# ebanalyse/ebnerd-benchmark

Hardware: AMD Instinct MI355X
Metric: training impressions/sec (higher is better)
Workload: dtype f32

## Files before the change

ebnerd-benchmark_amd/csrc/ebn_attention.hip:

```cpp
#include "ebn_common.h"

int ebn_attn_mfma_fwd(const float* qkv, int64_t ld_qkv, float* out, int64_t ld_out, int64_t n_seq, int32_t L,
                      int32_t h, int32_t d, const EbnDrop& dr, hipStream_t s, bool* handled);
int ebn_attn_mfma_bwd(const float* qkv, int64_t ld_qkv, const float* dout, int64_t ld_dout, float* dqkv,
                      int64_t ld_dqkv, int64_t n_seq, int32_t L, int32_t h, int32_t d, const EbnDrop& dr,
                      hipStream_t s, bool* handled, const float* pool_w, const float* pool_d, int64_t ld_pool);

namespace {

constexpr int DMAX = 32;

struct AttnArgs {
  const float* qkv;
  int64_t ld_qkv;
  const float* dout;
  int64_t ld_dout;
  float* out;
  int64_t ld_out;
  int64_t n_prob;
  int32_t L, h, d;
  const uint32_t* key_ptr;
  uint32_t thresh;
  float scale;
};

template <int GW>
__device__ __forceinline__ void load_tile(float* __restrict__ tile, const float* __restrict__ src,
                                          int64_t ld, int64_t row0, int col0, int L, int d, int gl) {
  const int n = L * d;
  for (int e = gl; e < n; e += GW) {
    const int l = e / d;
    const int c = e - l * d;
    tile[e] = src[(row0 + l) * ld + col0 + c];
  }
}

template <int GW>
__device__ __forceinline__ void softmax_scores(const float* __restrict__ sQ, const float* __restrict__ sK,
                                               float* __restrict__ sP, int L, int LP, int d, int gl) {
  if (gl < L) {
    float q[DMAX];
#pragma unroll
    for (int c = 0; c < DMAX; ++c) q[c] = (c < d) ? sQ[gl * d + c] : 0.f;
    const float inv = 1.0f / sqrtf(static_cast<float>(d));
    float mx = -INFINITY;
    for (int j = 0; j < L; ++j) {
      float s = 0.f;
#pragma unroll
      for (int c = 0; c < DMAX; ++c)
        if (c < d) s = fmaf(q[c], sK[j * d + c], s);
      s *= inv;
      sP[gl * LP + j] = s;
      mx = fmaxf(mx, s);
    }
    float sum = 0.f;
    for (int j = 0; j < L; ++j) {
      const float p = expf(sP[gl * LP + j] - mx);
      sP[gl * LP + j] = p;
      sum += p;
    }
    for (int j = 0; j < L; ++j) sP[gl * LP + j] = sP[gl * LP + j] / sum;
  }
}

template <int GW>
__global__ __launch_bounds__(64) void attn_fwd_kernel(AttnArgs a) {
  extern __shared__ __attribute__((aligned(16))) float smem[];
  constexpr int G = 64 / GW;
  const int lane = threadIdx.x;
  const int g = lane / GW;
  const int gl = lane % GW;
  const int L = a.L, d = a.d;
  const int LP = (L & 1) ? L + 2 : L + 1;
  const int tile = L * d;
  const int per_group = 3 * tile + L * LP;
  float* base = smem + g * per_group;
  float* sQ = base;
  float* sK = base + tile;
  float* sV = base + 2 * tile;
  float* sP = base + 3 * tile;

  const int64_t prob = static_cast<int64_t>(blockIdx.x) * G + g;
  const bool active = prob < a.n_prob;
  const int64_t seq = active ? prob / a.h : 0;
  const int head = active ? static_cast<int>(prob - seq * a.h) : 0;
  const int E = a.h * d;
  const int64_t row0 = seq * L;
  if (active) {
    load_tile<GW>(sQ, a.qkv, a.ld_qkv, row0, head * d, L, d, gl);
// ... 339 lines not shown
  const bool short_ok = L <= 64 && static_cast<size_t>((L <= 32 ? 2 : 1) * (3 * L * d + L * LPs)) * sizeof(float) <= 65536;
  if (!short_ok) {
    const size_t lds = static_cast<size_t>(3 * L * d + 2 * L) * sizeof(float);
    EBN_REQUIRE(lds <= 160 * 1024 && a.n_prob <= 0x7FFFFFFF, EBN_ERR_UNSUPPORTED);
    allow_big_lds(attn_long_fwd_kernel, lds);
    EBN_LAUNCH(attn_long_fwd_kernel, dim3(static_cast<unsigned>(a.n_prob)), dim3(LONG_THREADS), lds, ebn_stream(stream), a);
    EBN_CHECK_LAUNCH();
    return EBN_OK;
  }
  const int LP = (L & 1) ? L + 2 : L + 1;
  const int per_group = 3 * L * d + L * LP;
  EBN_REQUIRE(static_cast<size_t>((L <= 32 ? 2 : 1) * per_group) * sizeof(float) <= 65536, EBN_ERR_UNSUPPORTED);
  if (L <= 32) {
    const int64_t grid = ebn_ceil_div(a.n_prob, 2);
    EBN_LAUNCH(attn_fwd_kernel<32>, dim3(static_cast<unsigned>(grid)), dim3(64),
                       2 * per_group * sizeof(float), ebn_stream(stream), a);
  } else {
    EBN_LAUNCH(attn_fwd_kernel<64>, dim3(static_cast<unsigned>(a.n_prob)), dim3(64),
                       per_group * sizeof(float), ebn_stream(stream), a);
  }
  EBN_CHECK_LAUNCH();
  return EBN_OK;
}

extern "C" int ebn_attn_bwd_f32(const float* qkv, int64_t ld_qkv, const float* dout, int64_t ld_dout,
                                float* dqkv, int64_t ld_dqkv, int64_t n_seq, int32_t L, int32_t h, int32_t d,
                                const ebn_step_state* st, int32_t site, float drop_p, ebn_stream_t stream) {
  int rc = check_attn_args(qkv, dqkv, n_seq, L, h, d);
  if (rc != EBN_OK) return rc;
  EBN_REQUIRE(dout, EBN_ERR_BAD_ARG);
  if (n_seq == 0) return EBN_OK;
  EBN_REQUIRE(ld_qkv >= 3 * h * d && ld_dqkv >= 3 * h * d && ld_dout >= h * d, EBN_ERR_BAD_ARG);
  const EbnDrop dr = ebn_make_drop(st, site, drop_p);
  bool handled = false;
  rc = ebn_attn_mfma_bwd(qkv, ld_qkv, dout, ld_dout, dqkv, ld_dqkv, n_seq, L, h, d, dr, ebn_stream(stream), &handled, nullptr,
                         nullptr, 0);
  if (rc != EBN_OK || handled) return rc;
  AttnArgs a{qkv, ld_qkv, dout, ld_dout, dqkv, ld_dqkv, n_seq * h, L, h, d, dr.key_ptr, dr.thresh, dr.scale};
  const int LPs = (L & 1) ? L + 2 : L + 1;
  const bool short_ok = L <= 64 && static_cast<size_t>((L <= 32 ? 2 : 1) * (4 * L * d + 2 * L * LPs)) * sizeof(float) <= 65536;
  if (!short_ok) {
    const size_t lds = static_cast<size_t>(4 * L * d + 3 * L) * sizeof(float);
    EBN_REQUIRE(lds <= 160 * 1024 && a.n_prob <= 0x7FFFFFFF, EBN_ERR_UNSUPPORTED);
    allow_big_lds(attn_long_bwd_kernel, lds);
    EBN_LAUNCH(attn_long_bwd_kernel, dim3(static_cast<unsigned>(a.n_prob)), dim3(LONG_THREADS), lds, ebn_stream(stream), a);
    EBN_CHECK_LAUNCH();
    return EBN_OK;
  }
  const int LP = (L & 1) ? L + 2 : L + 1;
  const int per_group = 4 * L * d + 2 * L * LP;
  EBN_REQUIRE(static_cast<size_t>((L <= 32 ? 2 : 1) * per_group) * sizeof(float) <= 65536, EBN_ERR_UNSUPPORTED);
  if (L <= 32) {
    const int64_t grid = ebn_ceil_div(a.n_prob, 2);
    EBN_LAUNCH(attn_bwd_kernel<32>, dim3(static_cast<unsigned>(grid)), dim3(64),
                       2 * per_group * sizeof(float), ebn_stream(stream), a);
  } else {
    EBN_LAUNCH(attn_bwd_kernel<64>, dim3(static_cast<unsigned>(a.n_prob)), dim3(64),
                       per_group * sizeof(float), ebn_stream(stream), a);
  }
  EBN_CHECK_LAUNCH();
  return EBN_OK;
}

extern "C" int ebn_attn_bwd_pooled_f32(const float* qkv, int64_t ld_qkv, const float* dout, int64_t ld_dout,
                                       const float* pool_w, const float* pool_dout, int64_t ld_pool, float* dqkv,
                                       int64_t ld_dqkv, int64_t n_seq, int32_t L, int32_t h, int32_t d,
                                       const ebn_step_state* st, int32_t site, float drop_p, ebn_stream_t stream) {
  int rc = check_attn_args(qkv, dqkv, n_seq, L, h, d);
  if (rc != EBN_OK) return rc;
  EBN_REQUIRE(dout && pool_w && pool_dout, EBN_ERR_BAD_ARG);
  if (n_seq == 0) return EBN_OK;
  EBN_REQUIRE(ld_qkv >= 3 * h * d && ld_dqkv >= 3 * h * d && ld_dout >= h * d && ld_pool >= h * d, EBN_ERR_BAD_ARG);
  const EbnDrop dr = ebn_make_drop(st, site, drop_p);
  bool handled = false;
  rc = ebn_attn_mfma_bwd(qkv, ld_qkv, dout, ld_dout, dqkv, ld_dqkv, n_seq, L, h, d, dr, ebn_stream(stream), &handled, pool_w,
                         pool_dout, ld_pool);
  if (rc != EBN_OK) return rc;
  return handled ? EBN_OK : EBN_ERR_UNSUPPORTED;
}

extern "C" int ebn_attn_bwd_pooled_supported(int32_t L, int32_t d) {
  return (L > 0 && L <= 64 && (d == 16 || d == 20 || d == 32)) ? 1 : 0;
}
```

ebnerd-benchmark_amd/csrc/ebn_attention_mfma.hip:

```cpp
#include <stdlib.h>

#include "ebn_common.h"

namespace {

typedef float f32x16 __attribute__((ext_vector_type(16)));

constexpr int ATT_WAVES = 4;

struct MfmaAttnArgs {
  const float* qkv;
  int64_t ld_qkv;
  const float* dout;
  int64_t ld_dout;
  float* out;
  int64_t ld_out;
  int64_t n_prob;
  int32_t L, h;
  const uint32_t* key_ptr;
  uint32_t thresh;
  float scale;
  const float* pool_w;
  const float* pool_d;
  int64_t ld_pool;
  uint32_t stagger_units, stagger_shift, stagger_mod;
};

__device__ __forceinline__ int crow(int r, int hi) { return (r & 3) + 8 * (r >> 2) + 4 * hi; }

template <int D>
struct Tile {
  static constexpr int STRIDE = (D % 16 == 0) ? D + 4 : D;
  static constexpr int FLOATS = 32 * STRIDE;
  static constexpr int VPR = D / 4;
  static constexpr int VECS = 32 * VPR;
  static constexpr int ROUNDS = (VECS + 63) / 64;
};

__device__ __forceinline__ void wave_lds_sync() {
  __builtin_amdgcn_fence(__ATOMIC_RELEASE, "wavefront");
  __builtin_amdgcn_wave_barrier();
  __builtin_amdgcn_fence(__ATOMIC_ACQUIRE, "wavefront");
}

template <int D>
struct Staged {
  float4 v[Tile<D>::ROUNDS];
};

template <int D>
__device__ __forceinline__ void stage_load(Staged<D>& st, const float* __restrict__ base, uint32_t ld, int L, int lane) {
  using T = Tile<D>;
#pragma unroll
  for (int t = 0; t < T::ROUNDS; ++t) {
    int v = lane + 64 * t;
    if (T::VECS % 64 != 0 && v >= T::VECS) v = 0;
    const int r = v / T::VPR, c4 = v - r * T::VPR;
    const uint32_t rc = r < L ? r : 0;
    st.v[t] = *reinterpret_cast<const float4*>(base + (rc * ld + static_cast<uint32_t>(c4 * 4)));
  }
}

template <int D>
struct PoolTerm {
  float w[Tile<D>::ROUNDS];
  float4 p[Tile<D>::ROUNDS];
};

template <int D>
__device__ __forceinline__ void pool_load(PoolTerm<D>& pt, const float* __restrict__ w_rows, const float* __restrict__ d_cols,
                                          int L, int lane) {
  using T = Tile<D>;
#pragma unroll
  for (int t = 0; t < T::ROUNDS; ++t) {
    int v = lane + 64 * t;
    if (T::VECS % 64 != 0 && v >= T::VECS) v = 0;
    const int r = v / T::VPR, c4 = v - r * T::VPR;
    pt.w[t] = w_rows[r < L ? r : 0];
    pt.p[t] = *reinterpret_cast<const float4*>(d_cols + c4 * 4);
  }
}

template <int D>
__device__ __forceinline__ void pool_add(Staged<D>& st, const PoolTerm<D>& pt) {
#pragma unroll
  for (int t = 0; t < Tile<D>::ROUNDS; ++t) {
    st.v[t].x = fmaf(pt.w[t], pt.p[t].x, st.v[t].x);
    st.v[t].y = fmaf(pt.w[t], pt.p[t].y, st.v[t].y);
    st.v[t].z = fmaf(pt.w[t], pt.p[t].z, st.v[t].z);
    st.v[t].w = fmaf(pt.w[t], pt.p[t].w, st.v[t].w);
  }
}

template <int D, bool DROP>
__device__ __forceinline__ void stage_store(float* __restrict__ lds, const Staged<D>& st, int L, int lane, uint32_t key,
                                            uint64_t e0, int E, uint32_t thresh, float scale) {
  using T = Tile<D>;
#pragma unroll
  for (int t = 0; t < T::ROUNDS; ++t) {
    const int v = lane + 64 * t;
    if (T::VECS % 64 != 0 && v >= T::VECS) break;
    const int r = v / T::VPR, c4 = v - r * T::VPR;
    if (r >= L) continue;
    float4 y = st.v[t];
    if (DROP) {
      const uint64_t pr = (e0 >> 1) + ((static_cast<uint32_t>(r) * static_cast<uint32_t>(E) + static_cast<uint32_t>(c4 * 4)) >> 1);
      const uint32_t h0 = ebn_dropout_pair_hash(key, pr), h1 = ebn_dropout_pair_hash(key, pr + 1);
      y.x *= ((h0 & 0xFFFFu) >= thresh) ? scale : 0.f;
// ... 74 lines not shown
                                                 float mul) {
  if (row >= L) return;
#pragma unroll
  for (int g = 0; g < 4; ++g) {
    const int c0 = 8 * g + 4 * hi;
    if (c0 < D) {
      float4 v = make_float4(acc[4 * g] * mul, acc[4 * g + 1] * mul, acc[4 * g + 2] * mul, acc[4 * g + 3] * mul);
      *reinterpret_cast<float4*>(lds + row * Tile<D>::STRIDE + c0) = v;
    }
  }
}

template <int D, bool DROP>
__device__ __forceinline__ void tile_rows_to_global(float* __restrict__ base, uint32_t ld, const f32x16& acc, int L, int row,
                                                    int hi, float mul, uint32_t key, uint64_t e0, int E, uint32_t thresh,
                                                    float scale) {
  if (row >= L) return;
#pragma unroll
  for (int g = 0; g < 4; ++g) {
    const int c0 = 8 * g + 4 * hi;
    if (c0 < D) {
      float4 y = make_float4(acc[4 * g] * mul, acc[4 * g + 1] * mul, acc[4 * g + 2] * mul, acc[4 * g + 3] * mul);
      if (DROP) {
        const uint64_t pr = (e0 >> 1) + ((static_cast<uint32_t>(row) * static_cast<uint32_t>(E) + static_cast<uint32_t>(c0)) >> 1);
        const uint32_t h0 = ebn_dropout_pair_hash(key, pr), h1 = ebn_dropout_pair_hash(key, pr + 1);
        y.x *= ((h0 & 0xFFFFu) >= thresh) ? scale : 0.f;
        y.y *= ((h0 >> 16) >= thresh) ? scale : 0.f;
        y.z *= ((h1 & 0xFFFFu) >= thresh) ? scale : 0.f;
        y.w *= ((h1 >> 16) >= thresh) ? scale : 0.f;
      }
      *reinterpret_cast<float4*>(base + (static_cast<uint32_t>(row) * ld + static_cast<uint32_t>(c0))) = y;
    }
  }
}

template <int D>
__device__ __forceinline__ void global_row_form(float (&x)[D / 2], const float* __restrict__ base, uint32_t ld, int L, int row, int hi) {
  constexpr int KH = D / 2;
  const float2* p = reinterpret_cast<const float2*>(base + (static_cast<uint32_t>(row < L ? row : 0) * ld + static_cast<uint32_t>(hi * KH)));
#pragma unroll
  for (int s = 0; s < KH / 2; ++s) {
    const float2 v = p[s];
    x[2 * s] = v.x;
    x[2 * s + 1] = v.y;
  }
}

__device__ __forceinline__ void softmax_in_lane(f32x16& t, int L, int hi, float inv2) {
  float m = -INFINITY;
#pragma unroll
  for (int r = 0; r < 16; ++r) {
    t[r] *= inv2;
    if (crow(r, hi) < L) m = fmaxf(m, t[r]);
  }
  m = fmaxf(m, __shfl_xor(m, 32, 64));
  float z = 0.f;
#pragma unroll
  for (int r = 0; r < 16; ++r) {
    t[r] = (crow(r, hi) < L) ? __builtin_amdgcn_exp2f(t[r] - m) : 0.f;
    z += t[r];
  }
  z += __shfl_xor(z, 32, 64);
  const float rz = 1.0f / z;
#pragma unroll
  for (int r = 0; r < 16; ++r) t[r] *= rz;
}

constexpr int TP_STRIDE = 36;
constexpr int TP_FLOATS = 32 * TP_STRIDE;

__device__ __forceinline__ void tile_transpose(f32x16& t, float* __restrict__ buf, int L, int lane_row, int hi) {
  float* w = buf + 4 * hi * TP_STRIDE + lane_row;
#pragma unroll
  for (int r = 0; r < 16; ++r) w[((r & 3) + 8 * (r >> 2)) * TP_STRIDE] = t[r];
  wave_lds_sync();
  const float* rd = buf + lane_row * TP_STRIDE + 4 * hi;
#pragma unroll
  for (int g = 0; g < 4; ++g) {
    const float4 v = *reinterpret_cast<const float4*>(rd + 8 * g);
    t[4 * g] = (8 * g + 4 * hi + 0 < L) ? v.x : 0.f;
    t[4 * g + 1] = (8 * g + 4 * hi + 1 < L) ? v.y : 0.f;
    t[4 * g + 2] = (8 * g + 4 * hi + 2 < L) ? v.z : 0.f;
    t[4 * g + 3] = (8 * g + 4 * hi + 3 < L) ? v.w : 0.f;
  }
}


struct AttnProb {
  int64_t row0;
  uint32_t seq;
  uint32_t head;
};

__device__ __forceinline__ uint32_t xcd_chunked_block() {
  const uint32_t nwg = gridDim.x, orig = blockIdx.x;
  const uint32_t q = nwg >> 3, r = nwg & 7u, xcd = orig & 7u, idx = orig >> 3;
  return ((xcd < r) ? xcd * (q + 1) : r * (q + 1) + (xcd - r) * q) + idx;
}

__device__ __forceinline__ void stagger_first_round(const MfmaAttnArgs& a) {
  if (a.stagger_units != 0u && blockIdx.x < (a.stagger_mod << a.stagger_shift)) {
    const uint32_t n = ((blockIdx.x >> a.stagger_shift) % a.stagger_mod) * a.stagger_units;
    for (uint32_t i = 0; i < n; ++i) __builtin_amdgcn_s_sleep(8);
  }
}

__device__ __forceinline__ AttnProb attn_prob(int64_t prob, int h, int L) {
  AttnProb p;
  p.seq = static_cast<uint32_t>(prob) / static_cast<uint32_t>(h);
  p.head = static_cast<uint32_t>(prob) - p.seq * static_cast<uint32_t>(h);
  p.row0 = static_cast<int64_t>(p.seq) * L;
  return p;
}

template <int D>
__host__ __device__ constexpr int fwd_wave_floats(int L) {
  return L * Tile<D>::STRIDE > TP_FLOATS ? L * Tile<D>::STRIDE : TP_FLOATS;
}

template <int D, int LC>
__global__ __launch_bounds__(64 * ATT_WAVES) void attn_mfma_fwd_kernel(MfmaAttnArgs a) {
  extern __shared__ __attribute__((aligned(16))) float smem[];
  const int lane = threadIdx.x & 63;
  const int wv = __builtin_amdgcn_readfirstlane(threadIdx.x >> 6);
  const int64_t prob = static_cast<int64_t>(xcd_chunked_block()) * ATT_WAVES + wv;
  if (prob >= a.n_prob) return;
  const int L = LC ? LC : a.L, E = a.h * D;
  float* sv = smem + wv * fwd_wave_floats<D>(L);
  const int row = lane & 31, hi = lane >> 5;
  const float inv2 = 1.44269504088896341f / sqrtf(static_cast<float>(D));
  const bool drop = a.key_ptr != nullptr;
  const uint32_t key = drop ? *a.key_ptr : 0u;

  const AttnProb p = attn_prob(prob, a.h, L);
  const float* qb = a.qkv + p.row0 * a.ld_qkv + p.head * D;
  float qr[D / 2], kr[D / 2];
  {
    Staged<D> tv;
    stage_load<D>(tv, qb + 2 * E, a.ld_qkv, L, lane);
    global_row_form<D>(qr, qb, a.ld_qkv, L, row, hi);
    global_row_form<D>(kr, qb + E, a.ld_qkv, L, row, hi);
    stage_store<D, false>(sv, tv, L, lane, 0u, 0u, 0, 0u, 0.f);
  }
  wave_lds_sync();
  float vc[16];
  lds_col_form<D>(vc, sv, L, row, hi);

  f32x16 P = mm_rows<D / 2>(kr, qr);
  softmax_in_lane(P, L, hi, inv2);
  wave_lds_sync();
  tile_transpose(P, sv, L, row, hi);
  const f32x16 O = mm_col_tile(vc, P);
  float* ob = a.out + p.row0 * a.ld_out + p.head * D;
  const uint64_t e0 = static_cast<uint64_t>(p.row0) * E + p.head * D;
  if (drop) tile_rows_to_global<D, true>(ob, a.ld_out, O, L, row, hi, 1.0f, key, e0, E, a.thresh, a.scale);
  else tile_rows_to_global<D, false>(ob, a.ld_out, O, L, row, hi, 1.0f, 0u, 0u, 0, 0u, 0.f);
}

template <int D>
__host__ __device__ constexpr int fwd_group_v_offset(int L) {
  return 2 * L * Tile<D>::STRIDE > TP_FLOATS ? 2 * L * Tile<D>::STRIDE : TP_FLOATS;
}
__host__ __device__ constexpr int group_tile_pad(int L);
template <int D>
__host__ __device__ constexpr int fwd_group_wave_floats(int L) {
  return fwd_group_v_offset<D>(L) + L * Tile<D>::STRIDE + group_tile_pad(L);
// ... 14 lines not shown
  const int wave_floats = fwd_group_wave_floats<D>(L), v_off = fwd_group_v_offset<D>(L);
  const int row = lane & 31, hi = lane >> 5;
  const float inv2 = 1.44269504088896341f / sqrtf(static_cast<float>(D));
  const bool drop = a.key_ptr != nullptr;
  const uint32_t key = drop ? *a.key_ptr : 0u;

  const AttnProb p0 = attn_prob(static_cast<int64_t>(xcd_chunked_block()) * G, a.h, L);
  const uint32_t gcol = p0.head * D;
  const float* gq = a.qkv + p0.row0 * a.ld_qkv + gcol;
  const int nvec = L * GV;
  {
    float4 vq[ROUNDS], vk[ROUNDS], vv[ROUNDS];
    uint32_t dst[ROUNDS];
#pragma unroll
    for (int t = 0; t < ROUNDS; ++t) {
      const int idx = tid + NT * t;
      const int idc = idx < nvec ? idx : 0;
      const uint32_t r = static_cast<uint32_t>(idc) / static_cast<uint32_t>(GV), c4g = static_cast<uint32_t>(idc) - r * GV;
      const uint32_t head = c4g / T::VPR, c4 = c4g - head * T::VPR;
      dst[t] = head * wave_floats + r * T::STRIDE + c4 * 4;
      const uint32_t off = r * static_cast<uint32_t>(a.ld_qkv) + c4g * 4;
      vq[t] = *reinterpret_cast<const float4*>(gq + off);
      vk[t] = *reinterpret_cast<const float4*>(gq + E + off);
      vv[t] = *reinterpret_cast<const float4*>(gq + 2 * E + off);
    }
#pragma unroll
    for (int t = 0; t < ROUNDS; ++t) {
      if (tid + NT * t < nvec) {
        *reinterpret_cast<float4*>(smem + dst[t]) = vq[t];
        *reinterpret_cast<float4*>(smem + dst[t] + region) = vk[t];
        *reinterpret_cast<float4*>(smem + dst[t] + v_off) = vv[t];
      }
    }
  }
  __syncthreads();

  float* sq = smem + wv * wave_floats;
  float* sk = sq + region;
  float* sv = sq + v_off;
  f32x16 P;
  {
    float qr[D / 2], kr[D / 2];
    lds_row_form<D>(qr, sq, L, row, hi);
    lds_row_form<D>(kr, sk, L, row, hi);
    P = mm_rows<D / 2>(kr, qr);
  }
  float vc[16];
  lds_col_form<D>(vc, sv, L, row, hi);
  softmax_in_lane(P, L, hi, inv2);
  wave_lds_sync();
  tile_transpose(P, sq, L, row, hi);
  {
    const f32x16 O = mm_col_tile(vc, P);
    tile_rows_to_lds<D>(sv, O, L, row, hi, 1.0f);
  }
  __syncthreads();

  float* go = a.out + p0.row0 * a.ld_out + gcol;
#pragma unroll
  for (int t = 0; t < ROUNDS; ++t) {
    const int idx = tid + NT * t;
    if (idx < nvec) {
      const uint32_t r = static_cast<uint32_t>(idx) / static_cast<uint32_t>(GV), c4g = static_cast<uint32_t>(idx) - r * GV;
      const uint32_t head = c4g / T::VPR, c4 = c4g - head * T::VPR;
      float4 y = *reinterpret_cast<const float4*>(smem + head * wave_floats + v_off + r * T::STRIDE + c4 * 4);
      if (drop) {
        const uint64_t pr = ((static_cast<uint64_t>(p0.row0) * E + gcol) >> 1) + ((r * static_cast<uint32_t>(E) + c4g * 4) >> 1);
        const uint32_t h0 = ebn_dropout_pair_hash(key, pr), h1 = ebn_dropout_pair_hash(key, pr + 1);
        y.x *= ((h0 & 0xFFFFu) >= a.thresh) ? a.scale : 0.f;
        y.y *= ((h0 >> 16) >= a.thresh) ? a.scale : 0.f;
        y.z *= ((h1 & 0xFFFFu) >= a.thresh) ? a.scale : 0.f;
        y.w *= ((h1 >> 16) >= a.thresh) ? a.scale : 0.f;
      }
      *reinterpret_cast<float4*>(go + (r * static_cast<uint32_t>(a.ld_out) + c4g * 4)) = y;
    }
  }
}

template <int D>
__host__ __device__ constexpr int bwd_wave_floats(int L) {
  return 3 * L * Tile<D>::STRIDE > L * Tile<D>::STRIDE + TP_FLOATS ? 3 * L * Tile<D>::STRIDE : L * Tile<D>::STRIDE + TP_FLOATS;
}

template <int D, int LC>
__global__ __launch_bounds__(64 * ATT_WAVES) void attn_mfma_bwd_kernel(MfmaAttnArgs a) {
  using T = Tile<D>;
  constexpr int KH = D / 2;
  extern __shared__ __attribute__((aligned(16))) float smem[];
  const int lane = threadIdx.x & 63;
  const int wv = __builtin_amdgcn_readfirstlane(threadIdx.x >> 6);
  const int64_t prob = static_cast<int64_t>(xcd_chunked_block()) * ATT_WAVES + wv;
  if (prob >= a.n_prob) return;
  const int L = LC ? LC : a.L, E = a.h * D;
  const int region = L * T::STRIDE;
  float* sq = smem + wv * bwd_wave_floats<D>(L);
  float* sk = sq + region;
  float* sg = sk + region;
  const int row = lane & 31, hi = lane >> 5;
  const float inv = 1.0f / sqrtf(static_cast<float>(D));
  const float inv2 = inv * 1.44269504088896341f;
  const bool drop = a.key_ptr != nullptr, pooled = a.pool_w != nullptr;
  const uint32_t key = drop ? *a.key_ptr : 0u;

  const AttnProb p = attn_prob(prob, a.h, L);
  const float* qb = a.qkv + p.row0 * a.ld_qkv + p.head * D;
  float vr[KH];
  {
    Staged<D> tq, tk, tg;
    stage_load<D>(tq, qb, a.ld_qkv, L, lane);
    stage_load<D>(tk, qb + E, a.ld_qkv, L, lane);
    stage_load<D>(tg, a.dout + p.row0 * a.ld_dout + p.head * D, a.ld_dout, L, lane);
    global_row_form<D>(vr, qb + 2 * E, a.ld_qkv, L, row, hi);
    if (pooled) {
      PoolTerm<D> pt;
      pool_load<D>(pt, a.pool_w + p.row0, a.pool_d + p.seq * a.ld_pool + p.head * D, L, lane);
      pool_add<D>(tg, pt);
    }
    stage_store<D, false>(sq, tq, L, lane, 0u, 0u, 0, 0u, 0.f);
    stage_store<D, false>(sk, tk, L, lane, 0u, 0u, 0, 0u, 0.f);
    if (drop) stage_store<D, true>(sg, tg, L, lane, key, static_cast<uint64_t>(p.row0) * E + p.head * D, E, a.thresh, a.scale);
    else stage_store<D, false>(sg, tg, L, lane, 0u, 0u, 0, 0u, 0.f);
  }
  wave_lds_sync();

  float* ob = a.out + p.row0 * a.ld_out + p.head * D;
  f32x16 P, dP;
  {
    float qr[KH], kr[KH];
    lds_row_form<D>(qr, sq, L, row, hi);
    lds_row_form<D>(kr, sk, L, row, hi);
    P = mm_rows<KH>(kr, qr);
  }
  softmax_in_lane(P, L, hi, inv2);
  {
    float gr[KH];
    lds_row_form<D>(gr, sg, L, row, hi);
    dP = mm_rows<KH>(gr, vr);
  }
  float rowdot = 0.f;
#pragma unroll
  for (int r = 0; r < 16; ++r) rowdot = fmaf(P[r], dP[r], rowdot);
  rowdot += __shfl_xor(rowdot, 32, 64);

  float col[16];
  lds_col_form<D>(col, sg, L, row, hi);
  {
    const f32x16 dV = mm_col_tile(col, P);
    tile_rows_to_global<D, false>(ob + 2 * E, a.ld_out, dV, L, row, hi, 1.0f, 0u, 0u, 0, 0u, 0.f);
  }
#pragma unroll
  for (int r = 0; r < 16; ++r) P[r] = P[r] * (dP[r] - rowdot);
  lds_col_form<D>(col, sk, L, row, hi);
  {
    const f32x16 dQ = mm_col_tile(col, P);
    tile_rows_to_global<D, false>(ob, a.ld_out, dQ, L, row, hi, inv, 0u, 0u, 0, 0u, 0.f);
  }
  wave_lds_sync();
  tile_transpose(P, sk, L, row, hi);
  lds_col_form<D>(col, sq, L, row, hi);
  {
    const f32x16 dK = mm_col_tile(col, P);
    tile_rows_to_global<D, false>(ob + E, a.ld_out, dK, L, row, hi, inv, 0u, 0u, 0, 0u, 0.f);
  }
}


template <int D>
__host__ __device__ constexpr int bwd_group_g_offset(int L) {
  return 2 * L * Tile<D>::STRIDE > TP_FLOATS ? 2 * L * Tile<D>::STRIDE : TP_FLOATS;
}
__host__ __device__ constexpr int group_tile_pad(int L) { return L == 30 ? 12 : 0; }
template <int D>
__host__ __device__ constexpr int bwd_group_wave_floats(int L) {
  return bwd_group_g_offset<D>(L) + L * Tile<D>::STRIDE + group_tile_pad(L);
}

template <int D, int LC, int G>
__global__ __launch_bounds__(64 * G) void attn_mfma_bwd_group_kernel(MfmaAttnArgs a) {
  using T = Tile<D>;
  constexpr int KH = D / 2;
  constexpr int NT = 64 * G;
  constexpr int GV = G * T::VPR;
  constexpr int ROUNDS = (32 * GV + NT - 1) / NT;
  extern __shared__ __attribute__((aligned(16))) float smem[];
  const int tid = threadIdx.x;
  const int lane = tid & 63;
  const int wv = __builtin_amdgcn_readfirstlane(tid >> 6);
  const int L = LC ? LC : a.L, E = a.h * D;
  const int region = L * T::STRIDE;
  const int wave_floats = bwd_group_wave_floats<D>(L), g_off = bwd_group_g_offset<D>(L);
  const int row = lane & 31, hi = lane >> 5;
  const float inv = 1.0f / sqrtf(static_cast<float>(D));
  const float inv2 = inv * 1.44269504088896341f;
  const bool drop = a.key_ptr != nullptr, pooled = a.pool_w != nullptr;
  const uint32_t key = drop ? *a.key_ptr : 0u;

  stagger_first_round(a);
  const AttnProb p0 = attn_prob(static_cast<int64_t>(xcd_chunked_block()) * G, a.h, L);
  const uint32_t gcol = p0.head * D;
  const float* gq = a.qkv + p0.row0 * a.ld_qkv + gcol;
  const float* gd = a.dout + p0.row0 * a.ld_dout + gcol;
  const int nvec = L * GV;
  float vr[KH];
// ... 150 lines not shown
  for (int r = 0; r < 16; ++r) {
    const int il = crow(r, hi);
    const float ci = __shfl(c_ib, il, 64);
    s[r] = (32 * ib + il < L) ? __builtin_amdgcn_exp2f(s[r] * inv2 - ci) : 0.f;
  }
}

template <int D, int LC>
__global__ __launch_bounds__(64 * ATT2_WAVES) void attn_mfma2_fwd_kernel(MfmaAttnArgs a) {
  using T = Tile<D>;
  constexpr int KH = D / 2;
  extern __shared__ __attribute__((aligned(16))) float smem[];
  const int lane = threadIdx.x & 63;
  const int wv = __builtin_amdgcn_readfirstlane(threadIdx.x >> 6);
  const int64_t prob = static_cast<int64_t>(xcd_chunked_block()) * ATT2_WAVES + wv;
  if (prob >= a.n_prob) return;
  const int L = LC ? LC : a.L, E = a.h * D;
  const int region = L * T::STRIDE;
  float* sq = smem + wv * 3 * region;
  float* sk = sq + region;
  float* sv = sk + region;
  const int row = lane & 31, hi = lane >> 5;
  const int64_t seq = prob / a.h;
  const int head = static_cast<int>(prob - seq * a.h);
  const int64_t row0 = seq * L;
  const float* qb = a.qkv + row0 * a.ld_qkv + head * D;
  const float inv2 = 1.44269504088896341f / sqrtf(static_cast<float>(D));
  {
    Staged<D> tq[NB2], tk[NB2], tv[NB2];
#pragma unroll
    for (int b = 0; b < NB2; ++b) {
      stage_load<D>(tq[b], qb + 32 * b * a.ld_qkv, a.ld_qkv, L - 32 * b, lane);
      stage_load<D>(tk[b], qb + E + 32 * b * a.ld_qkv, a.ld_qkv, L - 32 * b, lane);
      stage_load<D>(tv[b], qb + 2 * E + 32 * b * a.ld_qkv, a.ld_qkv, L - 32 * b, lane);
    }
#pragma unroll
    for (int b = 0; b < NB2; ++b) {
      stage_store<D, false>(sq + 32 * b * T::STRIDE, tq[b], L - 32 * b, lane, 0u, 0u, 0, 0u, 0.f);
      stage_store<D, false>(sk + 32 * b * T::STRIDE, tk[b], L - 32 * b, lane, 0u, 0u, 0, 0u, 0.f);
      stage_store<D, false>(sv + 32 * b * T::STRIDE, tv[b], L - 32 * b, lane, 0u, 0u, 0, 0u, 0.f);
    }
  }
  wave_lds_sync();
  float qr[NB2][KH], kr[NB2][KH], vc[NB2][16];
#pragma unroll
  for (int b = 0; b < NB2; ++b) {
    lds_row_form<D>(qr[b], sq + 32 * b * T::STRIDE, L - 32 * b, row, hi);
    lds_row_form<D>(kr[b], sk + 32 * b * T::STRIDE, L - 32 * b, row, hi);
    lds_col_form<D>(vc[b], sv + 32 * b * T::STRIDE, L - 32 * b, row, hi);
  }
  float c[NB2];
#pragma unroll
  for (int ib = 0; ib < NB2; ++ib) {
    f32x16 t[NB2];
#pragma unroll
    for (int jb = 0; jb < NB2; ++jb) t[jb] = mm_rows<KH>(kr[jb], qr[ib]);
    c[ib] = softmax2_in_lane<false>(t, L, hi, inv2);
  }
  wave_lds_sync();
#pragma unroll
  for (int jb = 0; jb < NB2; ++jb) {
    f32x16 O = zero_tile();
#pragma unroll
    for (int ib = 0; ib < NB2; ++ib) {
      f32x16 S = mm_rows<KH>(qr[ib], kr[jb]);
      softmax2_from_stats(S, L, ib, hi, inv2, c[ib]);
      mm_col_tile_acc(O, vc[ib], S);
    }
    tile_rows_to_lds<D>(sq + 32 * jb * T::STRIDE, O, L - 32 * jb, row, hi, 1.0f);
  }
  wave_lds_sync();
  float* ob = a.out + row0 * a.ld_out + head * D;
  const uint64_t e0 = static_cast<uint64_t>(row0) * E + head * D;
#pragma unroll
  for (int b = 0; b < NB2; ++b) {
    if (a.key_ptr != nullptr)
      stage_out<D, true>(sq + 32 * b * T::STRIDE, ob + 32 * b * a.ld_out, a.ld_out, L - 32 * b, lane, *a.key_ptr,
                         e0 + static_cast<uint64_t>(32 * b) * E, E, a.thresh, a.scale);
    else
      stage_out<D, false>(sq + 32 * b * T::STRIDE, ob + 32 * b * a.ld_out, a.ld_out, L - 32 * b, lane, 0u, 0u, 0, 0u, 0.f);
  }
}

template <int D, int LC>
__global__ __launch_bounds__(64 * ATT2_WAVES) void attn_mfma2_bwd_kernel(MfmaAttnArgs a) {
  using T = Tile<D>;
  constexpr int KH = D / 2;
  extern __shared__ __attribute__((aligned(16))) float smem[];
  const int lane = threadIdx.x & 63;
  const int wv = __builtin_amdgcn_readfirstlane(threadIdx.x >> 6);
  const int64_t prob = static_cast<int64_t>(xcd_chunked_block()) * ATT2_WAVES + wv;
  if (prob >= a.n_prob) return;
  const int L = LC ? LC : a.L, E = a.h * D;
  const int region = L * T::STRIDE;
  float* sq = smem + wv * 4 * region;
  float* sk = sq + region;
  float* sv = sk + region;
  float* sg = sv + region;
  const int row = lane & 31, hi = lane >> 5;
  const int64_t seq = prob / a.h;
  const int head = static_cast<int>(prob - seq * a.h);
  const int64_t row0 = seq * L;
  const float* qb = a.qkv + row0 * a.ld_qkv + head * D;
  const float* gb = a.dout + row0 * a.ld_dout + head * D;
  const float inv = 1.0f / sqrtf(static_cast<float>(D));
  const float inv2 = inv * 1.44269504088896341f;
#pragma unroll
  for (int b = 0; b < NB2; ++b) {
    Staged<D> tq, tk, tv, tg;
    const int Lb = L - 32 * b;
    stage_load<D>(tq, qb + 32 * b * a.ld_qkv, a.ld_qkv, Lb, lane);
    stage_load<D>(tk, qb + E + 32 * b * a.ld_qkv, a.ld_qkv, Lb, lane);
    stage_load<D>(tv, qb + 2 * E + 32 * b * a.ld_qkv, a.ld_qkv, Lb, lane);
    stage_load<D>(tg, gb + 32 * b * a.ld_dout, a.ld_dout, Lb, lane);
    if (a.pool_w != nullptr) {
      PoolTerm<D> pt;
      pool_load<D>(pt, a.pool_w + row0 + 32 * b, a.pool_d + seq * a.ld_pool + head * D, Lb, lane);
      pool_add<D>(tg, pt);
    }
    stage_store<D, false>(sq + 32 * b * T::STRIDE, tq, Lb, lane, 0u, 0u, 0, 0u, 0.f);
    stage_store<D, false>(sk + 32 * b * T::STRIDE, tk, Lb, lane, 0u, 0u, 0, 0u, 0.f);
    stage_store<D, false>(sv + 32 * b * T::STRIDE, tv, Lb, lane, 0u, 0u, 0, 0u, 0.f);
    if (a.key_ptr != nullptr)
      stage_store<D, true>(sg + 32 * b * T::STRIDE, tg, Lb, lane, *a.key_ptr,
                           static_cast<uint64_t>(row0 + 32 * b) * E + head * D, E, a.thresh, a.scale);
    else
      stage_store<D, false>(sg + 32 * b * T::STRIDE, tg, Lb, lane, 0u, 0u, 0, 0u, 0.f);
  }
  wave_lds_sync();

  float* ob = a.out + row0 * a.ld_out + head * D;
  float c[NB2], rowdot[NB2];
  float vr[NB2][KH];
#pragma unroll
  for (int b = 0; b < NB2; ++b) lds_row_form<D>(vr[b], sv + 32 * b * T::STRIDE, L - 32 * b, row, hi);
  wave_lds_sync();
#pragma unroll
  for (int ib = 0; ib < NB2; ++ib) {
    f32x16 P[NB2], dP[NB2];
    {
      float qr[KH];
      lds_row_form<D>(qr, sq + 32 * ib * T::STRIDE, L - 32 * ib, row, hi);
#pragma unroll
      for (int jb = 0; jb < NB2; ++jb) {
        float kr[KH];
        lds_row_form<D>(kr, sk + 32 * jb * T::STRIDE, L - 32 * jb, row, hi);
        P[jb] = mm_rows<KH>(kr, qr);
      }
    }
    c[ib] = softmax2_in_lane<true>(P, L, hi, inv2);
    float rd = 0.f;
#pragma unroll
    for (int jb = 0; jb < NB2; ++jb) {
      float gr[KH];
      lds_row_form<D>(gr, sg + 32 * jb * T::STRIDE, L - 32 * jb, row, hi);
      dP[jb] = mm_rows<KH>(gr, vr[ib]);
#pragma unroll
      for (int r = 0; r < 16; ++r) rd = fmaf(P[jb][r], dP[jb][r], rd);
    }
    rd += __shfl_xor(rd, 32, 64);
    rowdot[ib] = rd;
    float col[16];
    {
      f32x16 dV = zero_tile();
#pragma unroll
      for (int jb = 0; jb < NB2; ++jb) {
        lds_col_form<D>(col, sg + 32 * jb * T::STRIDE, L - 32 * jb, row, hi);
        mm_col_tile_acc(dV, col, P[jb]);
      }
      wave_lds_sync();
      tile_rows_to_lds<D>(sv + 32 * ib * T::STRIDE, dV, L - 32 * ib, row, hi, 1.0f);
      wave_lds_sync();
      stage_out<D, false>(sv + 32 * ib * T::STRIDE, ob + 2 * E + 32 * ib * a.ld_out, a.ld_out, L - 32 * ib, lane, 0u, 0u, 0, 0u, 0.f);
    }
#pragma unroll
    for (int jb = 0; jb < NB2; ++jb)
#pragma unroll
      for (int r = 0; r < 16; ++r) P[jb][r] = P[jb][r] * (dP[jb][r] - rd);
    {
      f32x16 dQ = zero_tile();
#pragma unroll
      for (int jb = 0; jb < NB2; ++jb) {
        lds_col_form<D>(col, sk + 32 * jb * T::STRIDE, L - 32 * jb, row, hi);
        mm_col_tile_acc(dQ, col, P[jb]);
      }
      wave_lds_sync();
      tile_rows_to_lds<D>(sv + 32 * ib * T::STRIDE, dQ, L - 32 * ib, row, hi, inv);
      wave_lds_sync();
      stage_out<D, false>(sv + 32 * ib * T::STRIDE, ob + 32 * ib * a.ld_out, a.ld_out, L - 32 * ib, lane, 0u, 0u, 0, 0u, 0.f);
    }
  }
#pragma unroll
  for (int jb = 0; jb < NB2; ++jb) {
    float kr[KH], gr[KH];
    lds_row_form<D>(kr, sk + 32 * jb * T::STRIDE, L - 32 * jb, row, hi);
    lds_row_form<D>(gr, sg + 32 * jb * T::STRIDE, L - 32 * jb, row, hi);
    f32x16 dK = zero_tile();
#pragma unroll
    for (int ib = 0; ib < NB2; ++ib) {
      f32x16 P, dP;
      {
        float qr[KH];
        lds_row_form<D>(qr, sq + 32 * ib * T::STRIDE, L - 32 * ib, row, hi);
        P = mm_rows<KH>(qr, kr);
      }
      softmax2_from_stats(P, L, ib, hi, inv2, c[ib]);
      dP = mm_rows<KH>(vr[ib], gr);
#pragma unroll
      for (int r = 0; r < 16; ++r) {
        const float rdi = __shfl(rowdot[ib], crow(r, hi), 64);
        P[r] = P[r] * (dP[r] - rdi);
// ... 68 lines not shown
}

template <int D>
static void launch_mfma2(bool bwd, const MfmaAttnArgs& a, hipStream_t s) {
  if (D == 20 && a.L == 50 && !bwd) launch_mfma2_lc<D, 50>(bwd, a, s);
  else launch_mfma2_lc<D, 0>(bwd, a, s);
}

int ebn_attn_mfma_fwd(const float* qkv, int64_t ld_qkv, float* out, int64_t ld_out, int64_t n_seq, int32_t L,
                      int32_t h, int32_t d, const EbnDrop& dr, hipStream_t s, bool* handled) {
  *handled = mfma_path_ok(L, d, ld_qkv, ld_out, ld_out, qkv, out, out) && n_seq * h < (int64_t{1} << 31);
  if (!*handled) return EBN_OK;
  MfmaAttnArgs a{qkv, ld_qkv, nullptr, 0, out, ld_out, n_seq * h, L, h, dr.key_ptr, dr.thresh, dr.scale, nullptr, nullptr, 0, 0u, 0u, 1u};
  if (L > 32) {
    if (d == 16) launch_mfma2<16>(false, a, s);
    else if (d == 20) launch_mfma2<20>(false, a, s);
    else launch_mfma2<32>(false, a, s);
    EBN_CHECK_LAUNCH();
    return EBN_OK;
  }
  const bool big = a.n_prob * L * 3 * d * static_cast<int64_t>(sizeof(float)) >= FWD_GROUP_MIN_QKV_BYTES;
  if (d == 20 && (h % BWD_GROUP) == 0 && big && !bwd_group_off()) {
    const size_t lds = static_cast<size_t>(BWD_GROUP) * fwd_group_wave_floats<20>(L) * sizeof(float);
    const dim3 grid(static_cast<unsigned>(a.n_prob / BWD_GROUP)), block(64 * BWD_GROUP);
    if (L == 30) {
      allow_lds(attn_mfma_fwd_group_kernel<20, 30, BWD_GROUP>, lds);
      EBN_LAUNCH((attn_mfma_fwd_group_kernel<20, 30, BWD_GROUP>), grid, block, lds, s, a);
    } else {
      allow_lds(attn_mfma_fwd_group_kernel<20, 0, BWD_GROUP>, lds);
      EBN_LAUNCH((attn_mfma_fwd_group_kernel<20, 0, BWD_GROUP>), grid, block, lds, s, a);
    }
    EBN_CHECK_LAUNCH();
    return EBN_OK;
  }
  const size_t wb = static_cast<size_t>(ATT_WAVES) * sizeof(float);
  if (d == 16) launch_waves(attn_mfma_fwd_kernel<16, 0>, wb * fwd_wave_floats<16>(L), a, s);
  else if (d == 20 && L == 30) launch_waves(attn_mfma_fwd_kernel<20, 30>, wb * fwd_wave_floats<20>(L), a, s);
  else if (d == 20 && L == 20) launch_waves(attn_mfma_fwd_kernel<20, 20>, wb * fwd_wave_floats<20>(L), a, s);
  else if (d == 20) launch_waves(attn_mfma_fwd_kernel<20, 0>, wb * fwd_wave_floats<20>(L), a, s);
  else launch_waves(attn_mfma_fwd_kernel<32, 0>, wb * fwd_wave_floats<32>(L), a, s);
  EBN_CHECK_LAUNCH();
  return EBN_OK;
}

int ebn_attn_mfma_bwd(const float* qkv, int64_t ld_qkv, const float* dout, int64_t ld_dout, float* dqkv,
                      int64_t ld_dqkv, int64_t n_seq, int32_t L, int32_t h, int32_t d, const EbnDrop& dr,
                      hipStream_t s, bool* handled, const float* pool_w, const float* pool_d, int64_t ld_pool) {
  *handled = mfma_path_ok(L, d, ld_qkv, ld_dout, ld_dqkv, qkv, dout, dqkv) && n_seq * h < (int64_t{1} << 31) &&
             (pool_w == nullptr || ((ld_pool % 4) == 0 && ebn_aligned16(pool_d)));
  if (!*handled) return EBN_OK;
  MfmaAttnArgs a{qkv, ld_qkv, dout, ld_dout, dqkv, ld_dqkv, n_seq * h, L, h, dr.key_ptr, dr.thresh, dr.scale, pool_w, pool_d, ld_pool, 0u, 0u, 1u};
  if (L > 32) {
    if (d == 16) launch_mfma2<16>(true, a, s);
    else if (d == 20) launch_mfma2<20>(true, a, s);
    else launch_mfma2<32>(true, a, s);
    EBN_CHECK_LAUNCH();
    return EBN_OK;
  }
  if (d == 20 && (h % BWD_GROUP) == 0 && a.n_prob >= BWD_GROUP_MIN_PROBLEMS && !bwd_group_off()) {
    const size_t lds = static_cast<size_t>(BWD_GROUP) * bwd_group_wave_floats<20>(L) * sizeof(float);
    const dim3 grid(static_cast<unsigned>(a.n_prob / BWD_GROUP)), block(64 * BWD_GROUP);
    a.stagger_shift = stagger_shift_of_device();
    a.stagger_units = a.stagger_shift != 0u ? 7u : 0u;
    a.stagger_mod = 5u;
    if (L == 30) {
      allow_lds(attn_mfma_bwd_group_kernel<20, 30, BWD_GROUP>, lds);
      EBN_LAUNCH((attn_mfma_bwd_group_kernel<20, 30, BWD_GROUP>), grid, block, lds, s, a);
    } else {
      allow_lds(attn_mfma_bwd_group_kernel<20, 0, BWD_GROUP>, lds);
      EBN_LAUNCH((attn_mfma_bwd_group_kernel<20, 0, BWD_GROUP>), grid, block, lds, s, a);
    }
    EBN_CHECK_LAUNCH();
    return EBN_OK;
  }
  const size_t wb = static_cast<size_t>(ATT_WAVES) * sizeof(float);
  if (d == 16) launch_waves(attn_mfma_bwd_kernel<16, 0>, wb * bwd_wave_floats<16>(L), a, s);
  else if (d == 20 && L == 30) launch_waves(attn_mfma_bwd_kernel<20, 30>, wb * bwd_wave_floats<20>(L), a, s);
  else if (d == 20 && L == 20) launch_waves(attn_mfma_bwd_kernel<20, 20>, wb * bwd_wave_floats<20>(L), a, s);
  else if (d == 20) launch_waves(attn_mfma_bwd_kernel<20, 0>, wb * bwd_wave_floats<20>(L), a, s);
  else launch_waves(attn_mfma_bwd_kernel<32, 0>, wb * bwd_wave_floats<32>(L), a, s);
  EBN_CHECK_LAUNCH();
  return EBN_OK;
}
```

ebnerd-benchmark_amd/csrc/ebn_encoder.hip:

```cpp
#include "ebn_common.h"

#define EBN_TRY(call)            \
  do {                           \
    int rc__ = (call);           \
    if (rc__ != EBN_OK) return rc__; \
  } while (0)

static int check_dims(const ebn_encoder_dims* d) {
  EBN_REQUIRE(d, EBN_ERR_BAD_ARG);
  EBN_REQUIRE(d->n_seq >= 0 && d->L > 0 && d->Din > 0 && d->h > 0 && d->d > 0 && d->A > 0, EBN_ERR_BAD_ARG);
  return EBN_OK;
}

extern "C" int ebn_encoder_fwd_f32(const ebn_encoder_dims* dims, const ebn_encoder_params* p,
                                   const ebn_encoder_acts* a, const ebn_encoder_scratch* s,
                                   const ebn_step_state* st, ebn_stream_t stream) {
  EBN_TRY(check_dims(dims));
  EBN_REQUIRE(p && a && p->Wqkv && p->W && p->b && p->q, EBN_ERR_BAD_ARG);
  EBN_REQUIRE(a->X && a->QKV && a->Y && a->U && a->w && a->out, EBN_ERR_BAD_ARG);
  const int64_t R = dims->n_seq * dims->L;
  const int E = dims->h * dims->d;
  if (R == 0) return EBN_OK;
  float* ws = s ? s->gemm_ws : nullptr;
  const int64_t ws_n = s ? s->gemm_ws_floats : 0;
  EBN_TRY(ebn_gemm_f32_site(0, 0, R, 3 * E, dims->Din, 1.0f, a->X, dims->Din, p->Wqkv, 3 * E, 0.0f, a->QKV, 3 * E, ws, ws_n,
                            1, stream));
  EBN_TRY(ebn_attn_fwd_f32(a->QKV, 3 * E, a->Y, E, dims->n_seq, dims->L, dims->h, dims->d, st, dims->drop_site,
                           dims->drop_p, stream));
  EBN_TRY(ebn_gemm_f32_ws(0, 0, R, dims->A, E, 1.0f, a->Y, E, p->W, dims->A, 0.0f, a->U, dims->A, ws, ws_n, stream));
  EBN_TRY(ebn_attpool_fwd_f32(a->U, p->b, p->q, a->Y, a->out, a->w, dims->n_seq, dims->L, E, dims->A, stream));
  return EBN_OK;
}

extern "C" int ebn_encoder_fwd_gather_f32(const ebn_encoder_dims* dims, const ebn_encoder_params* p, const ebn_encoder_acts* a,
                                          const ebn_encoder_scratch* s, const int32_t* ids, const float* table, int64_t table_rows,
                                          int32_t* oob_flag, ebn_stream_t stream) {
  EBN_TRY(check_dims(dims));
  EBN_REQUIRE(p && a && ids && table && p->Wqkv && p->W && p->b && p->q, EBN_ERR_BAD_ARG);
  EBN_REQUIRE(a->QKV && a->Y && a->U && a->w && a->out, EBN_ERR_BAD_ARG);
  EBN_REQUIRE(dims->drop_p <= 0.0f, EBN_ERR_UNSUPPORTED);
  const int64_t R = dims->n_seq * dims->L;
  const int E = dims->h * dims->d;
  if (R == 0) return EBN_OK;
  float* ws = s ? s->gemm_ws : nullptr;
  const int64_t ws_n = s ? s->gemm_ws_floats : 0;
  EBN_TRY(ebn_gemm_f32_rowmap(ids, table_rows, R, 3 * E, dims->Din, table, dims->Din, p->Wqkv, 3 * E, a->QKV, 3 * E, oob_flag, stream));
  EBN_TRY(ebn_attn_fwd_f32(a->QKV, 3 * E, a->Y, E, dims->n_seq, dims->L, dims->h, dims->d, nullptr, -1, 0.0f, stream));
  EBN_TRY(ebn_gemm_f32_ws(0, 0, R, dims->A, E, 1.0f, a->Y, E, p->W, dims->A, 0.0f, a->U, dims->A, ws, ws_n, stream));
  EBN_TRY(ebn_attpool_fwd_f32(a->U, p->b, p->q, a->Y, a->out, a->w, dims->n_seq, dims->L, E, dims->A, stream));
  return EBN_OK;
}

extern "C" int ebn_encoder_bwd_f32(const ebn_encoder_dims* dims, const ebn_encoder_params* p,
                                   const ebn_encoder_acts* a, const float* dout, const ebn_encoder_grads* g,
                                   const ebn_encoder_scratch* s, float* dX, int32_t accumulate,
                                   const ebn_step_state* st, ebn_stream_t stream) {
  EBN_TRY(check_dims(dims));
  EBN_REQUIRE(p && a && g && s && dout, EBN_ERR_BAD_ARG);
  EBN_REQUIRE(p->Wqkv && p->W && p->q, EBN_ERR_BAD_ARG);
  EBN_REQUIRE(a->X && a->QKV && a->Y && a->U && a->w, EBN_ERR_BAD_ARG);
  EBN_REQUIRE(g->dWqkv && g->dW && g->db && g->dq, EBN_ERR_BAD_ARG);
  EBN_REQUIRE(s->dY && s->dQKV && s->de && s->partials, EBN_ERR_BAD_ARG);
  const int64_t R = dims->n_seq * dims->L;
  const int E = dims->h * dims->d;
  const int A = dims->A;
  if (R == 0) return EBN_OK;
  const float beta = accumulate ? 1.0f : 0.0f;
  EBN_TRY(ebn_attpool_bwd_pool_f32(a->Y, a->w, dout, nullptr, s->de, dims->n_seq, dims->L, E, stream));
  EBN_TRY(ebn_attpool_bwd_dpre_f32(a->U, p->q, s->de, g->dq, g->db, s->partials, R, A, accumulate, stream));
  const bool fold = ebn_attn_bwd_pooled_supported(dims->L, dims->d) != 0 && (E % 4) == 0 && ebn_aligned16(dout) &&
                    ebn_aligned16(s->dY) && ebn_aligned16(a->QKV) && ebn_aligned16(s->dQKV);
  if (fold) {
    EBN_TRY(ebn_dense_bwd_pair_f32(R, E, A, a->Y, E, a->U, A, p->W, A, beta, g->dW, A, s->dY, E, s->gemm_ws, s->gemm_ws_floats,
                                   stream));
    EBN_TRY(ebn_attn_bwd_pooled_f32(a->QKV, 3 * E, s->dY, E, a->w, dout, E, s->dQKV, 3 * E, dims->n_seq, dims->L, dims->h,
                                    dims->d, st, dims->drop_site, dims->drop_p, stream));
  } else {
    EBN_TRY(ebn_gemm_f32_ws(1, 0, E, A, R, 1.0f, a->Y, E, a->U, A, beta, g->dW, A, s->gemm_ws, s->gemm_ws_floats, stream));
    EBN_TRY(ebn_gemm_f32_rank1(R, E, A, 1.0f, a->U, A, p->W, A, s->dY, E, a->w, dout, E, dims->L, s->gemm_ws,
                               s->gemm_ws_floats, stream));
    EBN_TRY(ebn_attn_bwd_f32(a->QKV, 3 * E, s->dY, E, s->dQKV, 3 * E, dims->n_seq, dims->L, dims->h, dims->d, st, dims->drop_site,
                             dims->drop_p, stream));
  }
  if (dX != nullptr)
    return ebn_dense_bwd_pair_f32(R, dims->Din, 3 * E, a->X, dims->Din, s->dQKV, 3 * E, p->Wqkv, 3 * E, beta, g->dWqkv, 3 * E, dX,
                                  dims->Din, s->gemm_ws, s->gemm_ws_floats, stream);
  EBN_TRY(ebn_gemm_f32_ws(1, 0, dims->Din, 3 * E, R, 1.0f, a->X, dims->Din, s->dQKV, 3 * E, beta, g->dWqkv, 3 * E,
                          s->gemm_ws, s->gemm_ws_floats, stream));
  return EBN_OK;
}

extern "C" int ebn_user_stage_train_f32(const ebn_encoder_dims* dims, const ebn_encoder_params* p, const ebn_encoder_acts* a,
                                        const float* cand, const float* labels, float* scores, float* probs, float* loss_rows,
                                        float* loss_out, float* dcand, float* duser, const ebn_encoder_grads* g,
                                        const ebn_encoder_scratch* s, float* head_partials, float* dX, int32_t C,
                                        int32_t loss_kind, float inv_batch, const ebn_step_state* st, ebn_stream_t stream) {
  EBN_TRY(check_dims(dims));
  EBN_REQUIRE(p && a && g && s && cand && labels && scores && probs && loss_rows && loss_out && dcand && duser && dX, EBN_ERR_BAD_ARG);
  EBN_REQUIRE(p->Wqkv && p->W && p->b && p->q && a->X && a->QKV && a->Y && a->U && a->w && a->out, EBN_ERR_BAD_ARG);
  EBN_REQUIRE(g->dWqkv && g->dW && g->db && g->dq && s->dY && s->dQKV && s->de && s->partials, EBN_ERR_BAD_ARG);
  EBN_REQUIRE(C > 0 && dims->drop_p <= 0.0f, EBN_ERR_BAD_ARG);
  const int64_t B = dims->n_seq, R = dims->n_seq * dims->L;
  const int E = dims->h * dims->d, A = dims->A, L = dims->L;
  if (R == 0) return EBN_OK;
  const bool fused = head_partials != nullptr && ebn_user_head_supported(L, C, E, A) != 0 &&
                     ebn_attn_bwd_pooled_supported(L, dims->d) != 0 && ebn_aligned16(a->U) && ebn_aligned16(a->Y) &&
                     ebn_aligned16(cand) && ebn_aligned16(dcand) && ebn_aligned16(duser) && ebn_aligned16(a->out) &&
                     ebn_aligned16(p->b) && ebn_aligned16(p->q) && ebn_aligned16(s->dY) && ebn_aligned16(a->QKV) &&
                     ebn_aligned16(s->dQKV);
  if (!fused) {
    EBN_TRY(ebn_encoder_fwd_f32(dims, p, a, s, st, stream));
    EBN_TRY(ebn_score_loss_train_f32(cand, a->out, labels, scores, probs, loss_rows, loss_out, dcand, duser, B, C, E, loss_kind,
                                     inv_batch, stream));
    return ebn_encoder_bwd_f32(dims, p, a, duser, g, s, dX, 0, st, stream);
  }
  float* ws = s->gemm_ws;
  const int64_t ws_n = s->gemm_ws_floats;
  EBN_TRY(ebn_gemm_f32_site(0, 0, R, 3 * E, dims->Din, 1.0f, a->X, dims->Din, p->Wqkv, 3 * E, 0.0f, a->QKV, 3 * E, ws, ws_n, 1, stream));
  EBN_TRY(ebn_attn_fwd_f32(a->QKV, 3 * E, a->Y, E, B, L, dims->h, dims->d, nullptr, -1, 0.0f, stream));
  EBN_TRY(ebn_gemm_f32_ws(0, 0, R, A, E, 1.0f, a->Y, E, p->W, A, 0.0f, a->U, A, ws, ws_n, stream));
  EBN_TRY(ebn_user_head_train_f32(a->U, p->b, p->q, a->Y, cand, labels, a->w, a->out, scores, probs, loss_rows, loss_out, dcand,
                                  duser, s->de, g->dq, g->db, head_partials, B, L, C, E, A, loss_kind, inv_batch, stream));
  EBN_TRY(ebn_dense_bwd_pair_f32(R, E, A, a->Y, E, a->U, A, p->W, A, 0.0f, g->dW, A, s->dY, E, ws, ws_n, stream));
  EBN_TRY(ebn_attn_bwd_pooled_f32(a->QKV, 3 * E, s->dY, E, a->w, duser, E, s->dQKV, 3 * E, B, L, dims->h, dims->d, nullptr, -1, 0.0f,
                                  stream));
  return ebn_dense_bwd_pair_f32(R, dims->Din, 3 * E, a->X, dims->Din, s->dQKV, 3 * E, p->Wqkv, 3 * E, 0.0f, g->dWqkv, 3 * E, dX,
                                dims->Din, ws, ws_n, stream);
}
```

ebnerd-benchmark_amd/csrc/ebn_gemm.hip:

```cpp
#include <stdlib.h>

#include "ebn_common.h"
#include "ebn_finish.h"
#include "ebn_tn_finale.h"

typedef float ebn_f32x4 __attribute__((ext_vector_type(4)));
typedef int ebn_i32x4 __attribute__((ext_vector_type(4)));
__device__ ebn_f32x4 ebn_raw_buffer_load_x4(ebn_i32x4 rsrc, int voffset, int soffset, int aux) __asm("llvm.amdgcn.raw.buffer.load.v4f32");
__device__ void ebn_raw_buffer_load_lds(ebn_i32x4 rsrc, __attribute__((address_space(3))) void* lds, int size, int voffset,
                                        int soffset, int offset, int aux) __asm("llvm.amdgcn.raw.buffer.load.lds");

int ebn_gemm_direct_tn_slices(int64_t M, int64_t N, int64_t K);
int ebn_gemm_direct_tn_launch(int64_t M, int64_t N, int64_t K, float alpha, const float* A, int64_t lda, const float* B, int64_t ldb,
                              float* part, hipStream_t s);
bool ebn_gemm_direct_wanted(int32_t transA, int32_t transB, int64_t M, int64_t N, int64_t K);
int ebn_gemm_direct_launch(int32_t transB, int64_t M, int64_t N, int64_t K, float alpha, const float* A, int64_t lda, const float* B,
                           int64_t ldb, float* C, int64_t ldc, hipStream_t s);

namespace {

typedef float f32x16 __attribute__((ext_vector_type(16)));


typedef float f32x4n __attribute__((ext_vector_type(4)));
// ... 798 lines not shown
  if (nk > 1) EBN_SM_LOAD(1, 1);
  EBN_SM_STORE(0, 0);
  __syncthreads();
  for (int kt = 0; kt < nk; kt += 2) {
    if (kt + 2 < nk) EBN_SM_LOAD(0, kt + 2);
    EBN_SM_MMA(0, kt);
    if (kt + 1 < nk) EBN_SM_STORE(1, 1);
    __syncthreads();
    if (kt + 1 >= nk) break;
    if (kt + 3 < nk) EBN_SM_LOAD(1, kt + 3);
    EBN_SM_MMA(1, kt + 1);
    if (kt + 2 < nk) EBN_SM_STORE(0, 0);
    __syncthreads();
  }
#undef EBN_SM_LOAD
#undef EBN_SM_STORE
#undef EBN_SM_MMA
#undef EBN_SM_READ
#undef EBN_SM_MUL
  const f32x4 acc = (acc0 + acc1) + (acc2 + acc3);
  if (do_colsum) {
    constexpr int CG = T / 4, KR = THREADS / CG;
    float* sc = smem_small;
    *reinterpret_cast<float4*>(&sc[(tid / CG) * (T + 4) + (tid % CG) * 4]) = csum;
    __syncthreads();
    if (tid < T && n0 + tid < N) {
      float t = 0.f;
      for (int r = 0; r < KR; ++r) t += sc[r * (T + 4) + tid];
      epi.colsum[n0 + tid] = t;
      if (FIN) ebn_adam_flat_apply(fin->adam, fin->adam.st->adam_alpha, (epi.colsum + n0 + tid) - fin->adam.grad, t);
    }
  }
  const int64_t col = n0 + wn * 16 + r16;
  if (col < N) {
    const float al = FIN ? fin->adam.st->adam_alpha : 0.f;
#pragma unroll
    for (int r = 0; r < 4; ++r) {
      const int64_t row = m0 + wm * 16 + 4 * kq + r;
      if (row >= M) continue;
      float v = alpha * acc[r];
      if (beta != 0.f) v += beta * C[row * ldc + col];
      if (epi.rs != nullptr)
        v = fmaf(epi.rs[row], epi.cv[static_cast<int64_t>(static_cast<uint32_t>(row) / static_cast<uint32_t>(epi.L)) * epi.ldcv + col], v);
      if (epi.bias != nullptr) v = fmaxf(v + epi.bias[col], 0.f);
      if (epi.l2w != nullptr) v = fmaf(epi.two_lambda, epi.l2w[row * ldc + col], v);
      C[row * ldc + col] = v;
      if (FIN) ebn_adam_flat_apply(fin->adam, al, (C + row * ldc + col) - fin->adam.grad, v);
    }
  }
}

template <bool TA, bool TB, int T>
__global__ __launch_bounds__(T * T / 4) void gemm_small_vec_kernel(int64_t M, int64_t N, int64_t K, float alpha,
                                                                      const float* __restrict__ A, int64_t lda,
                                                                      const float* __restrict__ B, int64_t ldb, float beta,
                                                                      float* __restrict__ C, int64_t ldc, GemmEpi epi) {
  small_vec_body<TA, TB, T>(M, N, K, alpha, A, lda, B, ldb, beta, C, ldc, epi, blockIdx.x, blockIdx.y);
}

struct SmallProblem {
  int64_t M, N, K;
  float alpha;
  const float* A;
  int64_t lda;
  const float* B;
  int64_t ldb;
  float beta;
  float* C;
  int64_t ldc;
  int32_t tiles_x, tiles;
};

__global__ __launch_bounds__(GEMM_THREADS) void gemm_small_pair_kernel(SmallProblem p0, SmallProblem p1) {
  const GemmEpi none{nullptr, nullptr, 0, 1, nullptr};
  const int b = blockIdx.x;
  if (b < p0.tiles)
    small_vec_body<true, false, 32>(p0.M, p0.N, p0.K, p0.alpha, p0.A, p0.lda, p0.B, p0.ldb, p0.beta, p0.C, p0.ldc, none,
                                    b % p0.tiles_x, b / p0.tiles_x);
  else
    small_vec_body<false, true, 32>(p1.M, p1.N, p1.K, p1.alpha, p1.A, p1.lda, p1.B, p1.ldb, p1.beta, p1.C, p1.ldc, none,
                                    (b - p0.tiles) % p1.tiles_x, (b - p0.tiles) / p1.tiles_x);
}

struct SmallGroup {
  SmallProblem p[EBN_TN_GROUP_MAX];
  float* colsum[EBN_TN_GROUP_MAX];
  const float* l2w[EBN_TN_GROUP_MAX];
  float two_lambda[EBN_TN_GROUP_MAX];
  int32_t first[EBN_TN_GROUP_MAX + 1];
  int32_t n;
};

__device__ __forceinline__ int xcd_chunked_tile(int v, int nwg) {
  const int q = nwg >> 3, r = nwg & 7, xcd = v & 7, idx = v >> 3;
  return ((xcd < r) ? xcd * (q + 1) : r * (q + 1) + (xcd - r) * q) + idx;
}

template <int T>
__global__ __launch_bounds__(T * T / 4) void gemm_small_tn_group_kernel(SmallGroup g) {
  const int b = xcd_chunked_tile(blockIdx.x, gridDim.x);
  int i = 0;
  while (i + 1 < g.n && b >= g.first[i + 1]) ++i;
  const SmallProblem& p = g.p[i];
  GemmEpi epi{nullptr, nullptr, 0, 1, nullptr};
  epi.colsum = g.colsum[i];
  epi.l2w = g.l2w[i];
  epi.two_lambda = g.two_lambda[i];
  const int t = b - g.first[i];
  small_vec_body<true, false, T>(p.M, p.N, p.K, p.alpha, p.A, p.lda, p.B, p.ldb, p.beta, p.C, p.ldc, epi, t % p.tiles_x, t / p.tiles_x);
}

static_assert(EBN_TN_FINALE_MAX_REST == EBN_DVN_FINALE_MAX_REST, "ebn_tn_finale.h / ebnerd_hip.h");
struct SmallGroupFin {
  SmallGroup g;
  EbnTnFinale f;
};

template <int T>
__global__ __launch_bounds__(T * T / 4) void gemm_small_tn_finale_kernel(SmallGroupFin gf) {
  extern __shared__ __attribute__((aligned(16))) float smem_small[];
  const SmallGroup& g = gf.g;
  const EbnTnFinale& f = gf.f;
  const int nwg = gridDim.x, tid = threadIdx.x, b = xcd_chunked_tile(blockIdx.x, nwg);
  constexpr int NT = T * T / 4;
  if (b < g.first[g.n]) {
    int i = 0;
    while (i + 1 < g.n && b >= g.first[i + 1]) ++i;
    const SmallProblem& p = g.p[i];
    GemmEpi epi{nullptr, nullptr, 0, 1, nullptr};
    epi.colsum = g.colsum[i];
    epi.l2w = g.l2w[i];
    epi.two_lambda = g.two_lambda[i];
    const int t = b - g.first[i];
    small_vec_body<true, false, T, true>(p.M, p.N, p.K, p.alpha, p.A, p.lda, p.B, p.ldb, p.beta, p.C, p.ldc, epi, t % p.tiles_x, t / p.tiles_x, &f);
  }
  const float al = f.adam.st->adam_alpha;
  {
    const int64_t per = (f.rest_total + nwg - 1) / nwg, e0 = static_cast<int64_t>(b) * per;
    const int64_t e1 = e0 + per < f.rest_total ? e0 + per : f.rest_total;
    for (int64_t e = e0 + tid; e < e1; e += NT) {
      int64_t off = e;
      int r = 0;
      while (r + 1 < f.n_rest && off >= f.rest_len[r]) off -= f.rest_len[r++];
      off += f.rest_off[r];
      ebn_adam_flat_apply(f.adam, al, off, f.adam.grad[off]);
    }
  }
  const int nh = (2 * f.A + 255) / 256 + 1;
  if (f.head_partials != nullptr && b < nh) {
    __syncthreads();
    ebn_user_head_finish_body(smem_small, b, nh, f.head_partials, f.B, f.A, f.dq, f.db, f.loss_rows, f.loss_out);
    if (b < nh - 1) {
      const int idx = b * 256 + tid;
      if (tid < 256 && idx < 2 * f.A) {
        const int sidx = idx / f.A, k = idx - sidx * f.A;
        float* gp = (sidx == 0 ? f.dq : f.db) + k;
        ebn_adam_flat_apply(f.adam, al, gp - f.adam.grad, *gp);
      }
    } else if (tid == 0 && f.n_l2 > 0) {
      float tot = 0.f;
      for (int l = 0; l < f.n_l2; ++l) {
        float tl = 0.f;
        for (int j = 0; j < f.l2_tiles[l]; ++j) tl += f.l2_part[l * f.l2_slots + j];
        tot += tl;
      }
      f.loss_out[0] += f.l2 * tot;
// ... 242 lines not shown
  EBN_REQUIRE(M < (static_cast<int64_t>(1) << 31), EBN_ERR_UNSUPPORTED);
  if (M == 0 || N == 0) return EBN_OK;
  EBN_REQUIRE(A && B && C && row_scale && seq_rows, EBN_ERR_BAD_ARG);
  EBN_REQUIRE(lda >= K && ldb >= K && ldc >= N && ld_seq >= N, EBN_ERR_BAD_ARG);
  const GemmEpi epi{row_scale, seq_rows, ld_seq, L, nullptr};
  hipStream_t s = ebn_stream(stream);
  const bool vec = (lda % 4) == 0 && ebn_aligned16(A) && (ldb % 4) == 0 && ebn_aligned16(B) && (K % 4) == 0;
  if (vec)
    return gemm_dispatch(0, 1, M, N, K, alpha, A, lda, B, ldb, 0.0f, C, ldc, workspace, workspace_floats, 0, epi, s);
  int64_t grid = ebn_ceil_div(M * N, 256);
  if (grid > 4096) grid = 4096;
  EBN_LAUNCH(rank1_fill_kernel, dim3(static_cast<unsigned>(grid)), dim3(256), 0, s, C, ldc, M, N, epi);
  EBN_CHECK_LAUNCH();
  return gemm_dispatch(0, 1, M, N, K, alpha, A, lda, B, ldb, 1.0f, C, ldc, workspace, workspace_floats, 0,
                       GemmEpi{nullptr, nullptr, 0, 1, nullptr}, s);
}

extern "C" int ebn_dense_relu_fwd_f32(int64_t M, int64_t N, int64_t K, const float* A, int64_t lda, const float* B,
                                      int64_t ldb, const float* bias, float* C, int64_t ldc, float* workspace,
                                      int64_t workspace_floats, ebn_stream_t stream) {
  EBN_REQUIRE(M >= 0 && N >= 0 && K >= 0, EBN_ERR_BAD_ARG);
  if (M == 0 || N == 0) return EBN_OK;
  EBN_REQUIRE(A && B && C && bias, EBN_ERR_BAD_ARG);
  EBN_REQUIRE(lda >= K && ldb >= N && ldc >= N, EBN_ERR_BAD_ARG);
  hipStream_t s = ebn_stream(stream);
  const bool vec = (lda % 4) == 0 && ebn_aligned16(A) && (K % 4) == 0 && (ldb % 4) == 0 && ebn_aligned16(B) && (N % 4) == 0;
  if (vec)
    return gemm_dispatch(0, 0, M, N, K, 1.0f, A, lda, B, ldb, 0.0f, C, ldc, workspace, workspace_floats, 0,
                         GemmEpi{nullptr, nullptr, 0, 1, bias}, s);
  const int rc = gemm_dispatch(0, 0, M, N, K, 1.0f, A, lda, B, ldb, 0.0f, C, ldc, workspace, workspace_floats, 0,
                               GemmEpi{nullptr, nullptr, 0, 1, nullptr}, s);
  if (rc != EBN_OK) return rc;
  for (int64_t r = 0; ldc != N && r < M; ++r) {
    const int rr = ebn_bias_relu_f32(C + r * ldc, bias, C + r * ldc, 1, static_cast<int32_t>(N), stream);
    if (rr != EBN_OK) return rr;
  }
  return (ldc == N) ? ebn_bias_relu_f32(C, bias, C, M, static_cast<int32_t>(N), stream) : EBN_OK;
}

extern "C" int ebn_gemm_f32_ws(int32_t transA, int32_t transB, int64_t M, int64_t N, int64_t K, float alpha,
                               const float* A, int64_t lda, const float* B, int64_t ldb, float beta,
                               float* C, int64_t ldc, float* workspace, int64_t workspace_floats,
                               ebn_stream_t stream) {
  return ebn_gemm_f32_site(transA, transB, M, N, K, alpha, A, lda, B, ldb, beta, C, ldc, workspace, workspace_floats, 0,
                           stream);
}

extern "C" int ebn_dense_bwd_pair_f32(int64_t R, int64_t K_in, int64_t N_out, const float* X, int64_t ldx, const float* dY,
                                      int64_t lddy, const float* W, int64_t ldw, float beta_w, float* dW, int64_t lddw,
                                      float* dX, int64_t lddx, float* workspace, int64_t workspace_floats,
                                      ebn_stream_t stream) {
  EBN_REQUIRE(R >= 0 && K_in >= 0 && N_out >= 0, EBN_ERR_BAD_ARG);
  if (K_in == 0 || N_out == 0) return EBN_OK;
  EBN_REQUIRE(X && dY && W && dW && dX, EBN_ERR_BAD_ARG);
  EBN_REQUIRE(ldx >= K_in && lddy >= N_out && ldw >= N_out && lddw >= N_out && lddx >= K_in, EBN_ERR_BAD_ARG);
  hipStream_t s = ebn_stream(stream);
  const bool aligned = (ldx % 4) == 0 && (lddy % 4) == 0 && (ldw % 4) == 0 && ebn_aligned16(X) && ebn_aligned16(dY) &&
                       ebn_aligned16(W) && (K_in % 4) == 0 && (N_out % 4) == 0;
  const int64_t span = (R + SBK) * (ldx > lddy ? ldx : lddy) * 4 + 64 * ((ldx > lddy ? ldx : lddy) > ldw ? (ldx > lddy ? ldx : lddy) : ldw) * 4;
  const bool small = R > 0 && gemm_plan(K_in, N_out, R, workspace ? workspace_floats : 0).bm == 32 &&
                     gemm_plan(R, K_in, N_out, workspace ? workspace_floats : 0).bm == 32;
  if (aligned && small && span < (int64_t{1} << 31)) {
    SmallProblem p0{K_in, N_out, R, 1.0f, X, ldx, dY, lddy, beta_w, dW, lddw, static_cast<int32_t>(ebn_ceil_div(N_out, SBN)), 0};
    p0.tiles = p0.tiles_x * static_cast<int32_t>(ebn_ceil_div(K_in, SBM));
    SmallProblem p1{R, K_in, N_out, 1.0f, dY, lddy, W, ldw, 0.0f, dX, lddx, static_cast<int32_t>(ebn_ceil_div(K_in, SBN)), 0};
    p1.tiles = p1.tiles_x * static_cast<int32_t>(ebn_ceil_div(R, SBM));
    constexpr size_t lds = static_cast<size_t>(2) * 2 * SBM * SLV * sizeof(float);
    static const hipError_t attr = hipFuncSetAttribute(reinterpret_cast<const void*>(&gemm_small_pair_kernel),
                                                       hipFuncAttributeMaxDynamicSharedMemorySize, static_cast<int>(lds));
    if (attr != hipSuccess) return static_cast<int>(attr);
    EBN_LAUNCH(gemm_small_pair_kernel, dim3(static_cast<unsigned>(p0.tiles + p1.tiles)), dim3(GEMM_THREADS), lds, s, p0, p1);
    EBN_CHECK_LAUNCH();
    return EBN_OK;
  }
  const GemmEpi none{nullptr, nullptr, 0, 1, nullptr};
  if (R == 0) {
    return gemm_dispatch(1, 0, K_in, N_out, 0, 1.0f, X, ldx, dY, lddy, beta_w, dW, lddw, workspace, workspace_floats, 0, none, s);
  }
  const int rc = gemm_dispatch(1, 0, K_in, N_out, R, 1.0f, X, ldx, dY, lddy, beta_w, dW, lddw, workspace, workspace_floats, 0, none, s);
  if (rc != EBN_OK) return rc;
  return gemm_dispatch(0, 1, R, K_in, N_out, 1.0f, dY, lddy, W, ldw, 0.0f, dX, lddx, workspace, workspace_floats, 0, none, s);
}

extern "C" int ebn_gemm_f32_rowmap(const int32_t* ids, int64_t table_rows, int64_t M, int64_t N, int64_t K, const float* table,
                                   int64_t ldt, const float* B, int64_t ldb, float* C, int64_t ldc, int32_t* oob_flag, ebn_stream_t stream) {
  EBN_REQUIRE(ebn_dim_ok(M, N, K) && table_rows > 0, EBN_ERR_BAD_ARG);
  if (M == 0 || N == 0) return EBN_OK;
  EBN_REQUIRE(ids && table && B && C && ldt >= K && ldb >= N && ldc >= N && K > 0, EBN_ERR_BAD_ARG);
  const bool ok = M >= 256 && (ldt % 4) == 0 && (ldb % 4) == 0 && (K % 4) == 0 && (N % 4) == 0 && ebn_aligned16(table) && ebn_aligned16(B) &&
                  (table_rows * ldt + K + 16) * 4 < (int64_t{1} << 32) && ((K + 16) * ldb + 256) * 4 < (int64_t{1} << 32);
  if (!ok) return EBN_ERR_UNSUPPORTED;
  GemmEpi epi{nullptr, nullptr, 0, 1, nullptr};
  epi.rowmap = ids;
  epi.rowmap_rows = table_rows;
  epi.oob = oob_flag;
  return launch_gemm<256, 64, 4>(0, 0, M, N, K, 1.0f, table, ldt, B, ldb, 0.0f, C, ldc, 1, 1, 1, ebn_ceil_div(K, BK) * BK, nullptr,
                                 ebn_stream(stream), 0, epi);
}

extern "C" int ebn_gemm_tn_group_f32(const ebn_tn_problem* problems, int32_t n, ebn_stream_t stream) {
  EBN_REQUIRE(problems != nullptr && n >= 1 && n <= EBN_TN_GROUP_MAX, EBN_ERR_BAD_ARG);
  int64_t tiles64 = 0;
  for (int i = 0; i < n; ++i) {
    const ebn_tn_problem& q = problems[i];
    EBN_REQUIRE(ebn_dim_ok(q.M, q.N, q.K) && q.K >= 1, EBN_ERR_BAD_ARG);
    if (q.M == 0 || q.N == 0) continue;
    EBN_REQUIRE(q.A && q.B && q.C, EBN_ERR_BAD_ARG);
    EBN_REQUIRE(q.lda >= q.M && q.ldb >= q.N && q.ldc >= q.N, EBN_ERR_BAD_ARG);
    EBN_REQUIRE((q.lda % 4) == 0 && (q.ldb % 4) == 0 && (q.M % 4) == 0 && (q.N % 4) == 0 && ebn_aligned16(q.A) && ebn_aligned16(q.B),
                EBN_ERR_UNSUPPORTED);
    EBN_REQUIRE((q.K + SBK) * (q.lda > q.ldb ? q.lda : q.ldb) * 4 + 64 * 4 < (int64_t{1} << 31), EBN_ERR_UNSUPPORTED);
    tiles64 += ebn_ceil_div(q.M, 64) * ebn_ceil_div(q.N, 64);
  }
  const int T = tiles64 >= 192 ? 64 : 32;
  SmallGroup g{};
  int64_t total = 0;
  g.n = 0;
  for (int i = 0; i < n; ++i) {
    const ebn_tn_problem& q = problems[i];
    if (q.M == 0 || q.N == 0) continue;
    const int j = g.n++;
    g.p[j] = SmallProblem{q.M, q.N, q.K, 1.0f, q.A, q.lda, q.B, q.ldb, 0.0f, q.C, q.ldc, static_cast<int32_t>(ebn_ceil_div(q.N, T)), 0};
    g.p[j].tiles = g.p[j].tiles_x * static_cast<int32_t>(ebn_ceil_div(q.M, T));
    g.colsum[j] = q.colsum;
    g.l2w[j] = q.l2_W;
    g.two_lambda[j] = q.two_lambda;
    g.first[j] = static_cast<int32_t>(total);
    total += g.p[j].tiles;
    EBN_REQUIRE(total < (int64_t{1} << 30), EBN_ERR_UNSUPPORTED);
  }
  if (g.n == 0) return EBN_OK;
  g.first[g.n] = static_cast<int32_t>(total);
#define EBN_TN_GROUP(TT)                                                                                                          \
  do {                                                                                                                            \
    constexpr size_t lds = static_cast<size_t>(2) * 2 * (TT) * SLV * sizeof(float);                                               \
    static const hipError_t attr = hipFuncSetAttribute(reinterpret_cast<const void*>(&gemm_small_tn_group_kernel<TT>),            \
                                                       hipFuncAttributeMaxDynamicSharedMemorySize, static_cast<int>(lds));        \
    if (attr != hipSuccess) return static_cast<int>(attr);                                                                        \
    EBN_LAUNCH(gemm_small_tn_group_kernel<TT>, dim3(static_cast<unsigned>(total)), dim3((TT) * (TT) / 4), lds, ebn_stream(stream), g); \
  } while (0)
  if (T == 64) EBN_TN_GROUP(64);
  else EBN_TN_GROUP(32);
#undef EBN_TN_GROUP
  EBN_CHECK_LAUNCH();
  return EBN_OK;
}

int ebn_tn_group_finale_launch(const ebn_tn_problem* problems, int32_t n, const EbnTnFinale& fin, hipStream_t s) {
  EBN_REQUIRE(problems != nullptr && n >= 1 && n <= EBN_TN_GROUP_MAX, EBN_ERR_BAD_ARG);
  int64_t tiles64 = 0;
  for (int i = 0; i < n; ++i) {
    const ebn_tn_problem& q = problems[i];
    EBN_REQUIRE(ebn_dim_ok(q.M, q.N, q.K) && q.K >= 1 && q.M > 0 && q.N > 0, EBN_ERR_BAD_ARG);
    EBN_REQUIRE(q.A && q.B && q.C, EBN_ERR_BAD_ARG);
    EBN_REQUIRE(q.lda >= q.M && q.ldb >= q.N && q.ldc >= q.N, EBN_ERR_BAD_ARG);
    EBN_REQUIRE((q.lda % 4) == 0 && (q.ldb % 4) == 0 && (q.M % 4) == 0 && (q.N % 4) == 0 && ebn_aligned16(q.A) && ebn_aligned16(q.B),
                EBN_ERR_UNSUPPORTED);
    EBN_REQUIRE((q.K + SBK) * (q.lda > q.ldb ? q.lda : q.ldb) * 4 + 64 * 4 < (int64_t{1} << 31), EBN_ERR_UNSUPPORTED);
    tiles64 += ebn_ceil_div(q.M, 64) * ebn_ceil_div(q.N, 64);
  }
  const int T = tiles64 >= 192 ? 64 : 32;
  SmallGroupFin gf{};
  gf.f = fin;
  SmallGroup& g = gf.g;
  int64_t total = 0;
  g.n = n;
// ... 34 lines not shown
```

ebnerd-benchmark_amd/ebrec/models/newsrec/_engine.py:

```python
from __future__ import annotations

import ctypes

import numpy as np
import torch

from ebrec import _hip

from ._engine_base import (ADAM_EPS, BCE_ON, BETA1, BETA2, LOSS_KIND, FlatParams, StepStateOwner, conv_glorot_np,
                           glorot_uniform_np, loss_kind_of, pair_score_tail, require_gpu, score_loss_tail)
from ._engine_segments import SegmentsMixin
from ._engine_staging import StagingMixin


def eval_loss_from_news(eng, news_all: torch.Tensor, his_idx, pred_idx, y):
    his_idx, pred_idx = np.asarray(his_idx), np.asarray(pred_idx)
    B, C = his_idx.shape[0], pred_idx.shape[1]
    H, E = his_idx.shape[1], eng.E
    idx = torch.from_numpy(np.ascontiguousarray(np.concatenate([his_idx.reshape(-1), pred_idx.reshape(-1)]), dtype=np.int32)).to(eng.device)
    NE = torch.empty(B * (H + C), E, device=eng.device)
    S = _hip.stream_handle
    _hip.call("ebn_gather_rows_f32", _hip.ptr(idx), _hip.ptr(news_all), _hip.ptr(NE), B * (H + C), E, news_all.shape[0], None, -1,
              ctypes.c_float(0.0), None, S())
    user = eng.encode_users_from_news(NE[: B * H].view(B, H, E))
# ... 11 lines not shown
        self.QKV, self.Y, self.U, self.w = f(R, 3 * E), f(R, E), f(R, A), f(R)
        self.out = f(n_seq, E)
        self.dY, self.dQKV, self.de = f(R, E), f(R, 3 * E), f(R)
        self.partials = f(int(_hip.lib().ebn_attpool_partials_len(R, A)))
        wsf = _hip.lib().ebn_gemm_workspace_floats
        ws = max(int(wsf(Din, 3 * E, R)), int(wsf(E, A, R)), int(wsf(R, 3 * E, Din)), int(wsf(R, A, E)), int(wsf(R, E, A)),
                 int(wsf(R, Din, 3 * E)), 1)
        self.ws = f(ws)
        self.fwd_scratch = _hip.EncoderScratch(None, None, None, None, self.ws.data_ptr(), self.ws.numel())
        self.dX = f(R, Din) if need_dx else None


class NRMSEngine(StagingMixin, SegmentsMixin, StepStateOwner):
    def __init__(self, table: np.ndarray, title_size: int, history_size: int, head_num: int, head_dim: int,
                 attention_hidden_dim: int, dropout: float, learning_rate: float, loss: str, seed=None,
                 train_embedding: bool = True, device=None, process_group=None, shard_table: bool = False,
                 shard_mode: str = "alltoall", deterministic: bool = True, units=None, l2: float = 0.0,
                 shard_partition: str | None = None, shard_capacity_factor: float = 1.25, table_grad_exchange: str = "auto",
                 bce_on: str = "logits", precision: str = "exact"):
        self.device = require_gpu() if device is None else torch.device(device)
        if precision not in ("exact", "split"):
            raise ValueError(f"precision must be 'exact' (fp32 MFMA, the default) or 'split' (bf16x6 split on the bf16 matrix pipe, "
                             f"fp32-accurate, fp32 accumulate), got {precision}")
        self.precision = precision
        if loss not in LOSS_KIND:
            raise ValueError(f"this loss not defined {loss}")
        loss_kind_of(loss, bce_on)
        self.bce_on = bce_on
        self.T, self.H = int(title_size), int(history_size)
        self.h, self.d, self.A = int(head_num), int(head_dim), int(attention_hidden_dim)
        self.E = self.h * self.d
        self.p = float(dropout)
        self.loss = loss
        self.seed = seed
        self.train_embedding = bool(train_embedding)
        if table_grad_exchange not in ("auto", "dense", "sparse"):
            raise ValueError(f"table_grad_exchange must be auto | dense | sparse, got {table_grad_exchange}")
        self.table_grad_exchange = table_grad_exchange
        self._sparse_pin = None
        self.pg = process_group
        table = np.ascontiguousarray(table, dtype=np.float32)
        self.V, self.D = table.shape
        self.exchange = None
        if shard_table:
            from ._dist import ShardedTableExchange

            self.exchange = ShardedTableExchange(self.V, self.D, group=process_group, mode=shard_mode, partition=shard_partition,
                                                 capacity_factor=shard_capacity_factor)
            table = self.exchange.shard_of(table)
        self.table = torch.from_numpy(np.ascontiguousarray(table)).to(self.device)
        D, E, A = self.D, self.E, self.A
        self.units = [int(u) for u in units] if units else []
        if self.units and self.precision == "split":
            raise ValueError("precision='split' covers the news encoder without the optional per-token Dense stack "
                             "(newsencoder_units_per_layer); use precision='exact' with it")
        if self.units and self.units[-1] != E:
            raise ValueError(f"newsencoder_units_per_layer must end with head_num*head_dim = {E} (the news vector is dotted with "
                             f"the {E}-wide user vector, nrms.py:201), got {self.units}")
        shapes = {"n_Wqkv": (D, 3 * E)}
        if self.units:
            from ._mlp import MLPStack

            shapes.update(MLPStack.shapes("n_", E, self.units))
        shapes.update({"n_W": (E, A), "n_b": (A,), "n_q": (A,), "u_Wqkv": (E, 3 * E), "u_W": (E, A), "u_b": (A,), "u_q": (A,)})
        self.params = FlatParams(shapes, self.device)
        self._graphs = {}
        self.mlp = MLPStack(self.params, "n_", E, self.units, self.device, l2, on_realloc=lambda: self._graphs.clear()) if self.units else None
        self._init_weights(seed)
        self.deterministic = bool(deterministic)
        if self.train_embedding:
            self.table_grad = torch.zeros_like(self.table)
            self.table_m = torch.zeros_like(self.table)
            self.table_v = torch.zeros_like(self.table)
            if self.deterministic:
                self.table_acc = torch.zeros(self.table.shape, dtype=torch.int64, device=self.device)
        self._init_step_state(seed, learning_rate)
        self._bufs = {}
        self.oob_flag = torch.zeros(1, dtype=torch.int32, device=self.device)
        self.keep_table_grad = False
        self.range_flag = torch.zeros(1, dtype=torch.int32, device=self.device)
        self.loss_dev = torch.zeros(1, device=self.device)
        self.use_graph = False
        self.fuse_user_head = True
        self.fuse_eval_gather = True
        self.defer_finish = True
        self.atomic_table_grad = False
        self.graph_collectives = False
        self.overlap_collectives = True
        self.skip_collectives = False
        self._pending = []
        self.defer_flag_checks = False
        self.trace = None
        self.world = 1
        if process_group is not None or (torch.distributed.is_available() and torch.distributed.is_initialized()):
            self.world = torch.distributed.get_world_size(process_group)
        self.guard = None
        if self.world > 1:
            from ._dist import LockStepGuard

            self.guard = LockStepGuard(process_group)
        self.force_collectives = False
        self.adam_in_finish = True
        self._adam_done_in_finish = False

    @property
    def multi(self) -> bool:
        return self.world > 1 or self.force_collectives

    def _init_weights(self, seed):
        D, E, A = self.D, self.E, self.A
        s = (lambda: seed) if seed is not None else (lambda: None)
        pv = self.params.view
        with torch.no_grad():
            for pre, din in (("n", D), ("u", E)):
                w = np.concatenate([glorot_uniform_np((din, E), s()) for _ in range(3)], axis=1)
                pv(f"{pre}_Wqkv").copy_(torch.from_numpy(w))
                pv(f"{pre}_W").copy_(torch.from_numpy(glorot_uniform_np((E, A), s())))
                pv(f"{pre}_b").zero_()
                pv(f"{pre}_q").copy_(torch.from_numpy(glorot_uniform_np((A, 1), s())[:, 0]))
        if self.mlp is not None:
            self.mlp.init_weights((lambda k: None) if seed is None else (lambda k: int(seed) * 1000 + k), glorot_uniform_np)

    def weight_names(self):
        base = ["news.emb", "news.attn.WQ", "news.attn.WK", "news.attn.WV"]
        if self.mlp is not None:
            base += self.mlp.weight_names("news")
        return base + ["news.att.W", "news.att.b", "news.att.q", "user.attn.WQ", "user.attn.WK", "user.attn.WV", "user.att.W",
                       "user.att.b", "user.att.q"]

    def get_weights(self):
        E = self.E
        out = [self._full_table().cpu().numpy()]
        for pre in ("n", "u"):
            w = self.params.view(f"{pre}_Wqkv").cpu().numpy()
            out += [w[:, :E].copy(), w[:, E:2 * E].copy(), w[:, 2 * E:].copy()]
            if pre == "n" and self.mlp is not None:
                out += self.mlp.get_weights()
            out += [self.params.view(f"{pre}_W").cpu().numpy(), self.params.view(f"{pre}_b").cpu().numpy(),
                    self.params.view(f"{pre}_q").cpu().numpy().reshape(-1, 1)]
        return out

    def set_weights(self, weights):
        n_mlp = 6 * len(self.units)
        if len(weights) != 13 + n_mlp:
            raise ValueError(f"expected {13 + n_mlp} weight arrays (emb, 2x[WQ,WK,WV,W,b,q]{' + 6 per Dense/BN layer' if n_mlp else ''}), "
                             f"got {len(weights)}")
        w = [np.asarray(a, dtype=np.float32) for a in weights]
        if n_mlp:
            self.mlp.set_weights([torch.from_numpy(np.ascontiguousarray(a)) for a in w[4:4 + n_mlp]])
            w = w[:4] + w[4 + n_mlp:]
        if w[0].shape != (self.V, self.D):
            raise ValueError(f"embedding shape {w[0].shape} != {(self.V, self.D)}")
        with torch.no_grad():
            t0 = w[0] if self.exchange is None else self.exchange.shard_of(w[0])
            self.table.copy_(torch.from_numpy(np.ascontiguousarray(t0)))
            i = 1
            for pre in ("n", "u"):
                self.params.view(f"{pre}_Wqkv").copy_(torch.from_numpy(np.concatenate(w[i:i + 3], axis=1)))
                self.params.view(f"{pre}_W").copy_(torch.from_numpy(w[i + 3]))
                self.params.view(f"{pre}_b").copy_(torch.from_numpy(w[i + 4].reshape(-1)))
                self.params.view(f"{pre}_q").copy_(torch.from_numpy(w[i + 5].reshape(-1)))
                i += 6

    def _full_table(self) -> torch.Tensor:
        if self.exchange is None or self.exchange.world == 1:
            return self.table
# ... 505 lines not shown
        S = _hip.stream_handle
        nb, ub = self._train_bufs(B, C)
        st = _hip.ptr(self.state)
        site1, p1 = (1, self.p) if self.p > 0 else (-1, 0.0)
        deferred = self._deferred(C)
        if part in ("all", "a"):
            self._adam_done_in_finish = False
        if part == "b":
            if deferred:
                return self._news_bwd_deferred(nb, ub, B, N, "p2")
            return self._news_bwd_p2(nb, N, nb.X, nb.dNE, site1, p1)
        if part in ("all", "a"):
            if deferred:
                self._news_forward(nb, N, True, B * H, looked_up=True)
                self._user_stage_deferred(B, C, nb, ub)
            else:
                self._fwd_user_stage_kernels(B, C, nb, ub)
        if part == "a":
            if deferred:
                return self._news_bwd_deferred(nb, ub, B, N, "p1")
            return self._news_bwd_p1(nb, N, nb.dNE)
        if part == "all" and deferred:
            self._news_bwd_deferred(nb, ub, B, N, "p1")
            self._adam_done_in_finish = self._adam_fused(C)
            if self._adam_done_in_finish:
                self._news_bwd_deferred(nb, ub, B, N, "p2a")
                if nb.dX is not None:
                    self._news_bwd_p3(nb, N, nb.dX)
                self._news_bwd_deferred(nb, ub, B, N, "p2b")
            else:
                self._news_bwd_deferred(nb, ub, B, N, "p2")
                if nb.dX is not None:
                    self._news_bwd_p3(nb, N, nb.dX)
        elif part == "all":
            self._encoder_bwd("n", nb, N, nb.X, nb.dNE, nb.dX, B * H)
        elif nb.dX is not None:
            self._news_bwd_p3(nb, N, nb.dX)
        self._table_grad_kernels(nb, N, sparse_table_grads)

    def _deferred(self, C) -> bool:
        L = _hip.lib()
        return bool(self.defer_finish and self.mlp is None and self.precision == "exact" and self.fuse_user_head
                    and self._fold_pooling(self.T) and self._fold_pooling(self.H)
                    and int(L.ebn_user_head_supported(self.H, C, self.E, self.A)) != 0)

    def _adam_fused(self, C) -> bool:
        return bool(self.adam_in_finish and not self.multi and self._deferred(C))

    def _adam_flat_args(self):
        a = getattr(self, "_adam_flat", None)
        if a is None:
            P = self.params
            a = _hip.AdamFlat()
            a.theta, a.grad, a.m, a.v, a.numel = P.data.data_ptr(), P.grad.data_ptr(), P.m.data_ptr(), P.v.data_ptr(), P.numel
            a.beta1, a.beta2, a.eps, a.grad_scale = BETA1, BETA2, ADAM_EPS, 1.0
            rest = sorted((P.offsets[k], int(np.prod(P.shapes[k]))) for k in ("u_Wqkv", "u_W"))
            a.n_rest = len(rest)
            for i, (off, n) in enumerate(rest):
                a.rest_off[i], a.rest_len[i] = off, n
            self._adam_flat = a
        return a

    def _defer_bufs(self, nb):
        if getattr(nb, "ws_dw", None) is None:
            L = _hip.lib()
            nb.ws_dw = torch.empty(max(int(L.ebn_gemm_partials_workspace_floats(self.E, self.A, nb.R)), 1), device=self.device)
            nb.ws_dwqkv = torch.empty(max(int(L.ebn_gemm_partials_workspace_floats(self.D, 3 * self.E, nb.R)), 1), device=self.device)
            nb.finish_jobs = {}
        return nb

    def _user_stage_deferred(self, B, C, nb, ub):
        S, H, E, A = _hip.stream_handle, self.H, self.E, self.A
        R = B * H
        pv, g = self.params.view, self.params.g
        ws, wsn = _hip.ptr(ub.ws), ub.ws.numel()
        one, zero = ctypes.c_float(1.0), ctypes.c_float(0.0)
        X, cand, dcand = nb.out, nb.out[B * H:], nb.dNE[B * H:]
        _hip.call("ebn_gemm_f32_site", 0, 0, R, 3 * E, E, one, _hip.ptr(X), E, _hip.ptr(pv("u_Wqkv")), 3 * E, zero, _hip.ptr(ub.QKV), 3 * E, ws, wsn, 1, S())
        _hip.call("ebn_attn_fwd_f32", _hip.ptr(ub.QKV), 3 * E, _hip.ptr(ub.Y), E, B, H, self.h, self.d, None, -1, zero, S())
        _hip.call("ebn_gemm_f32_ws", 0, 0, R, A, E, one, _hip.ptr(ub.Y), E, _hip.ptr(pv("u_W")), A, zero, _hip.ptr(ub.U), A, ws, wsn, S())
        _hip.call("ebn_user_head_train_f32", _hip.ptr(ub.U), _hip.ptr(pv("u_b")), _hip.ptr(pv("u_q")), _hip.ptr(ub.Y), _hip.ptr(cand), _hip.ptr(nb.labels),
                  _hip.ptr(ub.w), _hip.ptr(ub.out), _hip.ptr(nb.scores), _hip.ptr(nb.probs), _hip.ptr(ub.loss_rows), _hip.ptr(self.loss_dev), _hip.ptr(dcand),
                  _hip.ptr(ub.duser), _hip.ptr(ub.de), None, None, _hip.ptr(ub.head_partials), B, H, C, E, A, self.loss_kind, ctypes.c_float(1.0 / B), S())
        _hip.call("ebn_dense_bwd_pair_f32", R, E, A, _hip.ptr(ub.Y), E, _hip.ptr(ub.U), A, _hip.ptr(pv("u_W")), A, zero, _hip.ptr(g("u_W")), A,
                  _hip.ptr(ub.dY), E, ws, wsn, S())
        _hip.call("ebn_attn_bwd_pooled_f32", _hip.ptr(ub.QKV), 3 * E, _hip.ptr(ub.dY), E, _hip.ptr(ub.w), _hip.ptr(ub.duser), E, _hip.ptr(ub.dQKV), 3 * E,
                  B, H, self.h, self.d, None, -1, zero, S())
        _hip.call("ebn_dense_bwd_pair_f32", R, E, 3 * E, _hip.ptr(X), E, _hip.ptr(ub.dQKV), 3 * E, _hip.ptr(pv("u_Wqkv")), 3 * E, zero, _hip.ptr(g("u_Wqkv")),
                  3 * E, _hip.ptr(nb.dNE), E, ws, wsn, S())

    def _news_bwd_deferred(self, nb, ub, B, N, part):
        S, E, A, T, D = _hip.stream_handle, self.E, self.A, self.T, self.D
        R = N * T
        pv, g = self.params.view, self.params.g
        one, zero = ctypes.c_float(1.0), ctypes.c_float(0.0)
        L = _hip.lib()
        self._defer_bufs(nb)
        if part == "p1":
            _hip.call("ebn_attpool_bwd_pool_f32", _hip.ptr(nb.Y), _hip.ptr(nb.w), _hip.ptr(nb.dNE), None, _hip.ptr(nb.de), N, T, E, S())
            _hip.call("ebn_attpool_bwd_dpre_f32", _hip.ptr(nb.U), _hip.ptr(pv("n_q")), _hip.ptr(nb.de), None, None, _hip.ptr(nb.partials), R, A, 0, S())
            n = ctypes.c_int32(0)
            _hip.call("ebn_gemm_f32_partials", 1, 0, E, A, R, one, _hip.ptr(nb.Y), E, _hip.ptr(nb.U), A, _hip.ptr(nb.ws_dw), nb.ws_dw.numel(), ctypes.byref(n), S())
            nb.finish_jobs["dW"] = int(n.value)
            _hip.call("ebn_gemm_f32_ws", 0, 1, R, E, A, one, _hip.ptr(nb.U), A, _hip.ptr(pv("n_W")), A, zero, _hip.ptr(nb.dY), E, _hip.ptr(nb.ws), nb.ws.numel(), S())
            return
        site, p = (1, self.p) if self.p > 0 else (-1, 0.0)
        if part in ("p2", "p2a"):
            _hip.call("ebn_attn_bwd_pooled_f32", _hip.ptr(nb.QKV), 3 * E, _hip.ptr(nb.dY), E, _hip.ptr(nb.w), _hip.ptr(nb.dNE), E, _hip.ptr(nb.dQKV), 3 * E,
                      N, T, self.h, self.d, _hip.ptr(self.state), site, ctypes.c_float(p), S())
            n = ctypes.c_int32(0)
            _hip.call("ebn_gemm_f32_partials", 1, 0, D, 3 * E, R, one, _hip.ptr(nb.X), D, _hip.ptr(nb.dQKV), 3 * E, _hip.ptr(nb.ws_dwqkv), nb.ws_dwqkv.numel(),
                      ctypes.byref(n), S())
            nb.finish_jobs["dWqkv"] = int(n.value)
            if part == "p2a":
                return
        jobs = (_hip.FinishJob * 4)()
        jobs[0] = _hip.FinishJob(_hip.FINISH_COLRED, int(L.ebn_attpool_partials_len(R, A)) // (2 * A), 1, A, nb.partials.data_ptr(), g("n_q").data_ptr(),
                                 g("n_b").data_ptr(), A, 0.0, 1.0, None, None)
        jobs[1] = _hip.FinishJob(_hip.FINISH_HEAD, 1, B, A, ub.head_partials.data_ptr(), g("u_q").data_ptr(), g("u_b").data_ptr(), A, 0.0, 1.0,
                                 ub.loss_rows.data_ptr(), self.loss_dev.data_ptr())
        jobs[2] = _hip.FinishJob(_hip.FINISH_SPLITK, nb.finish_jobs["dW"], E, A, nb.ws_dw.data_ptr(), g("n_W").data_ptr(), None, A, 0.0, 1.0, None, None)
        jobs[3] = _hip.FinishJob(_hip.FINISH_SPLITK, nb.finish_jobs["dWqkv"], D, 3 * E, nb.ws_dwqkv.data_ptr(), g("n_Wqkv").data_ptr(), None, 3 * E, 0.0, 1.0, None, None)
        if part == "p2b":
            _hip.call("ebn_grad_finish_adam_f32", jobs, 4, ctypes.byref(self._adam_flat_args()), _hip.ptr(self.state), S())
        else:
            _hip.call("ebn_grad_finish_f32", jobs, 4, S())

    def _fwd_user_stage_kernels(self, B, C, nb, ub):
        H, E = self.H, self.E
        N = B * (H + C)
        S = _hip.stream_handle
        st = _hip.ptr(self.state)
        self._news_forward(nb, N, True, B * H, looked_up=True)
        cand, dcand = nb.out[B * H:], nb.dNE[B * H:]
        dims, params, acts = self._enc_structs("u", ub, B, nb.out, -1, 0.0)
        g = self.params.g
        grads = _hip.EncoderGrads(g("u_Wqkv").data_ptr(), g("u_W").data_ptr(), g("u_b").data_ptr(), g("u_q").data_ptr())
        scratch = _hip.EncoderScratch(ub.dY.data_ptr(), ub.dQKV.data_ptr(), ub.de.data_ptr(), ub.partials.data_ptr(),
                                      ub.ws.data_ptr(), ub.ws.numel())
        _hip.call("ebn_user_stage_train_f32", ctypes.byref(dims), ctypes.byref(params), ctypes.byref(acts), _hip.ptr(cand),
                  _hip.ptr(nb.labels), _hip.ptr(nb.scores), _hip.ptr(nb.probs), _hip.ptr(ub.loss_rows), _hip.ptr(self.loss_dev),
                  _hip.ptr(dcand), _hip.ptr(ub.duser), ctypes.byref(grads), ctypes.byref(scratch),
                  _hip.ptr(ub.head_partials) if self.fuse_user_head else None, _hip.ptr(nb.dNE), C, self.loss_kind,
                  ctypes.c_float(1.0 / B), st, S())

    def _accumulate_fixed(self, ids, dX, n_tok, st, site, p):
        _hip.call("ebn_embedding_grad_scatter_fixed_atomic" if self.atomic_table_grad else "ebn_embedding_grad_scatter_fixed", _hip.ptr(ids),
                  _hip.ptr(dX), _hip.ptr(self.table_acc), n_tok, self.D, self.V, st, site, ctypes.c_float(p), _hip.ptr(self.range_flag),
                  _hip.stream_handle())

    def _table_grad_kernels(self, nb, N, sparse_table_grads):
        S = _hip.stream_handle
        st = _hip.ptr(self.state)
        if self.train_embedding and not self._planned and not sparse_table_grads:
            if self.exchange is not None or not self.deterministic:
                self.table_grad.zero_()
            site, p = (0, self.p) if self.p > 0 else (-1, 0.0)
            if self.exchange is not None:
                d_uniq = torch.zeros_like(nb.rows_uniq)
                _hip.call("ebn_embedding_grad_scatter_f32", _hip.ptr(nb.plan.inv), _hip.ptr(nb.dX), _hip.ptr(d_uniq),
                          N * self.T, self.D, d_uniq.shape[0], st, site, ctypes.c_float(p), S())
                self.exchange.scatter_grads(nb.plan, d_uniq, self._local_scatter_add)
            elif self.deterministic:
                self._accumulate_fixed(nb.ids, nb.dX, N * self.T, st, site, p)
                if not self._adam_from_acc:
                    _hip.call("ebn_fixed_to_f32", _hip.ptr(self.table_acc), _hip.ptr(self.table_grad), self.table.numel(),
                              _hip.ptr(self.range_flag), S())
            else:
                _hip.call("ebn_embedding_grad_scatter_f32", _hip.ptr(nb.ids), _hip.ptr(nb.dX), _hip.ptr(self.table_grad),
                          N * self.T, self.D, self.V, st, site, ctypes.c_float(p), S())

    def _optimizer_kernels(self, from_acc=None):
        from_acc = self._adam_from_acc if from_acc is None else from_acc
        S = _hip.stream_handle
        st = _hip.ptr(self.state)
        gs = ctypes.c_float(1.0 / self.world)
        P = self.params
        if not self._adam_done_in_finish:
            _hip.call("ebn_adam_keras_step_f32", _hip.ptr(P.data), _hip.ptr(P.grad), _hip.ptr(P.m), _hip.ptr(P.v), P.numel,
                      st, BETA1, BETA2, ADAM_EPS, gs, S())
        if self.train_embedding and from_acc:
            _hip.call("ebn_adam_keras_step_fixed_f32", _hip.ptr(self.table), _hip.ptr(self.table_acc), _hip.ptr(self.table_m),
                      _hip.ptr(self.table_v), self.table.numel(), st, BETA1, BETA2, ADAM_EPS, gs, _hip.ptr(self.range_flag), S())
        elif self.train_embedding:
            _hip.call("ebn_adam_keras_step_f32", _hip.ptr(self.table), _hip.ptr(self.table_grad), _hip.ptr(self.table_m),
                      _hip.ptr(self.table_v), self.table.numel(), st, BETA1, BETA2, ADAM_EPS, gs, S())
```

ebnerd-benchmark_amd/ebrec/models/newsrec/_engine_docvec.py:

```python
from __future__ import annotations

import ctypes

import numpy as np
import torch

from ebrec import _hip

from ._engine import ADAM_EPS, BETA1, BETA2, LOSS_KIND, loss_kind_of, EncoderBuffers, FlatParams, glorot_uniform_np, require_gpu
from ._engine_base import StepStateOwner, pair_score_tail, score_loss_tail
from ._mlp import MLPStack


class DocVecEngine(StepStateOwner):
    def __init__(self, doc_dim: int, units, history_size: int, head_num: int, head_dim: int, attention_hidden_dim: int,
                 dropout: float, learning_rate: float, loss: str, l2: float, seed=None, device=None, process_group=None,
                 bce_on: str = "logits"):
        self.device = require_gpu() if device is None else torch.device(device)
        if loss not in LOSS_KIND:
            raise ValueError(f"this loss not defined {loss}")
        loss_kind_of(loss, bce_on)
        self.bce_on = bce_on
        self.Din, self.units, self.H = int(doc_dim), [int(u) for u in (units or [])], int(history_size)
        self.h, self.d, self.A = int(head_num), int(head_dim), int(attention_hidden_dim)
        self.E = self.h * self.d
        self.p, self.loss, self.l2, self.seed, self.pg = float(dropout), loss, float(l2), seed, process_group
        E, A = self.E, self.A
        shapes = MLPStack.shapes("", self.Din, self.units)
        prev = self.units[-1] if self.units else self.Din
        shapes.update({"out_W": (prev, E), "out_b": (E,), "u_Wqkv": (E, 3 * E), "u_W": (E, A), "u_b": (A,), "u_q": (A,)})
        self.params = FlatParams(shapes, self.device)
        self.use_graph, self._graphs = False, {}
        self.fuse_user_head = True
        self.fuse_news_mlp = True
        self.fuse_finale = True
        self._dvn_dirty = False
        self.mlp = MLPStack(self.params, "", self.Din, self.units, self.device, self.l2, on_realloc=lambda: self._graphs.clear())
        self.bn_mean, self.bn_var = self.mlp.bn_mean, self.mlp.bn_var
        self._init_weights(seed)
        self._init_step_state(seed, learning_rate)
        self._bufs = {}
        self.loss_dev = torch.zeros(1, device=self.device)
        self.reg_dev = torch.zeros(1, device=self.device)
        self.range_flag = torch.zeros(1, dtype=torch.int32, device=self.device)
        self.world = 1
        if process_group is not None or (torch.distributed.is_available() and torch.distributed.is_initialized()):
            self.world = torch.distributed.get_world_size(process_group)
        self.guard = None
        if self.world > 1:
            from ._dist import LockStepGuard

            self.guard = LockStepGuard(process_group)
        self.force_collectives = False

    @property
    def multi(self) -> bool:
        return self.world > 1 or self.force_collectives

    def _init_weights(self, seed):
        rng_seed = (lambda k: None) if seed is None else (lambda k: int(seed) * 1000 + k)
        pv = self.params.view
        self.mlp.init_weights(rng_seed, glorot_uniform_np)
        with torch.no_grad():
            prev = self.mlp.out_dim
            pv("out_W").copy_(torch.from_numpy(glorot_uniform_np((prev, self.E), rng_seed(99))))
            s = (lambda: seed) if seed is not None else (lambda: None)
            pv("u_Wqkv").copy_(torch.from_numpy(np.concatenate([glorot_uniform_np((self.E, self.E), s()) for _ in range(3)], 1)))
            pv("u_W").copy_(torch.from_numpy(glorot_uniform_np((self.E, self.A), s())))
            pv("u_q").copy_(torch.from_numpy(glorot_uniform_np((self.A, 1), s())[:, 0]))

    def weight_names(self):
        return self.mlp.weight_names("news") + ["news.out.kernel", "news.out.bias", "user.attn.WQ", "user.attn.WK",
                                                 "user.attn.WV", "user.att.W", "user.att.b", "user.att.q"]

    def get_weights(self):
        pv, E = self.params.view, self.E
        w = pv("u_Wqkv").cpu().numpy()
        return self.mlp.get_weights() + [pv("out_W").cpu().numpy(), pv("out_b").cpu().numpy(), w[:, :E].copy(), w[:, E:2 * E].copy(),
                                         w[:, 2 * E:].copy(), pv("u_W").cpu().numpy(), pv("u_b").cpu().numpy(),
                                         pv("u_q").cpu().numpy().reshape(-1, 1)]

    def set_weights(self, weights):
        n = 6 * len(self.units) + 8
        if len(weights) != n:
            raise ValueError(f"expected {n} weight arrays, got {len(weights)}")
        w = [torch.from_numpy(np.ascontiguousarray(np.asarray(a, dtype=np.float32))) for a in weights]
        pv = self.params.view
        self.mlp.set_weights(w)
        i = 6 * len(self.units)
        with torch.no_grad():
            pv("out_W").copy_(w[i]); pv("out_b").copy_(w[i + 1])
            pv("u_Wqkv").copy_(torch.cat(w[i + 2:i + 5], dim=1))
            pv("u_W").copy_(w[i + 5]); pv("u_b").copy_(w[i + 6].reshape(-1)); pv("u_q").copy_(w[i + 7].reshape(-1))

    def count_params(self):
        return sum(int(np.prod(s)) for s in self.params.shapes.values()) + 2 * sum(self.units)

    def _mlp_bufs(self, N):
        b = self._bufs.get("mlp")
        if b is None or b["N"] < N:
            f = lambda *s: torch.empty(*s, device=self.device)
            b = {"N": N, "X0": f(N, self.Din), "NE": f(N, self.E), "dNE": f(N, self.E), "dXl": f(N, self.mlp.out_dim),
                 "scores": f(N), "probs": f(N), "labels": f(N)}
            b["partials"] = f(int(_hip.lib().ebn_colsum_partials_len(N, self.E)))
            wsf = _hip.lib().ebn_gemm_workspace_floats
            b["ws"] = f(max(int(wsf(self.mlp.out_dim, self.E, N)), int(wsf(N, self.E, self.mlp.out_dim)), int(wsf(N, self.mlp.out_dim, self.E)), 1))
            self.mlp.bufs(N)
            self._bufs["mlp"] = b
            self._graphs.clear()
        return b

    def _user_bufs(self, B, H=None):
        H = self.H if H is None else int(H)
        key = "user" if H == self.H else ("user", H)
        b = self._bufs.get(key)
        if b is None or b.n_seq < B:
# ... 210 lines not shown
    def pair_scores(self, user, news, u_idx, n_idx, sigmoid=True):
        return pair_score_tail(user, news, u_idx, n_idx, self.E, sigmoid)

    def enable_graphs(self, flag=True):
        self.use_graph = bool(flag)
        if not flag:
            self._graphs = {}
        return self

    def set_article_matrix(self, matrix) -> None:
        m = np.asarray(matrix)
        if m.ndim != 2 or m.shape[1] != self.Din or not np.issubdtype(m.dtype, np.floating):
            raise ValueError(f"article matrix must be float (n_articles+1, {self.Din}), got {m.dtype} {m.shape}")
        self.article_matrix = torch.from_numpy(np.ascontiguousarray(m.astype(np.float32))).to(self.device)
        self._article_matrix_src = matrix
        self._oob = torch.zeros(1, dtype=torch.int32, device=self.device)

    def _stage_indexed(self, mb, his_idx, pred_idx, y=None):
        n = his_idx.shape[0] * (self.H + pred_idx.shape[1])
        if "art_idx" not in mb:
            mb["art_idx"] = torch.empty(mb["N"], dtype=torch.int32, device=self.device)
        same_dev = lambda t: t.is_cuda and (self.device.index is None or t.device.index == self.device.index)
        ok = lambda t, dt: isinstance(t, torch.Tensor) and same_dev(t) and t.dtype == dt and t.is_contiguous()
        if ok(his_idx, torch.int32) and ok(pred_idx, torch.int32) and ok(y, torch.float32):
            _hip.call("ebn_docvec_stage_gather_f32", _hip.ptr(his_idx), his_idx.numel(), _hip.ptr(pred_idx), pred_idx.numel(), _hip.ptr(y),
                      _hip.ptr(mb["labels"]), y.numel(), _hip.ptr(self.article_matrix), self.article_matrix.shape[0], self.Din,
                      _hip.ptr(mb["X0"]), _hip.ptr(self._oob), _hip.ptr(self.state), BETA1, BETA2, _hip.stream_handle())
            self._advanced = True
            return None
        elif not isinstance(his_idx, torch.Tensor) and not isinstance(pred_idx, torch.Tensor) and y is not None and not isinstance(y, torch.Tensor):
            B, C = his_idx.shape[0], pred_idx.shape[1]
            n_lab, tot = B * C, n + B * C
            st = getattr(self, "_host_stage", None)
            if st is None or st["pinned"][0].numel() < tot:
                st = self._host_stage = {"pinned": [torch.empty(2 * tot, dtype=torch.int32).pin_memory() for _ in range(2)],
                                         "dev": torch.empty(2 * tot, dtype=torch.int32, device=self.device), "ev": [None, None], "k": 0}
            k = st["k"] = st["k"] ^ 1
            if st["ev"][k] is not None:
                st["ev"][k].synchronize()
            hs = st["pinned"][k].numpy()
            nh = B * self.H
            hs[:nh] = np.asarray(his_idx).reshape(-1)
            hs[nh:n] = np.asarray(pred_idx).reshape(-1)
            hs[n:tot].view(np.float32)[:] = np.asarray(y, dtype=np.float32).reshape(-1)
            st["dev"][:tot].copy_(st["pinned"][k][:tot], non_blocking=True)
            st["ev"][k] = torch.cuda.Event()
            st["ev"][k].record()
            _hip.call("ebn_docvec_stage_gather_f32", _hip.ptr(st["dev"]), n, None, 0, _hip.ptr(st["dev"][n:]), _hip.ptr(mb["labels"]), n_lab,
                      _hip.ptr(self.article_matrix), self.article_matrix.shape[0], self.Din, _hip.ptr(mb["X0"]), _hip.ptr(self._oob),
                      _hip.ptr(self.state), BETA1, BETA2, _hip.stream_handle())
            self._advanced = True
            return None
        else:
            off = 0
            for a in (his_idx, pred_idx):
                t = a if isinstance(a, torch.Tensor) else torch.from_numpy(np.ascontiguousarray(np.asarray(a).reshape(-1).astype(np.int32, copy=False)))
                t = t.reshape(-1)
                mb["art_idx"][off: off + t.numel()].copy_(t.to(device=self.device, dtype=torch.int32), non_blocking=True)
                off += t.numel()
        _hip.call("ebn_gather_rows_f32", _hip.ptr(mb["art_idx"]), _hip.ptr(self.article_matrix), _hip.ptr(mb["X0"]), n, self.Din,
                  self.article_matrix.shape[0], None, -1, ctypes.c_float(0.0), _hip.ptr(self._oob), _hip.stream_handle())
        return y

    def train_step(self, his, pred, y, return_probs=False, indexed=False):
        his = his if isinstance(his, torch.Tensor) else np.asarray(his)
        pred = pred if isinstance(pred, torch.Tensor) else np.asarray(pred)
        if not indexed:
            self._check_shapes(his, pred)
        elif his.ndim != 2 or his.shape[1] != self.H or pred.ndim != 2 or pred.shape[0] != his.shape[0]:
            raise ValueError(f"indexed batches must be (B, {self.H}) and (B, C), got {tuple(his.shape)} {tuple(pred.shape)}")
        B, C = his.shape[0], pred.shape[1]
        mb, ub = self._mlp_bufs(B * (self.H + C)), self._user_bufs(B)
        self._dvn(mb, B * self.H, B * C)
        self._advanced = False
        if indexed:
            y = self._stage_indexed(mb, his, pred, y)
        else:
            self._upload(mb, his, pred)
        if y is not None:
            labels = (y if isinstance(y, torch.Tensor) else torch.from_numpy(np.ascontiguousarray(np.asarray(y, dtype=np.float32))))
            mb["labels"][: B * C].copy_(labels.reshape(-1).to(device=self.device, dtype=torch.float32))
        if self.use_graph:
            adv = self._advanced
            gkey = (B, C, adv, bool(self.fuse_news_mlp), self.p, self.l2, bool(self.fuse_finale), bool(self.multi))
            g = self._graphs.get(gkey)
            if g is None:
                torch.cuda.synchronize()
                g1, g2 = torch.cuda.CUDAGraph(), torch.cuda.CUDAGraph()
                with _hip.capture(g1):
                    self._fwd_bwd_kernels(B, C, adv)
                if self._step_applied_adam(mb):
                    g2 = None
                else:
                    with _hip.capture(g2, pool=g1.pool()):
                        self._optimizer_kernels()
                g = self._graphs[gkey] = (g1, g2)
            g[0].replay()
            if g[1] is not None:
                self._allreduce_grads()
                g[1].replay()
        else:
            self._fwd_bwd_kernels(B, C, self._advanced)
            if not self._step_applied_adam(mb):
                self._allreduce_grads()
                self._optimizer_kernels()
        if return_probs:
            return self.loss_dev, mb["probs"][: B * C].view(B, C), mb["labels"][: B * C].view(B, C)
        return self.loss_dev

    @staticmethod
    def _step_applied_adam(mb) -> bool:
        a = mb.get("dvn_live")
        return a is not None and a._finale is not None

    def _fwd_bwd_kernels(self, B, C, advanced=False):
        E = self.E
        S = _hip.stream_handle
        mb, ub = self._mlp_bufs(B * (self.H + C)), self._user_bufs(B)
        n_hist, n_cand = B * self.H, B * C
        st = _hip.ptr(self.state)
        if not advanced:
            _hip.call("ebn_step_advance", st, BETA1, BETA2, S())
        self._news_forward(mb, n_hist, n_cand, True)
        a = mb.get("dvn_live")
        if a is not None and a._finale is not None:
            self._user_stage_deferred(B, C, mb, ub)
            self._news_backward(mb, n_hist, n_cand)
            return
        dims, params, acts = self._enc(ub, B, mb["NE"])
        cand = mb["NE"][n_hist:]
        g = self.params.g
        grads = _hip.EncoderGrads(g("u_Wqkv").data_ptr(), g("u_W").data_ptr(), g("u_b").data_ptr(), g("u_q").data_ptr())
        scratch = _hip.EncoderScratch(ub.dY.data_ptr(), ub.dQKV.data_ptr(), ub.de.data_ptr(), ub.partials.data_ptr(),
                                      ub.ws.data_ptr(), ub.ws.numel())
        _hip.call("ebn_user_stage_train_f32", ctypes.byref(dims), ctypes.byref(params), ctypes.byref(acts), _hip.ptr(cand),
                  _hip.ptr(mb["labels"]), _hip.ptr(mb["scores"]), _hip.ptr(mb["probs"]), _hip.ptr(ub.loss_rows), _hip.ptr(self.loss_dev),
                  _hip.ptr(mb["dNE"][n_hist:]), _hip.ptr(ub.duser), ctypes.byref(grads), ctypes.byref(scratch),
                  _hip.ptr(ub.head_partials) if self.fuse_user_head else None, _hip.ptr(mb["dNE"]), C, self.loss_kind,
                  ctypes.c_float(1.0 / B), st, S())
        self._news_backward(mb, n_hist, n_cand)

    def _user_stage_deferred(self, B, C, mb, ub):
        S, H, E, A = _hip.stream_handle, self.H, self.E, self.A
        R = B * H
        pv, g = self.params.view, self.params.g
        ws, wsn = _hip.ptr(ub.ws), ub.ws.numel()
        one, zero = ctypes.c_float(1.0), ctypes.c_float(0.0)
        X, cand, dcand = mb["NE"], mb["NE"][R:], mb["dNE"][R:]
        _hip.call("ebn_gemm_f32_site", 0, 0, R, 3 * E, E, one, _hip.ptr(X), E, _hip.ptr(pv("u_Wqkv")), 3 * E, zero, _hip.ptr(ub.QKV), 3 * E, ws, wsn, 1, S())
        _hip.call("ebn_attn_fwd_f32", _hip.ptr(ub.QKV), 3 * E, _hip.ptr(ub.Y), E, B, H, self.h, self.d, None, -1, zero, S())
        _hip.call("ebn_gemm_f32_ws", 0, 0, R, A, E, one, _hip.ptr(ub.Y), E, _hip.ptr(pv("u_W")), A, zero, _hip.ptr(ub.U), A, ws, wsn, S())
        _hip.call("ebn_user_head_train_f32", _hip.ptr(ub.U), _hip.ptr(pv("u_b")), _hip.ptr(pv("u_q")), _hip.ptr(ub.Y), _hip.ptr(cand), _hip.ptr(mb["labels"]),
                  _hip.ptr(ub.w), _hip.ptr(ub.out), _hip.ptr(mb["scores"]), _hip.ptr(mb["probs"]), _hip.ptr(ub.loss_rows), _hip.ptr(self.loss_dev), _hip.ptr(dcand),
                  _hip.ptr(ub.duser), _hip.ptr(ub.de), None, None, _hip.ptr(ub.head_partials), B, H, C, E, A, self.loss_kind, ctypes.c_float(1.0 / B), S())
        _hip.call("ebn_dense_bwd_pair_f32", R, E, A, _hip.ptr(ub.Y), E, _hip.ptr(ub.U), A, _hip.ptr(pv("u_W")), A, zero, _hip.ptr(g("u_W")), A,
                  _hip.ptr(ub.dY), E, ws, wsn, S())
        _hip.call("ebn_attn_bwd_pooled_f32", _hip.ptr(ub.QKV), 3 * E, _hip.ptr(ub.dY), E, _hip.ptr(ub.w), _hip.ptr(ub.duser), E, _hip.ptr(ub.dQKV), 3 * E,
                  B, H, self.h, self.d, None, -1, zero, S())
        _hip.call("ebn_dense_bwd_pair_f32", R, E, 3 * E, _hip.ptr(X), E, _hip.ptr(ub.dQKV), 3 * E, _hip.ptr(pv("u_Wqkv")), 3 * E, zero, _hip.ptr(g("u_Wqkv")),
                  3 * E, _hip.ptr(mb["dNE"]), E, ws, wsn, S())

    def _allreduce_grads(self):
        if self.multi:
            torch.distributed.all_reduce(self.params.grad, group=self.pg)

    def _optimizer_kernels(self):
        S = _hip.stream_handle
        st = _hip.ptr(self.state)
        P = self.params
        _hip.call("ebn_adam_keras_step_f32", _hip.ptr(P.data), _hip.ptr(P.grad), _hip.ptr(P.m), _hip.ptr(P.v), P.numel, st,
                  BETA1, BETA2, ADAM_EPS, ctypes.c_float(1.0 / self.world), S())

    def roofline_kernels(self, B, C):
        mb = self._mlp_bufs(B * (self.H + C))
        n = B * (self.H + C)
        S = _hip.stream_handle

        def make_gather(rows):
            def gather():
                _hip.call("ebn_gather_rows_f32", _hip.ptr(rows), _hip.ptr(self.article_matrix), _hip.ptr(mb["X0"]), n, self.Din,
                          self.article_matrix.shape[0], None, -1, ctypes.c_float(0.0), _hip.ptr(self._oob), S())

            return gather

        out = {"gather": make_gather}
        a = self._dvn(mb, B * self.H, B * C)
        if a is not None:
            out["dw_group_flops"] = float(sum(2.0 * q.M * q.N * q.K for q in a._probs))
            out["dw_group_bytes"] = float(sum(4.0 * (q.K * (q.M + q.N) + q.M * q.N) for q in a._probs))
            if a._finale is not None:
                P, f = self.params, _hip.DvnFinale()
                ctypes.memmove(ctypes.byref(f), ctypes.byref(a._finale), ctypes.sizeof(f))
                shadow = mb.setdefault("finale_shadow", [P.data.clone(), P.m.clone(), P.v.clone()])
                f.theta, f.m, f.v = (t.data_ptr() for t in shadow)
                ub = self._user_bufs(B)
                f.head_partials, f.loss_rows, f.B = ub.head_partials.data_ptr(), ub.loss_rows.data_ptr(), B
                out["dw_group"] = lambda: _hip.call("ebn_dvn_finale_f32", ctypes.byref(a), a._probs, len(a._probs), ctypes.byref(f), _hip.ptr(self.state), S())
                out["dw_group_bytes"] += 4.0 * 7 * P.numel
                out["dw_group_is_finale"] = True
            else:
                out["dw_group"] = lambda: _hip.call("ebn_gemm_tn_group_f32", a._probs, len(a._probs), S())
        return out

    def check_oob(self):
        oob = getattr(self, "_oob", None)
        flags = torch.cat([oob if oob is not None else torch.zeros(1, dtype=torch.int32, device=self.device), self.range_flag])
        if self.world > 1:
            torch.distributed.all_reduce(flags, op=torch.distributed.ReduceOp.MAX, group=self.pg)
        bad_rows, bad_range = (int(v) != 0 for v in flags.cpu().tolist())
        if bad_rows and oob is not None:
            oob.zero_()
        if bad_range:
            self.range_flag.zero_()
            self._dvn_dirty = True
        if bad_rows:
            raise IndexError(f"article row out of range [0, {self.article_matrix.shape[0]}) for the document-vector matrix")
        if bad_range:
            raise FloatingPointError("a column sum of the news encoder's BatchNormalization left the range of its fixed-point accumulator or was not "
                                     "finite: the run has diverged (fuse_news_mlp=False runs the separate passes, which propagate NaN instead)")

    def sync_moving_statistics(self) -> None:
        if self.world > 1:
            self.mlp.sync_moving_statistics(self.pg)

    def l2_penalty(self) -> float:
        return self.mlp.l2_penalty()

    def extra_state(self):
        return {}
```

ebnerd-benchmark_amd/ebrec/models/newsrec/_engine_segments.py:

```python
from __future__ import annotations

import ctypes

import numpy as np
import torch

from ebrec import _hip

BETA1, BETA2, ADAM_EPS = 0.9, 0.999, 1e-7


def _named(kind, fn, what):
    fn.what = what
    return kind, fn


class SegmentsMixin:
    def _lookup_segments(self, b, N):
        ex, n_tok = self.exchange, N * self.T

        def plan(ids, n, cap, ws, slot_rows, inv, counts):
            _hip.call("ebn_shard_plan_i32", _hip.ptr(ids), n, self.V, ex.world, 1 if ex.cyclic else 0, cap, _hip.ptr(ws),
                      _hip.ptr(slot_rows), _hip.ptr(inv), _hip.ptr(counts), _hip.stream_handle())

        def serve(local_rows, out):
            _hip.call("ebn_gather_rows_f32", _hip.ptr(local_rows), _hip.ptr(self.table), _hip.ptr(out), local_rows.numel(), self.D,
                      self.table.shape[0], None, -1, ctypes.c_float(0.0), None, _hip.stream_handle())

        return ex.lookup_segments(b.ids, n_tok, b.xb, plan, serve)

    def _table_grad_segments(self, b, N):
        ex, n_tok = self.exchange, N * self.T
        site, p = (0, self.p) if self.p > 0 else (-1, 0.0)

        def reduce_local(inv, d_slot):
            d_slot.zero_()
            _hip.call("ebn_embedding_grad_scatter_f32", _hip.ptr(inv), _hip.ptr(b.dX), _hip.ptr(d_slot), n_tok, self.D,
                      d_slot.shape[0], _hip.ptr(self.state), site, ctypes.c_float(p), _hip.stream_handle())

        def accumulate(local_rows, grads):
            self.table_grad.zero_()
            _hip.call("ebn_embedding_grad_scatter_f32", _hip.ptr(local_rows), _hip.ptr(grads), _hip.ptr(self.table_grad),
                      local_rows.numel(), self.D, self.table.shape[0], None, -1, ctypes.c_float(0.0), _hip.stream_handle())

        return ex.grad_segments(n_tok, b.xb, reduce_local, accumulate)

    def _local_gather(self, local_rows: torch.Tensor) -> torch.Tensor:
        m = local_rows.numel()
        out = torch.empty(m, self.D, device=self.device)
        if m:
            _hip.call("ebn_gather_rows_f32", _hip.ptr(local_rows), _hip.ptr(self.table), _hip.ptr(out), m, self.D,
                      self.table.shape[0], None, -1, ctypes.c_float(0.0), _hip.ptr(self.oob_flag), _hip.stream_handle())
        return out

    def _local_scatter_add(self, local_rows: torch.Tensor, grads: torch.Tensor) -> None:
        m = local_rows.numel()
        if m:
            _hip.call("ebn_embedding_grad_scatter_f32", _hip.ptr(local_rows), _hip.ptr(grads), _hip.ptr(self.table_grad),
                      m, self.D, self.table.shape[0], None, -1, ctypes.c_float(0.0), _hip.stream_handle())

    def _state_tensors(self):
        ts = [self.params.data, self.params.grad, self.params.m, self.params.v, self.state, self.loss_dev]
        if self.train_embedding:
            ts += [self.table, self.table_grad, self.table_m, self.table_v] + ([self.table_acc] if self.deterministic else [])
        return ts

    def verify_graph_collectives(self, his, pred, y) -> bool:
        if not (self.use_graph and self.graph_capable and self.multi):
            self.graph_collectives = False
            return False
        if torch.distributed.get_backend(self.pg) != "nccl":
            self.graph_collectives = False
            return False
        torch.cuda.synchronize()
        snap = [t.clone() for t in self._state_tensors()]

        def restore():
            for t, s in zip(self._state_tensors(), snap):
                t.copy_(s)

        def one_step(flag):
            self.graph_collectives = flag
            self._graphs.clear()
            self.train_step(his, pred, y)
            restore()
            self.train_step(his, pred, y)
            torch.cuda.synchronize()
            out = [t.clone() for t in self._state_tensors()]
            restore()
            return out

        ok = True
        try:
            ref = one_step(False)
            got = one_step(True)
            ok = all(torch.equal(a, b) for a, b in zip(ref, got))
        except Exception:
            ok = False
            restore()
        verdict = torch.tensor([1 if ok else 0], dtype=torch.int32, device=self.device)
        torch.distributed.all_reduce(verdict, op=torch.distributed.ReduceOp.MIN, group=self.pg)
        self.graph_collectives = bool(int(verdict.item()))
        self._graphs.clear()
        return self.graph_collectives

    def _graph_key(self, B, C, advanced=False):
        return (B, C, advanced, bool(self.adam_in_finish), bool(self.defer_finish), bool(self.multi))

    def _capture(self, B, C, advanced=False):
        torch.cuda.synchronize()
        key = self._graph_key(B, C, advanced)
        segs, run, pool, i = self._segments(B, C, advanced), [], None, 0
        desc = self.__dict__.setdefault("_graph_desc", {}).setdefault(key, [])
        desc.clear()
        if self.graph_collectives and self.multi:
            g = torch.cuda.CUDAGraph()
            with _hip.capture(g):
                for _kind, fn in segs:
                    fn()
            self._graph_objs = getattr(self, "_graph_objs", []) + [g]
            self._graphs[key] = [g.replay]
            desc.append("ONE hipGraph: " + " | ".join(self.SEG_KINDS[k] for k, _fn in segs))
            return self._graphs[key]
        while i < len(segs):
            if segs[i][0] != "k":
                run.append(segs[i][1])
                desc.append(f"{self.SEG_KINDS[segs[i][0]]}: {getattr(segs[i][1], 'what', 'unnamed')} (segment {i} of the step's {len(segs)})")
                i += 1
                continue
            j = i
            while j < len(segs) and segs[j][0] == "k":
                j += 1
            g = torch.cuda.CUDAGraph()
            with _hip.capture(g, pool=pool):
                for _kind, fn in segs[i:j]:
                    fn()
            pool = pool or g.pool()
            run.append(g.replay)
            desc.append(f"hipGraph replay of kernel segments {i}..{j - 1} of the step's {len(segs)}")
            self._graph_objs = getattr(self, "_graph_objs", []) + [g]
            i = j
        self._graphs[key] = run
        return run

    def _segments(self, B, C, advanced=False):
        N = B * (self.H + C)
        nb, _ub = self._train_bufs(B, C)
        multi = self.multi
        segs = [] if advanced else [("k", lambda: _hip.call("ebn_step_advance", _hip.ptr(self.state), BETA1, BETA2, _hip.stream_handle()))]
        if self._planned:
            segs += self._lookup_segments(nb, N)
        sparse = self._sparse_dp(N * self.T)
        if multi and self.mlp is None and self.overlap_collectives and self.train_embedding:
            segs.append(("k", lambda: (self._fwd_bwd_kernels(B, C, sparse, part="a"), self._fwd_bwd_kernels(B, C, sparse, part="b"))))
            segs.append(_named("a", lambda: self._allreduce_async(self.params.grad), "all-reduce of the flat dense-gradient bucket"))
            segs.append(("k", lambda: self._fwd_bwd_kernels(B, C, sparse, part="c")))
            if self._planned:
                segs += self._table_grad_segments(nb, N)
            if self.exchange is None and not sparse:
                segs.append(_named("c", lambda: self._allreduce_table_grad(), "all-reduce of the dense (V, D) table gradient"))
            if sparse:
                segs += self._sparse_table_grad_segments(nb, N)
            segs.append(("w", self._wait_collectives))
        else:
            segs.append(("k", lambda: self._fwd_bwd_kernels(B, C, sparse)))
            if self._planned and self.train_embedding:
                segs += self._table_grad_segments(nb, N)
            if multi:
                segs.append(_named("c", lambda: self._allreduce_grads(dense_table=not sparse),
                                   "all-reduce of the flat dense-gradient bucket" + (" and of the dense table gradient" if (self.train_embedding and self.exchange is None and not sparse) else "")))
            if sparse:
                segs += self._sparse_table_grad_segments(nb, N)
        segs.append(("k", lambda: self._optimizer_kernels(from_acc=self._adam_from_acc or sparse)))
        return segs

    def _allreduce_async(self, t):
        if self.multi and not self.skip_collectives:
            self._pending.append(torch.distributed.all_reduce(t, group=self.pg, async_op=True))

    def _wait_collectives(self):
        for w in self._pending:
            w.wait()
        self._pending = []

    def _allreduce_table_grad(self):
        if self.multi and not self.skip_collectives:
            torch.distributed.all_reduce(self.table_grad, group=self.pg)

    def _sparse_table_grad_segments(self, nb, N):
        n_tok, W = N * self.T, self.world
# ... 25 lines not shown
```

include/ebnerd_hip.h:

```cpp
#ifndef EBNERD_HIP_H
#define EBNERD_HIP_H

#include <stdint.h>

#ifdef __cplusplus
extern "C" {
#endif

#define EBN_ABI_VERSION 1

#define EBN_OK 0
#define EBN_ERR_BAD_ARG (-1)
#define EBN_ERR_UNSUPPORTED (-2)
#define EBN_ERR_ALIGN (-3)

typedef void* ebn_stream_t;

#define EBN_SITE_NEWS_IN 0
#define EBN_SITE_NEWS_ATT 1
#define EBN_SITE_MLP0 8
#define EBN_N_SITES 12

typedef struct ebn_step_state {
  uint32_t step;
// ... 39 lines not shown
                       int64_t workspace_bytes, ebn_stream_t stream);
int64_t ebn_planes_bytes(int64_t rows, int64_t K);
int ebn_split_planes_f32(const float* src, int64_t ld, int64_t rows, int64_t K, int32_t trans, void* planes,
                         ebn_stream_t stream);
int ebn_gather_split_planes_f32(const int32_t* ids, const float* table, int64_t n_rows, int32_t D, int64_t V,
                                const ebn_step_state* st, int32_t site, float drop_p, int32_t* oob_flag, void* planes_n,
                                void* planes_t, ebn_stream_t stream);
int64_t ebn_gemm_planes_workspace_floats(int64_t M, int64_t N, int64_t K);
int ebn_gemm_planes_f32(const void* a_planes, int64_t M, const void* b_planes, int64_t N, int64_t K, float alpha, float beta,
                        float* C, int64_t ldc, float* workspace, int64_t workspace_floats, ebn_stream_t stream);
int64_t ebn_gemm_prec_workspace_bytes(int64_t M, int64_t N, int64_t K, int32_t precision);
int ebn_gemm_f32_prec(int32_t transA, int32_t transB, int64_t M, int64_t N, int64_t K, float alpha, const float* A,
                      int64_t lda, const float* B, int64_t ldb, float beta, float* C, int64_t ldc, void* workspace,
                      int64_t workspace_bytes, int32_t precision, ebn_stream_t stream);

int64_t ebn_shard_plan_workspace_ints(int64_t V, int32_t world);
int ebn_shard_plan_i32(const int32_t* ids, int64_t n_tok, int64_t V, int32_t world, int32_t cyclic, int64_t cap,
                       int32_t* workspace, int32_t* slot_rows, int32_t* inv, int32_t* counts, ebn_stream_t stream);

int ebn_gemm_f32(int32_t transA, int32_t transB, int64_t M, int64_t N, int64_t K, float alpha,
                 const float* A, int64_t lda, const float* B, int64_t ldb, float beta, float* C,
                 int64_t ldc, ebn_stream_t stream);
int64_t ebn_gemm_workspace_floats(int64_t M, int64_t N, int64_t K);
int ebn_gemm_plan(int64_t M, int64_t N, int64_t K, int64_t workspace_floats, int32_t* bm, int32_t* bn, int32_t* splits);
int ebn_gemm_f32_ws(int32_t transA, int32_t transB, int64_t M, int64_t N, int64_t K, float alpha,
                    const float* A, int64_t lda, const float* B, int64_t ldb, float beta, float* C,
                    int64_t ldc, float* workspace, int64_t workspace_floats, ebn_stream_t stream);

int64_t ebn_gemm_partials_workspace_floats(int64_t M, int64_t N, int64_t K);
int ebn_gemm_f32_partials(int32_t transA, int32_t transB, int64_t M, int64_t N, int64_t K, float alpha, const float* A,
                          int64_t lda, const float* B, int64_t ldb, float* workspace, int64_t workspace_floats,
                          int32_t* n_parts, ebn_stream_t stream);

#define EBN_FINISH_SPLITK 0
#define EBN_FINISH_COLRED 1
#define EBN_FINISH_HEAD 2
#define EBN_FINISH_MAX_JOBS 6
typedef struct {
  int32_t kind;
  int32_t n_parts;
  int64_t rows, cols;
  const float* partials;
  float* out0;
  float* out1;
  int64_t ld;
  float beta, scale;
  const float* loss_rows;
  float* loss_out;
} ebn_finish_job;
int ebn_grad_finish_f32(const ebn_finish_job* jobs, int32_t n_jobs, ebn_stream_t stream);

#define EBN_ADAM_FLAT_MAX_REST 12
typedef struct ebn_adam_flat {
  float* theta;
  const float* grad;
  float* m;
  float* v;
  int64_t numel;
  double beta1, beta2, eps;
  float grad_scale;
  int32_t n_rest;
  int64_t rest_off[EBN_ADAM_FLAT_MAX_REST];
  int64_t rest_len[EBN_ADAM_FLAT_MAX_REST];
} ebn_adam_flat;
int ebn_grad_finish_adam_f32(const ebn_finish_job* jobs, int32_t n_jobs, const ebn_adam_flat* adam, const ebn_step_state* st,
                             ebn_stream_t stream);

int ebn_gemm_f32_site(int32_t transA, int32_t transB, int64_t M, int64_t N, int64_t K, float alpha,
                      const float* A, int64_t lda, const float* B, int64_t ldb, float beta, float* C,
                      int64_t ldc, float* workspace, int64_t workspace_floats, int32_t site,
                      ebn_stream_t stream);

int ebn_attn_fwd_f32(const float* qkv, int64_t ld_qkv, float* out, int64_t ld_out, int64_t n_seq,
                     int32_t L, int32_t h, int32_t d, const ebn_step_state* st, int32_t site,
                     float drop_p, ebn_stream_t stream);
int ebn_attn_bwd_f32(const float* qkv, int64_t ld_qkv, const float* dout, int64_t ld_dout,
                     float* dqkv, int64_t ld_dqkv, int64_t n_seq, int32_t L, int32_t h, int32_t d,
                     const ebn_step_state* st, int32_t site, float drop_p, ebn_stream_t stream);
int ebn_attn_bwd_pooled_f32(const float* qkv, int64_t ld_qkv, const float* dout, int64_t ld_dout, const float* pool_w,
                            const float* pool_dout, int64_t ld_pool, float* dqkv, int64_t ld_dqkv, int64_t n_seq,
                            int32_t L, int32_t h, int32_t d, const ebn_step_state* st, int32_t site, float drop_p,
                            ebn_stream_t stream);
int ebn_attn_bwd_pooled_supported(int32_t L, int32_t d);

int ebn_gemm_f32_rank1(int64_t M, int64_t N, int64_t K, float alpha, const float* A, int64_t lda, const float* B,
                       int64_t ldb, float* C, int64_t ldc, const float* row_scale, const float* seq_rows,
                       int64_t ld_seq, int32_t L, float* workspace, int64_t workspace_floats, ebn_stream_t stream);

int ebn_dense_bwd_pair_f32(int64_t R, int64_t K_in, int64_t N_out, const float* X, int64_t ldx, const float* dY,
                           int64_t lddy, const float* W, int64_t ldw, float beta_w, float* dW, int64_t lddw, float* dX,
                           int64_t lddx, float* workspace, int64_t workspace_floats, ebn_stream_t stream);

int ebn_dense_relu_fwd_f32(int64_t M, int64_t N, int64_t K, const float* A, int64_t lda, const float* B, int64_t ldb,
                           const float* bias, float* C, int64_t ldc, float* workspace, int64_t workspace_floats,
                           ebn_stream_t stream);

int ebn_attpool_fwd_f32(float* U, const float* b, const float* q, const float* X, float* out,
                        float* w, int64_t n_seq, int32_t L, int32_t E, int32_t A,
                        ebn_stream_t stream);
int ebn_attpool_bwd_pool_f32(const float* X, const float* w, const float* dout, float* dX,
                             float* de, int64_t n_seq, int32_t L, int32_t E,
                             ebn_stream_t stream);
int64_t ebn_attpool_partials_len(int64_t R, int32_t A);
int ebn_attpool_bwd_dpre_f32(float* U, const float* q, const float* de, float* dq, float* db,
                             float* partials, int64_t R, int32_t A, int32_t accumulate,
                             ebn_stream_t stream);
typedef struct ebn_encoder_dims {
  int64_t n_seq;
  int32_t L;
  int32_t Din;
  int32_t h, d;
  int32_t A;
  int32_t drop_site;
  float drop_p;
} ebn_encoder_dims;

typedef struct ebn_encoder_params {
  const float* Wqkv;
  const float* W;
  const float* b;
  const float* q;
} ebn_encoder_params;

typedef struct ebn_encoder_acts {
  const float* X;
  float* QKV;
  float* Y;
  float* U;
  float* w;
  float* out;
} ebn_encoder_acts;

typedef struct ebn_encoder_grads {
  float* dWqkv;
  float* dW;
  float* db;
  float* dq;
} ebn_encoder_grads;

typedef struct ebn_encoder_scratch {
  float* dY;
  float* dQKV;
  float* de;
  float* partials;
  float* gemm_ws;
  int64_t gemm_ws_floats;
} ebn_encoder_scratch;

int ebn_encoder_fwd_f32(const ebn_encoder_dims* dims, const ebn_encoder_params* params,
                        const ebn_encoder_acts* acts, const ebn_encoder_scratch* scratch,
                        const ebn_step_state* st, ebn_stream_t stream);
int ebn_encoder_fwd_gather_f32(const ebn_encoder_dims* dims, const ebn_encoder_params* params, const ebn_encoder_acts* acts,
                               const ebn_encoder_scratch* scratch, const int32_t* ids, const float* table, int64_t table_rows,
                               int32_t* oob_flag, ebn_stream_t stream);
int ebn_gemm_f32_rowmap(const int32_t* ids, int64_t table_rows, int64_t M, int64_t N, int64_t K, const float* table,
                        int64_t ldt, const float* B, int64_t ldb, float* C, int64_t ldc, int32_t* oob_flag, ebn_stream_t stream);

int ebn_encoder_bwd_f32(const ebn_encoder_dims* dims, const ebn_encoder_params* params,
                        const ebn_encoder_acts* acts, const float* dout,
                        const ebn_encoder_grads* grads, const ebn_encoder_scratch* scratch,
                        float* dX, int32_t accumulate, const ebn_step_state* st,
                        ebn_stream_t stream);

int ebn_user_stage_train_f32(const ebn_encoder_dims* dims, const ebn_encoder_params* p, const ebn_encoder_acts* a,
                             const float* cand, const float* labels, float* scores, float* probs, float* loss_rows,
                             float* loss_out, float* dcand, float* duser, const ebn_encoder_grads* g,
                             const ebn_encoder_scratch* s, float* head_partials, float* dX, int32_t C, int32_t loss_kind,
                             float inv_batch, const ebn_step_state* st, ebn_stream_t stream);

int ebn_score_fwd_f32(const float* cand, const float* user, float* scores, float* probs,
                      int64_t B, int32_t C, int32_t E, int32_t mode, ebn_stream_t stream);
int ebn_score_loss_bwd_f32(const float* cand, const float* user, const float* scores,
                           const float* labels, float* loss_rows, float* dcand, float* duser,
                           int64_t B, int32_t C, int32_t E, int32_t loss_kind, float inv_batch,
                           ebn_stream_t stream);
int ebn_score_loss_train_f32(const float* cand, const float* user, const float* labels, float* scores, float* probs,
                             float* loss_rows, float* loss_out, float* dcand, float* duser, int64_t B, int32_t C,
                             int32_t E, int32_t loss_kind, float inv_batch, ebn_stream_t stream);
int ebn_user_head_supported(int32_t L, int32_t C, int32_t E, int32_t A);
int64_t ebn_user_head_partials_len(int64_t B, int32_t A);
int ebn_user_head_train_f32(float* U, const float* b, const float* q, const float* X, const float* cand, const float* labels,
                            float* w, float* user, float* scores, float* probs, float* loss_rows, float* loss_out,
                            float* dcand, float* duser, float* de, float* dq, float* db, float* partials, int64_t B,
                            int32_t L, int32_t C, int32_t E, int32_t A, int32_t loss_kind, float inv_batch,
                            ebn_stream_t stream);
int ebn_auc_hist_f32(const float* probs, const float* labels, int64_t n, const double* thresholds, int32_t n_thresholds,
                     int64_t* pos_hist, int64_t* neg_hist, ebn_stream_t stream);
int ebn_pair_score_f32(const float* user, const float* news, const int32_t* u_idx,
                       const int32_t* n_idx, float* out, int64_t n_pairs, int32_t E, int32_t mode,
                       ebn_stream_t stream);

int ebn_adam_keras_step_f32(float* theta, const float* g, float* m, float* v, int64_t n,
                            const ebn_step_state* st, double beta1, double beta2, double eps,
                            float grad_scale, ebn_stream_t stream);

int ebn_bias_relu_f32(const float* X, const float* bias, float* Y, int64_t R, int32_t Ccols,
                      ebn_stream_t stream);
int64_t ebn_colsum_partials_len(int64_t R, int32_t Ccols);
int ebn_bias_relu_bwd_f32(const float* Y, const float* dY, float* dX, float* dbias,
                          float* partials, int64_t R, int32_t Ccols, int32_t accumulate,
                          ebn_stream_t stream);
int ebn_batchnorm_fwd_f32(const float* X, const float* gamma, const float* beta,
                          float* moving_mean, float* moving_var, float* Y, float* xhat,
                          float* mean_out, float* istd_out, float* partials, int64_t R,
                          int32_t Ccols, int32_t training, const ebn_step_state* st,
                          int32_t site, float drop_p, int64_t elem_offset,
                          ebn_stream_t stream);
int ebn_batchnorm_bwd_f32(const float* dY, const float* xhat, const float* gamma,
                          const float* istd, float* dX, float* dgamma, float* dbeta,
                          float* partials, int64_t R, int32_t Ccols, int32_t training,
                          int32_t accumulate, const ebn_step_state* st, int32_t site,
                          float drop_p, int64_t elem_offset, ebn_stream_t stream);
int ebn_batchnorm2_fwd_f32(const float* X, const float* gamma, const float* beta, float* moving_mean, float* moving_var,
                           float* Y, float* xhat, float* mean_out0, float* istd_out0, float* mean_out1, float* istd_out1,
                           int64_t R0, int64_t R1, int32_t Ccols, const ebn_step_state* st, int32_t site, float drop_p,
                           ebn_stream_t stream);
int ebn_batchnorm2_relu_bwd_f32(const float* dY, const float* xhat, const float* relu_out, const float* gamma,
                                const float* istd0, const float* istd1, float* dX, float* dgamma, float* dbeta,
                                float* dbias, int64_t R0, int64_t R1, int32_t Ccols, const ebn_step_state* st, int32_t site,
                                float drop_p, ebn_stream_t stream);

#define EBN_DVN_MAX_LAYERS 4
typedef struct ebn_dvn_args {
  int32_t n_layers, din, e_out;
  int32_t units[EBN_DVN_MAX_LAYERS];
  int32_t n0, n1;
  float drop_p, l2;
  const float* W[EBN_DVN_MAX_LAYERS + 1];
  const float* b[EBN_DVN_MAX_LAYERS + 1];
  const float* gamma[EBN_DVN_MAX_LAYERS];
  const float* beta[EBN_DVN_MAX_LAYERS];
  float* moving_mean[EBN_DVN_MAX_LAYERS];
  float* moving_var[EBN_DVN_MAX_LAYERS];
  const float* X0;
  float* R[EBN_DVN_MAX_LAYERS];
  float* Xn[EBN_DVN_MAX_LAYERS];
  float* NE;
  float* stat;
  const float* dNE;
  float* dY[EBN_DVN_MAX_LAYERS];
  float* dP[EBN_DVN_MAX_LAYERS + 1];
  float* ggamma[EBN_DVN_MAX_LAYERS];
  float* gbeta[EBN_DVN_MAX_LAYERS];
  float* loss;
  int32_t* range_flag;
} ebn_dvn_args;
int ebn_dvn_supported(const ebn_dvn_args* args);
int64_t ebn_dvn_stat_floats(const ebn_dvn_args* args);
int ebn_dvn_fwd_train_f32(const ebn_dvn_args* args, const ebn_step_state* st, ebn_stream_t stream);
int ebn_dvn_bwd_f32(const ebn_dvn_args* args, const ebn_step_state* st, ebn_stream_t stream);

// ... 338 lines not shown
```

Measured before the change: 25480.

## Fuse user-stage dY projection into pooled attention backward kernel

The attention backward kernel gains a PROJ variant. It computes the gradient of the attention output directly inside the kernel as dpre·Wᵀ plus the pooling term, using MFMA with double-buffered loads, and writes it to LDS. This removes the separate dY GEMM and its round trip through global memory. The dW projection gradient is then computed with a new paired TN dense-backward call alongside the Wqkv backward. The cost is recomputing the projection per head tile inside the kernel, which raises register pressure. The fused path is enabled by default and falls back to the unfused path when shapes are unsupported.

```diff
diff --git a/ebnerd-benchmark_amd/csrc/ebn_attention.hip b/ebnerd-benchmark_amd/csrc/ebn_attention.hip
--- a/ebnerd-benchmark_amd/csrc/ebn_attention.hip
+++ b/ebnerd-benchmark_amd/csrc/ebn_attention.hip
@@ -5,6 +5,9 @@
 int ebn_attn_mfma_bwd(const float* qkv, int64_t ld_qkv, const float* dout, int64_t ld_dout, float* dqkv,
                       int64_t ld_dqkv, int64_t n_seq, int32_t L, int32_t h, int32_t d, const EbnDrop& dr,
                       hipStream_t s, bool* handled, const float* pool_w, const float* pool_d, int64_t ld_pool);
+int ebn_attn_mfma_bwd_proj(const float* qkv, int64_t ld_qkv, const float* dpre, int64_t ld_dpre, const float* W, int64_t ldw, int32_t A,
+                           const float* pool_w, const float* pool_d, int64_t ld_pool, float* dqkv, int64_t ld_dqkv, int64_t n_seq,
+                           int32_t L, int32_t h, int32_t d, hipStream_t s, bool* handled);
 
 namespace {
 
@@ -510,3 +513,23 @@
 extern "C" int ebn_attn_bwd_pooled_supported(int32_t L, int32_t d) {
   return (L > 0 && L <= 64 && (d == 16 || d == 20 || d == 32)) ? 1 : 0;
 }
+
+extern "C" int ebn_attn_bwd_pooled_proj_f32(const float* qkv, int64_t ld_qkv, const float* dpre, int64_t ld_dpre, const float* W,
+                                            int64_t ldw, int32_t A, const float* pool_w, const float* pool_dout, int64_t ld_pool,
+                                            float* dqkv, int64_t ld_dqkv, int64_t n_seq, int32_t L, int32_t h, int32_t d,
+                                            ebn_stream_t stream) {
+  int rc = check_attn_args(qkv, dqkv, n_seq, L, h, d);
+  if (rc != EBN_OK) return rc;
+  EBN_REQUIRE(dpre && W && pool_w && pool_dout && A > 0, EBN_ERR_BAD_ARG);
+  if (n_seq == 0) return EBN_OK;
+  EBN_REQUIRE(ld_qkv >= 3 * h * d && ld_dqkv >= 3 * h * d && ld_dpre >= A && ldw >= A && ld_pool >= h * d, EBN_ERR_BAD_ARG);
+  bool handled = false;
+  rc = ebn_attn_mfma_bwd_proj(qkv, ld_qkv, dpre, ld_dpre, W, ldw, A, pool_w, pool_dout, ld_pool, dqkv, ld_dqkv, n_seq, L, h, d,
+                              ebn_stream(stream), &handled);
+  if (rc != EBN_OK) return rc;
+  return handled ? EBN_OK : EBN_ERR_UNSUPPORTED;
+}
+
+extern "C" int ebn_user_stage_fused_supported(int32_t H, int32_t E, int32_t h, int32_t d, int32_t A) {
+  return (ebn_attn_bwd_pooled_supported(H, d) != 0 && h > 0 && static_cast<int64_t>(E) == static_cast<int64_t>(h) * d && (E % 4) == 0 && A > 0 && (A % 4) == 0) ? 1 : 0;
+}
diff --git a/ebnerd-benchmark_amd/csrc/ebn_attention_mfma.hip b/ebnerd-benchmark_amd/csrc/ebn_attention_mfma.hip
--- a/ebnerd-benchmark_amd/csrc/ebn_attention_mfma.hip
+++ b/ebnerd-benchmark_amd/csrc/ebn_attention_mfma.hip
@@ -24,6 +24,11 @@
   const float* pool_d;
   int64_t ld_pool;
   uint32_t stagger_units, stagger_shift, stagger_mod;
+  const float* proj_x;
+  int64_t ld_proj_x;
+  const float* proj_w;
+  int64_t ld_proj_w;
+  int32_t proj_k;
 };
 
 __device__ __forceinline__ int crow(int r, int hi) { return (r & 3) + 8 * (r >> 2) + 4 * hi; }
@@ -264,6 +269,115 @@
     t[4 * g + 1] = (8 * g + 4 * hi + 1 < L) ? v.y : 0.f;
     t[4 * g + 2] = (8 * g + 4 * hi + 2 < L) ? v.z : 0.f;
     t[4 * g + 3] = (8 * g + 4 * hi + 3 < L) ? v.w : 0.f;
+  }
+}
+
+constexpr int PJ = 5;
+
+template <int NB>
+struct ProjSet {
+  float4 x[NB][PJ], w[PJ];
+};
+
+template <int NB>
+__device__ __forceinline__ void proj_load(ProjSet<NB>& s, const float* __restrict__ xb, const uint32_t (&xo)[NB], const float* __restrict__ wb,
+                                          uint32_t wo) {
+#pragma unroll
+  for (int t = 0; t < PJ; ++t) {
+#pragma unroll
+    for (int n = 0; n < NB; ++n) s.x[n][t] = *reinterpret_cast<const float4*>((xb + 8 * t) + xo[n]);
+    s.w[t] = *reinterpret_cast<const float4*>((wb + 8 * t) + wo);
+  }
+}
+
+template <int NB>
+__device__ __forceinline__ void proj_mul4(f32x16 (&acc)[NB], const float4& w, const float4 (&x)[NB]) {
+#pragma unroll
+  for (int n = 0; n < NB; ++n) acc[n] = __builtin_amdgcn_mfma_f32_32x32x2f32(w.x, x[n].x, acc[n], 0, 0, 0);
+#pragma unroll
+  for (int n = 0; n < NB; ++n) acc[n] = __builtin_amdgcn_mfma_f32_32x32x2f32(w.y, x[n].y, acc[n], 0, 0, 0);
+#pragma unroll
+  for (int n = 0; n < NB; ++n) acc[n] = __builtin_amdgcn_mfma_f32_32x32x2f32(w.z, x[n].z, acc[n], 0, 0, 0);
+#pragma unroll
+  for (int n = 0; n < NB; ++n) acc[n] = __builtin_amdgcn_mfma_f32_32x32x2f32(w.w, x[n].w, acc[n], 0, 0, 0);
+}
+
+template <int NB>
+__device__ __forceinline__ void proj_mul(f32x16 (&acc)[NB], const ProjSet<NB>& s) {
+#pragma unroll
+  for (int t = 0; t < PJ; ++t) {
+    float4 x[NB];
+#pragma unroll
+    for (int n = 0; n < NB; ++n) x[n] = s.x[n][t];
+    proj_mul4<NB>(acc, s.w[t], x);
+  }
+}
+
+template <int NB>
+__device__ __forceinline__ void proj_tile(f32x16 (&acc)[NB], const float* __restrict__ xb, const uint32_t (&xo)[NB],
+                                          const float* __restrict__ wb, uint32_t wo, int K, int hi) {
+#pragma unroll
+  for (int n = 0; n < NB; ++n)
+#pragma unroll
+    for (int r = 0; r < 16; ++r) acc[n][r] = 0.f;
+  const int nq = K >> 2;
+  const int nch = (nq >> 1) / PJ;
+  if (nch > 0) {
+    ProjSet<NB> s0, s1;
+    proj_load<NB>(s0, xb, xo, wb, wo);
+    for (int c = 0; c + 1 < nch; c += 2) {
+      proj_load<NB>(s1, xb + 8 * PJ * (c + 1), xo, wb + 8 * PJ * (c + 1), wo);
+      __builtin_amdgcn_sched_barrier(0);
+      proj_mul<NB>(acc, s0);
+      const int c2 = c + 2 < nch ? c + 2 : nch - 1;
+      proj_load<NB>(s0, xb + 8 * PJ * c2, xo, wb + 8 * PJ * c2, wo);
+      __builtin_amdgcn_sched_barrier(0);
+      proj_mul<NB>(acc, s1);
+    }
+    if (nch & 1) proj_mul<NB>(acc, s0);
+  }
+  for (int b = nch * PJ; 2 * b < nq; ++b) {
+    float4 x[NB], w = make_float4(0.f, 0.f, 0.f, 0.f);
+#pragma unroll
+    for (int n = 0; n < NB; ++n) x[n] = w;
+    if (2 * b + hi < nq) {
+#pragma unroll
+      for (int n = 0; n < NB; ++n) x[n] = *reinterpret_cast<const float4*>((xb + 8 * b) + xo[n]);
+      w = *reinterpret_cast<const float4*>((wb + 8 * b) + wo);
+    }
+    proj_mul4<NB>(acc, w, x);
+  }
+}
+
+template <int D, int NB>
+__device__ __forceinline__ void proj_dout_to_lds(float* __restrict__ sg, const MfmaAttnArgs& a, int64_t xrow0, uint32_t seq, uint32_t head,
+                                                 int L, int row, int hi) {
+  const uint32_t cc = row < D ? row : 0;
+  uint32_t rc[NB], xo[NB];
+  float pw[NB];
+#pragma unroll
+  for (int n = 0; n < NB; ++n) {
+    rc[n] = 32 * n + (row < L - 32 * n ? row : 0);
+    pw[n] = a.pool_w[xrow0 + rc[n]];
+    xo[n] = rc[n] * static_cast<uint32_t>(a.ld_proj_x) + static_cast<uint32_t>(4 * hi);
+  }
+  const float* pd = a.pool_d + seq * a.ld_pool + head * D;
+  float4 pt[4];
+#pragma unroll
+  for (int g = 0; g < 4; ++g) pt[g] = *reinterpret_cast<const float4*>(pd + ((8 * g + 4 * hi < D) ? 8 * g + 4 * hi : 0));
+  f32x16 acc[NB];
+  proj_tile<NB>(acc, a.proj_x + xrow0 * a.ld_proj_x, xo, a.proj_w + static_cast<int64_t>(head) * D * a.ld_proj_w,
+                cc * static_cast<uint32_t>(a.ld_proj_w) + static_cast<uint32_t>(4 * hi), a.proj_k, hi);
+#pragma unroll
+  for (int n = 0; n < NB; ++n) {
+#pragma unroll
+    for (int g = 0; g < 4; ++g) {
+      acc[n][4 * g] = fmaf(pw[n], pt[g].x, acc[n][4 * g]);
+      acc[n][4 * g + 1] = fmaf(pw[n], pt[g].y, acc[n][4 * g + 1]);
+      acc[n][4 * g + 2] = fmaf(pw[n], pt[g].z, acc[n][4 * g + 2]);
+      acc[n][4 * g + 3] = fmaf(pw[n], pt[g].w, acc[n][4 * g + 3]);
+    }
+    tile_rows_to_lds<D>(sg + 32 * n * Tile<D>::STRIDE, acc[n], L - 32 * n, row, hi, 1.0f);
   }
 }
 
@@ -444,7 +558,7 @@
   return 3 * L * Tile<D>::STRIDE > L * Tile<D>::STRIDE + TP_FLOATS ? 3 * L * Tile<D>::STRIDE : L * Tile<D>::STRIDE + TP_FLOATS;
 }
 
-template <int D, int LC>
+template <int D, int LC, bool PROJ = false>
 __global__ __launch_bounds__(64 * ATT_WAVES) void attn_mfma_bwd_kernel(MfmaAttnArgs a) {
   using T = Tile<D>;
   constexpr int KH = D / 2;
@@ -471,16 +585,19 @@
     Staged<D> tq, tk, tg;
     stage_load<D>(tq, qb, a.ld_qkv, L, lane);
     stage_load<D>(tk, qb + E, a.ld_qkv, L, lane);
-    stage_load<D>(tg, a.dout + p.row0 * a.ld_dout + p.head * D, a.ld_dout, L, lane);
+    if constexpr (!PROJ) stage_load<D>(tg, a.dout + p.row0 * a.ld_dout + p.head * D, a.ld_dout, L, lane);
     global_row_form<D>(vr, qb + 2 * E, a.ld_qkv, L, row, hi);
-    if (pooled) {
-      PoolTerm<D> pt;
-      pool_load<D>(pt, a.pool_w + p.row0, a.pool_d + p.seq * a.ld_pool + p.head * D, L, lane);
-      pool_add<D>(tg, pt);
+    if constexpr (!PROJ) {
+      if (pooled) {
+        PoolTerm<D> pt;
+        pool_load<D>(pt, a.pool_w + p.row0, a.pool_d + p.seq * a.ld_pool + p.head * D, L, lane);
+        pool_add<D>(tg, pt);
+      }
     }
     stage_store<D, false>(sq, tq, L, lane, 0u, 0u, 0, 0u, 0.f);
     stage_store<D, false>(sk, tk, L, lane, 0u, 0u, 0, 0u, 0.f);
-    if (drop) stage_store<D, true>(sg, tg, L, lane, key, static_cast<uint64_t>(p.row0) * E + p.head * D, E, a.thresh, a.scale);
+    if constexpr (PROJ) proj_dout_to_lds<D, 1>(sg, a, p.row0, p.seq, p.head, L, row, hi);
+    else if (drop) stage_store<D, true>(sg, tg, L, lane, key, static_cast<uint64_t>(p.row0) * E + p.head * D, E, a.thresh, a.scale);
     else stage_store<D, false>(sg, tg, L, lane, 0u, 0u, 0, 0u, 0.f);
   }
   wave_lds_sync();
@@ -797,7 +914,7 @@
   }
 }
 
-template <int D, int LC>
+template <int D, int LC, bool PROJ = false>
 __global__ __launch_bounds__(64 * ATT2_WAVES) void attn_mfma2_bwd_kernel(MfmaAttnArgs a) {
   using T = Tile<D>;
   constexpr int KH = D / 2;
@@ -827,21 +944,26 @@
     stage_load<D>(tq, qb + 32 * b * a.ld_qkv, a.ld_qkv, Lb, lane);
     stage_load<D>(tk, qb + E + 32 * b * a.ld_qkv, a.ld_qkv, Lb, lane);
     stage_load<D>(tv, qb + 2 * E + 32 * b * a.ld_qkv, a.ld_qkv, Lb, lane);
-    stage_load<D>(tg, gb + 32 * b * a.ld_dout, a.ld_dout, Lb, lane);
-    if (a.pool_w != nullptr) {
-      PoolTerm<D> pt;
-      pool_load<D>(pt, a.pool_w + row0 + 32 * b, a.pool_d + seq * a.ld_pool + head * D, Lb, lane);
-      pool_add<D>(tg, pt);
+    if constexpr (!PROJ) {
+      stage_load<D>(tg, gb + 32 * b * a.ld_dout, a.ld_dout, Lb, lane);
+      if (a.pool_w != nullptr) {
+        PoolTerm<D> pt;
+        pool_load<D>(pt, a.pool_w + row0 + 32 * b, a.pool_d + seq * a.ld_pool + head * D, Lb, lane);
+        pool_add<D>(tg, pt);
+      }
     }
     stage_store<D, false>(sq + 32 * b * T::STRIDE, tq, Lb, lane, 0u, 0u, 0, 0u, 0.f);
     stage_store<D, false>(sk + 32 * b * T::STRIDE, tk, Lb, lane, 0u, 0u, 0, 0u, 0.f);
     stage_store<D, false>(sv + 32 * b * T::STRIDE, tv, Lb, lane, 0u, 0u, 0, 0u, 0.f);
-    if (a.key_ptr != nullptr)
-      stage_store<D, true>(sg + 32 * b * T::STRIDE, tg, Lb, lane, *a.key_ptr,
-                           static_cast<uint64_t>(row0 + 32 * b) * E + head * D, E, a.thresh, a.scale);
-    else
-      stage_store<D, false>(sg + 32 * b * T::STRIDE, tg, Lb, lane, 0u, 0u, 0, 0u, 0.f);
-  }
+    if constexpr (!PROJ) {
+      if (a.key_ptr != nullptr)
+        stage_store<D, true>(sg + 32 * b * T::STRIDE, tg, Lb, lane, *a.key_ptr,
+                             static_cast<uint64_t>(row0 + 32 * b) * E + head * D, E, a.thresh, a.scale);
+      else
+        stage_store<D, false>(sg + 32 * b * T::STRIDE, tg, Lb, lane, 0u, 0u, 0, 0u, 0.f);
+    }
+  }
+  if constexpr (PROJ) proj_dout_to_lds<D, NB2>(sg, a, row0, static_cast<uint32_t>(seq), static_cast<uint32_t>(head), L, row, hi);
   wave_lds_sync();
 
   float* ob = a.out + row0 * a.ld_out + head * D;
@@ -1076,3 +1198,38 @@
   EBN_CHECK_LAUNCH();
   return EBN_OK;
 }
+
+int ebn_attn_mfma_bwd_proj(const float* qkv, int64_t ld_qkv, const float* dpre, int64_t ld_dpre, const float* W, int64_t ldw, int32_t A,
+                           const float* pool_w, const float* pool_d, int64_t ld_pool, float* dqkv, int64_t ld_dqkv, int64_t n_seq,
+                           int32_t L, int32_t h, int32_t d, hipStream_t s, bool* handled) {
+  *handled = mfma_path_ok(L, d, ld_qkv, ld_dpre, ld_dqkv, qkv, dpre, dqkv) && n_seq * h < (int64_t{1} << 31) && A > 0 && (A % 4) == 0 &&
+             (ldw % 4) == 0 && ldw < (1 << 24) && ebn_aligned16(W) && (ld_pool % 4) == 0 && ebn_aligned16(pool_d);
+  if (!*handled) return EBN_OK;
+  MfmaAttnArgs a{qkv, ld_qkv, nullptr, 0, dqkv, ld_dqkv, n_seq * h, L, h, nullptr, 0u, 1.0f, pool_w, pool_d, ld_pool, 0u, 0u, 1u,
+                 dpre, ld_dpre, W, ldw, A};
+  if (L > 32) {
+    const dim3 grid(static_cast<unsigned>(ebn_ceil_div(a.n_prob, ATT2_WAVES))), block(64 * ATT2_WAVES);
+    if (d == 16) {
+      const size_t lds = static_cast<size_t>(ATT2_WAVES) * 4 * L * Tile<16>::STRIDE * sizeof(float);
+      allow_lds(attn_mfma2_bwd_kernel<16, 0, true>, lds);
+      EBN_LAUNCH((attn_mfma2_bwd_kernel<16, 0, true>), grid, block, lds, s, a);
+    } else if (d == 20) {
+      const size_t lds = static_cast<size_t>(ATT2_WAVES) * 4 * L * Tile<20>::STRIDE * sizeof(float);
+      allow_lds(attn_mfma2_bwd_kernel<20, 0, true>, lds);
+      EBN_LAUNCH((attn_mfma2_bwd_kernel<20, 0, true>), grid, block, lds, s, a);
+    } else {
+      const size_t lds = static_cast<size_t>(ATT2_WAVES) * 4 * L * Tile<32>::STRIDE * sizeof(float);
+      allow_lds(attn_mfma2_bwd_kernel<32, 0, true>, lds);
+      EBN_LAUNCH((attn_mfma2_bwd_kernel<32, 0, true>), grid, block, lds, s, a);
+    }
+    EBN_CHECK_LAUNCH();
+    return EBN_OK;
+  }
+  const size_t wb = static_cast<size_t>(ATT_WAVES) * sizeof(float);
+  if (d == 16) launch_waves(attn_mfma_bwd_kernel<16, 0, true>, wb * bwd_wave_floats<16>(L), a, s);
+  else if (d == 20 && L == 20) launch_waves(attn_mfma_bwd_kernel<20, 20, true>, wb * bwd_wave_floats<20>(L), a, s);
+  else if (d == 20) launch_waves(attn_mfma_bwd_kernel<20, 0, true>, wb * bwd_wave_floats<20>(L), a, s);
+  else launch_waves(attn_mfma_bwd_kernel<32, 0, true>, wb * bwd_wave_floats<32>(L), a, s);
+  EBN_CHECK_LAUNCH();
+  return EBN_OK;
+}
diff --git a/ebnerd-benchmark_amd/csrc/ebn_encoder.hip b/ebnerd-benchmark_amd/csrc/ebn_encoder.hip
--- a/ebnerd-benchmark_amd/csrc/ebn_encoder.hip
+++ b/ebnerd-benchmark_amd/csrc/ebn_encoder.hip
@@ -90,11 +90,11 @@
   return EBN_OK;
 }
 
-extern "C" int ebn_user_stage_train_f32(const ebn_encoder_dims* dims, const ebn_encoder_params* p, const ebn_encoder_acts* a,
-                                        const float* cand, const float* labels, float* scores, float* probs, float* loss_rows,
-                                        float* loss_out, float* dcand, float* duser, const ebn_encoder_grads* g,
-                                        const ebn_encoder_scratch* s, float* head_partials, float* dX, int32_t C,
-                                        int32_t loss_kind, float inv_batch, const ebn_step_state* st, ebn_stream_t stream) {
+static int user_stage_train(const ebn_encoder_dims* dims, const ebn_encoder_params* p, const ebn_encoder_acts* a, const float* cand,
+                            const float* labels, float* scores, float* probs, float* loss_rows, float* loss_out, float* dcand,
+                            float* duser, const ebn_encoder_grads* g, const ebn_encoder_scratch* s, float* head_partials, float* dX,
+                            int32_t C, int32_t loss_kind, float inv_batch, const ebn_step_state* st, ebn_stream_t stream,
+                            bool allow_proj) {
   EBN_TRY(check_dims(dims));
   EBN_REQUIRE(p && a && g && s && cand && labels && scores && probs && loss_rows && loss_out && dcand && duser && dX, EBN_ERR_BAD_ARG);
   EBN_REQUIRE(p->Wqkv && p->W && p->b && p->q && a->X && a->QKV && a->Y && a->U && a->w && a->out, EBN_ERR_BAD_ARG);
@@ -121,9 +121,35 @@
   EBN_TRY(ebn_gemm_f32_ws(0, 0, R, A, E, 1.0f, a->Y, E, p->W, A, 0.0f, a->U, A, ws, ws_n, stream));
   EBN_TRY(ebn_user_head_train_f32(a->U, p->b, p->q, a->Y, cand, labels, a->w, a->out, scores, probs, loss_rows, loss_out, dcand,
                                   duser, s->de, g->dq, g->db, head_partials, B, L, C, E, A, loss_kind, inv_batch, stream));
+  if (allow_proj && ebn_user_stage_fused_supported(L, E, dims->h, dims->d, A) != 0 && ebn_aligned16(p->W) && (dims->Din % 4) == 0 &&
+      ebn_aligned16(a->X) && ebn_aligned16(p->Wqkv)) {
+    EBN_TRY(ebn_attn_bwd_pooled_proj_f32(a->QKV, 3 * E, a->U, A, p->W, A, A, a->w, duser, E, s->dQKV, 3 * E, B, L, dims->h, dims->d,
+                                         stream));
+    return ebn_dense_bwd_pair_tn_f32(R, dims->Din, 3 * E, a->X, dims->Din, s->dQKV, 3 * E, p->Wqkv, 3 * E, g->dWqkv, 3 * E, dX, dims->Din,
+                                     E, A, a->Y, E, a->U, A, g->dW, A, ws, ws_n, stream);
+  }
   EBN_TRY(ebn_dense_bwd_pair_f32(R, E, A, a->Y, E, a->U, A, p->W, A, 0.0f, g->dW, A, s->dY, E, ws, ws_n, stream));
   EBN_TRY(ebn_attn_bwd_pooled_f32(a->QKV, 3 * E, s->dY, E, a->w, duser, E, s->dQKV, 3 * E, B, L, dims->h, dims->d, nullptr, -1, 0.0f,
                                   stream));
   return ebn_dense_bwd_pair_f32(R, dims->Din, 3 * E, a->X, dims->Din, s->dQKV, 3 * E, p->Wqkv, 3 * E, 0.0f, g->dWqkv, 3 * E, dX,
                                 dims->Din, ws, ws_n, stream);
 }
+
+extern "C" int ebn_user_stage_train_f32(const ebn_encoder_dims* dims, const ebn_encoder_params* p, const ebn_encoder_acts* a,
+                                        const float* cand, const float* labels, float* scores, float* probs, float* loss_rows,
+                                        float* loss_out, float* dcand, float* duser, const ebn_encoder_grads* g,
+                                        const ebn_encoder_scratch* s, float* head_partials, float* dX, int32_t C,
+                                        int32_t loss_kind, float inv_batch, const ebn_step_state* st, ebn_stream_t stream) {
+  return user_stage_train(dims, p, a, cand, labels, scores, probs, loss_rows, loss_out, dcand, duser, g, s, head_partials, dX, C,
+                          loss_kind, inv_batch, st, stream, true);
+}
+
+extern "C" int ebn_user_stage_train_unfused_f32(const ebn_encoder_dims* dims, const ebn_encoder_params* p, const ebn_encoder_acts* a,
+                                                const float* cand, const float* labels, float* scores, float* probs,
+                                                float* loss_rows, float* loss_out, float* dcand, float* duser,
+                                                const ebn_encoder_grads* g, const ebn_encoder_scratch* s, float* head_partials,
+                                                float* dX, int32_t C, int32_t loss_kind, float inv_batch, const ebn_step_state* st,
+                                                ebn_stream_t stream) {
+  return user_stage_train(dims, p, a, cand, labels, scores, probs, loss_rows, loss_out, dcand, duser, g, s, head_partials, dX, C,
+                          loss_kind, inv_batch, st, stream, false);
+}
diff --git a/ebnerd-benchmark_amd/csrc/ebn_gemm.hip b/ebnerd-benchmark_amd/csrc/ebn_gemm.hip
--- a/ebnerd-benchmark_amd/csrc/ebn_gemm.hip
+++ b/ebnerd-benchmark_amd/csrc/ebn_gemm.hip
@@ -904,6 +904,21 @@
                                     (b - p0.tiles) % p1.tiles_x, (b - p0.tiles) / p1.tiles_x);
 }
 
+__global__ __launch_bounds__(GEMM_THREADS) void gemm_small_triple_kernel(SmallProblem pn, SmallProblem p0, SmallProblem p1) {
+  const GemmEpi none{nullptr, nullptr, 0, 1, nullptr};
+  const int b = blockIdx.x;
+  if (b < pn.tiles) {
+    small_vec_body<false, true, 32>(pn.M, pn.N, pn.K, pn.alpha, pn.A, pn.lda, pn.B, pn.ldb, pn.beta, pn.C, pn.ldc, none,
+                                    b % pn.tiles_x, b / pn.tiles_x);
+  } else {
+    const bool first = b - pn.tiles < p0.tiles;
+    const SmallProblem& p = first ? p0 : p1;
+    const int t = b - pn.tiles - (first ? 0 : p0.tiles);
+    small_vec_body<true, false, 32>(p.M, p.N, p.K, p.alpha, p.A, p.lda, p.B, p.ldb, p.beta, p.C, p.ldc, none, t % p.tiles_x,
+                                    t / p.tiles_x);
+  }
+}
+
 struct SmallGroup {
   SmallProblem p[EBN_TN_GROUP_MAX];
   float* colsum[EBN_TN_GROUP_MAX];
@@ -1312,6 +1327,46 @@
   return gemm_dispatch(0, 1, R, K_in, N_out, 1.0f, dY, lddy, W, ldw, 0.0f, dX, lddx, workspace, workspace_floats, 0, none, s);
 }
 
+extern "C" int ebn_dense_bwd_pair_tn_f32(int64_t R, int64_t K_in, int64_t N_out, const float* X, int64_t ldx, const float* dY,
+                                         int64_t lddy, const float* W, int64_t ldw, float* dW, int64_t lddw, float* dX, int64_t lddx,
+                                         int64_t K2, int64_t N2, const float* X2, int64_t ldx2, const float* dY2, int64_t lddy2,
+                                         float* dW2, int64_t lddw2, float* workspace, int64_t workspace_floats, ebn_stream_t stream) {
+  EBN_REQUIRE(ebn_dim_ok(R, K_in, N_out) && ebn_dim_ok(K2, N2) && K_in > 0 && N_out > 0 && K2 > 0 && N2 > 0, EBN_ERR_BAD_ARG);
+  EBN_REQUIRE(X && dY && W && dW && dX && X2 && dY2 && dW2, EBN_ERR_BAD_ARG);
+  EBN_REQUIRE(ebn_dim_ok(ldx, lddy, ldw) && ebn_dim_ok(ldx2, lddy2), EBN_ERR_BAD_ARG);
+  EBN_REQUIRE(ldx >= K_in && lddy >= N_out && ldw >= N_out && lddw >= N_out && lddx >= K_in, EBN_ERR_BAD_ARG);
+  EBN_REQUIRE(ldx2 >= K2 && lddy2 >= N2 && lddw2 >= N2, EBN_ERR_BAD_ARG);
+  hipStream_t s = ebn_stream(stream);
+  const int64_t wsf = workspace ? workspace_floats : 0;
+  const bool aligned = (ldx % 4) == 0 && (lddy % 4) == 0 && (ldw % 4) == 0 && ebn_aligned16(X) && ebn_aligned16(dY) && ebn_aligned16(W) &&
+                       (K_in % 4) == 0 && (N_out % 4) == 0 && (ldx2 % 4) == 0 && (lddy2 % 4) == 0 && ebn_aligned16(X2) &&
+                       ebn_aligned16(dY2) && (K2 % 4) == 0 && (N2 % 4) == 0;
+  int64_t ld_max = ldx > lddy ? ldx : lddy;
+  ld_max = ld_max > ldx2 ? ld_max : ldx2;
+  ld_max = ld_max > lddy2 ? ld_max : lddy2;
+  const int64_t span = (R + SBK) * ld_max * 4 + 64 * (ld_max > ldw ? ld_max : ldw) * 4;
+  const bool small = R > 0 && gemm_plan(K_in, N_out, R, wsf).bm == 32 && gemm_plan(R, K_in, N_out, wsf).bm == 32 &&
+                     gemm_plan(K2, N2, R, wsf).bm == 32;
+  if (!(aligned && small && span < (int64_t{1} << 31))) {
+    const int rc = ebn_dense_bwd_pair_f32(R, K_in, N_out, X, ldx, dY, lddy, W, ldw, 0.0f, dW, lddw, dX, lddx, workspace, workspace_floats, stream);
+    if (rc != EBN_OK) return rc;
+    return ebn_gemm_f32_ws(1, 0, K2, N2, R, 1.0f, X2, ldx2, dY2, lddy2, 0.0f, dW2, lddw2, workspace, workspace_floats, stream);
+  }
+  SmallProblem pn{R, K_in, N_out, 1.0f, dY, lddy, W, ldw, 0.0f, dX, lddx, static_cast<int32_t>(ebn_ceil_div(K_in, SBN)), 0};
+  pn.tiles = pn.tiles_x * static_cast<int32_t>(ebn_ceil_div(R, SBM));
+  SmallProblem p0{K_in, N_out, R, 1.0f, X, ldx, dY, lddy, 0.0f, dW, lddw, static_cast<int32_t>(ebn_ceil_div(N_out, SBN)), 0};
+  p0.tiles = p0.tiles_x * static_cast<int32_t>(ebn_ceil_div(K_in, SBM));
+  SmallProblem p1{K2, N2, R, 1.0f, X2, ldx2, dY2, lddy2, 0.0f, dW2, lddw2, static_cast<int32_t>(ebn_ceil_div(N2, SBN)), 0};
+  p1.tiles = p1.tiles_x * static_cast<int32_t>(ebn_ceil_div(K2, SBM));
+  constexpr size_t lds = static_cast<size_t>(2) * 2 * SBM * SLV * sizeof(float);
+  static const hipError_t attr = hipFuncSetAttribute(reinterpret_cast<const void*>(&gemm_small_triple_kernel),
+                                                     hipFuncAttributeMaxDynamicSharedMemorySize, static_cast<int>(lds));
+  if (attr != hipSuccess) return static_cast<int>(attr);
+  EBN_LAUNCH(gemm_small_triple_kernel, dim3(static_cast<unsigned>(pn.tiles + p0.tiles + p1.tiles)), dim3(GEMM_THREADS), lds, s, pn, p0, p1);
+  EBN_CHECK_LAUNCH();
+  return EBN_OK;
+}
+
 extern "C" int ebn_gemm_f32_rowmap(const int32_t* ids, int64_t table_rows, int64_t M, int64_t N, int64_t K, const float* table,
                                    int64_t ldt, const float* B, int64_t ldb, float* C, int64_t ldc, int32_t* oob_flag, ebn_stream_t stream) {
   EBN_REQUIRE(ebn_dim_ok(M, N, K) && table_rows > 0, EBN_ERR_BAD_ARG);
diff --git a/ebnerd-benchmark_amd/ebrec/models/newsrec/_engine.py b/ebnerd-benchmark_amd/ebrec/models/newsrec/_engine.py
--- a/ebnerd-benchmark_amd/ebrec/models/newsrec/_engine.py
+++ b/ebnerd-benchmark_amd/ebrec/models/newsrec/_engine.py
@@ -117,6 +117,7 @@
         self.loss_dev = torch.zeros(1, device=self.device)
         self.use_graph = False
         self.fuse_user_head = True
+        self.fuse_user_stage = True
         self.fuse_eval_gather = True
         self.defer_finish = True
         self.atomic_table_grad = False
@@ -788,12 +789,22 @@
         _hip.call("ebn_user_head_train_f32", _hip.ptr(ub.U), _hip.ptr(pv("u_b")), _hip.ptr(pv("u_q")), _hip.ptr(ub.Y), _hip.ptr(cand), _hip.ptr(nb.labels),
                   _hip.ptr(ub.w), _hip.ptr(ub.out), _hip.ptr(nb.scores), _hip.ptr(nb.probs), _hip.ptr(ub.loss_rows), _hip.ptr(self.loss_dev), _hip.ptr(dcand),
                   _hip.ptr(ub.duser), _hip.ptr(ub.de), None, None, _hip.ptr(ub.head_partials), B, H, C, E, A, self.loss_kind, ctypes.c_float(1.0 / B), S())
+        if self._user_stage_fused():
+            _hip.call("ebn_attn_bwd_pooled_proj_f32", _hip.ptr(ub.QKV), 3 * E, _hip.ptr(ub.U), A, _hip.ptr(pv("u_W")), A, A, _hip.ptr(ub.w),
+                      _hip.ptr(ub.duser), E, _hip.ptr(ub.dQKV), 3 * E, B, H, self.h, self.d, S())
+            _hip.call("ebn_dense_bwd_pair_tn_f32", R, E, 3 * E, _hip.ptr(X), E, _hip.ptr(ub.dQKV), 3 * E, _hip.ptr(pv("u_Wqkv")), 3 * E,
+                      _hip.ptr(g("u_Wqkv")), 3 * E, _hip.ptr(nb.dNE), E, E, A, _hip.ptr(ub.Y), E, _hip.ptr(ub.U), A, _hip.ptr(g("u_W")), A, ws, wsn, S())
+            return
         _hip.call("ebn_dense_bwd_pair_f32", R, E, A, _hip.ptr(ub.Y), E, _hip.ptr(ub.U), A, _hip.ptr(pv("u_W")), A, zero, _hip.ptr(g("u_W")), A,
                   _hip.ptr(ub.dY), E, ws, wsn, S())
         _hip.call("ebn_attn_bwd_pooled_f32", _hip.ptr(ub.QKV), 3 * E, _hip.ptr(ub.dY), E, _hip.ptr(ub.w), _hip.ptr(ub.duser), E, _hip.ptr(ub.dQKV), 3 * E,
                   B, H, self.h, self.d, None, -1, zero, S())
         _hip.call("ebn_dense_bwd_pair_f32", R, E, 3 * E, _hip.ptr(X), E, _hip.ptr(ub.dQKV), 3 * E, _hip.ptr(pv("u_Wqkv")), 3 * E, zero, _hip.ptr(g("u_Wqkv")),
                   3 * E, _hip.ptr(nb.dNE), E, ws, wsn, S())
+
+    def _user_stage_fused(self) -> bool:
+        return bool(self.fuse_user_stage and int(_hip.lib().ebn_user_stage_fused_supported(self.H, self.E, self.h, self.d, self.A)) != 0
+                    and self.params.view("u_W").data_ptr() % 16 == 0 and self.params.view("u_Wqkv").data_ptr() % 16 == 0)
 
     def _news_bwd_deferred(self, nb, ub, B, N, part):
         S, E, A, T, D = _hip.stream_handle, self.E, self.A, self.T, self.D
@@ -844,9 +855,9 @@
         grads = _hip.EncoderGrads(g("u_Wqkv").data_ptr(), g("u_W").data_ptr(), g("u_b").data_ptr(), g("u_q").data_ptr())
         scratch = _hip.EncoderScratch(ub.dY.data_ptr(), ub.dQKV.data_ptr(), ub.de.data_ptr(), ub.partials.data_ptr(),
                                       ub.ws.data_ptr(), ub.ws.numel())
-        _hip.call("ebn_user_stage_train_f32", ctypes.byref(dims), ctypes.byref(params), ctypes.byref(acts), _hip.ptr(cand),
-                  _hip.ptr(nb.labels), _hip.ptr(nb.scores), _hip.ptr(nb.probs), _hip.ptr(ub.loss_rows), _hip.ptr(self.loss_dev),
-                  _hip.ptr(dcand), _hip.ptr(ub.duser), ctypes.byref(grads), ctypes.byref(scratch),
+        _hip.call("ebn_user_stage_train_f32" if self.fuse_user_stage else "ebn_user_stage_train_unfused_f32", ctypes.byref(dims),
+                  ctypes.byref(params), ctypes.byref(acts), _hip.ptr(cand), _hip.ptr(nb.labels), _hip.ptr(nb.scores), _hip.ptr(nb.probs),
+                  _hip.ptr(ub.loss_rows), _hip.ptr(self.loss_dev), _hip.ptr(dcand), _hip.ptr(ub.duser), ctypes.byref(grads), ctypes.byref(scratch),
                   _hip.ptr(ub.head_partials) if self.fuse_user_head else None, _hip.ptr(nb.dNE), C, self.loss_kind,
                   ctypes.c_float(1.0 / B), st, S())
 
diff --git a/ebnerd-benchmark_amd/ebrec/models/newsrec/_engine_docvec.py b/ebnerd-benchmark_amd/ebrec/models/newsrec/_engine_docvec.py
--- a/ebnerd-benchmark_amd/ebrec/models/newsrec/_engine_docvec.py
+++ b/ebnerd-benchmark_amd/ebrec/models/newsrec/_engine_docvec.py
@@ -32,6 +32,7 @@
         self.params = FlatParams(shapes, self.device)
         self.use_graph, self._graphs = False, {}
         self.fuse_user_head = True
+        self.fuse_user_stage = True
         self.fuse_news_mlp = True
         self.fuse_finale = True
         self._dvn_dirty = False
@@ -408,7 +409,7 @@
             mb["labels"][: B * C].copy_(labels.reshape(-1).to(device=self.device, dtype=torch.float32))
         if self.use_graph:
             adv = self._advanced
-            gkey = (B, C, adv, bool(self.fuse_news_mlp), self.p, self.l2, bool(self.fuse_finale), bool(self.multi))
+            gkey = (B, C, adv, bool(self.fuse_news_mlp), self.p, self.l2, bool(self.fuse_finale), bool(self.multi), bool(self.fuse_user_stage))
             g = self._graphs.get(gkey)
             if g is None:
                 torch.cuda.synchronize()
@@ -459,8 +460,8 @@
         grads = _hip.EncoderGrads(g("u_Wqkv").data_ptr(), g("u_W").data_ptr(), g("u_b").data_ptr(), g("u_q").data_ptr())
         scratch = _hip.EncoderScratch(ub.dY.data_ptr(), ub.dQKV.data_ptr(), ub.de.data_ptr(), ub.partials.data_ptr(),
                                       ub.ws.data_ptr(), ub.ws.numel())
-        _hip.call("ebn_user_stage_train_f32", ctypes.byref(dims), ctypes.byref(params), ctypes.byref(acts), _hip.ptr(cand),
-                  _hip.ptr(mb["labels"]), _hip.ptr(mb["scores"]), _hip.ptr(mb["probs"]), _hip.ptr(ub.loss_rows), _hip.ptr(self.loss_dev),
+        _hip.call("ebn_user_stage_train_f32" if self.fuse_user_stage else "ebn_user_stage_train_unfused_f32", ctypes.byref(dims),
+                  ctypes.byref(params), ctypes.byref(acts), _hip.ptr(cand), _hip.ptr(mb["labels"]), _hip.ptr(mb["scores"]), _hip.ptr(mb["probs"]), _hip.ptr(ub.loss_rows), _hip.ptr(self.loss_dev),
                   _hip.ptr(mb["dNE"][n_hist:]), _hip.ptr(ub.duser), ctypes.byref(grads), ctypes.byref(scratch),
                   _hip.ptr(ub.head_partials) if self.fuse_user_head else None, _hip.ptr(mb["dNE"]), C, self.loss_kind,
                   ctypes.c_float(1.0 / B), st, S())
@@ -479,6 +480,13 @@
         _hip.call("ebn_user_head_train_f32", _hip.ptr(ub.U), _hip.ptr(pv("u_b")), _hip.ptr(pv("u_q")), _hip.ptr(ub.Y), _hip.ptr(cand), _hip.ptr(mb["labels"]),
                   _hip.ptr(ub.w), _hip.ptr(ub.out), _hip.ptr(mb["scores"]), _hip.ptr(mb["probs"]), _hip.ptr(ub.loss_rows), _hip.ptr(self.loss_dev), _hip.ptr(dcand),
                   _hip.ptr(ub.duser), _hip.ptr(ub.de), None, None, _hip.ptr(ub.head_partials), B, H, C, E, A, self.loss_kind, ctypes.c_float(1.0 / B), S())
+        if (self.fuse_user_stage and int(_hip.lib().ebn_user_stage_fused_supported(H, E, self.h, self.d, A)) != 0
+                and pv("u_W").data_ptr() % 16 == 0 and pv("u_Wqkv").data_ptr() % 16 == 0):
+            _hip.call("ebn_attn_bwd_pooled_proj_f32", _hip.ptr(ub.QKV), 3 * E, _hip.ptr(ub.U), A, _hip.ptr(pv("u_W")), A, A, _hip.ptr(ub.w),
+                      _hip.ptr(ub.duser), E, _hip.ptr(ub.dQKV), 3 * E, B, H, self.h, self.d, S())
+            _hip.call("ebn_dense_bwd_pair_tn_f32", R, E, 3 * E, _hip.ptr(X), E, _hip.ptr(ub.dQKV), 3 * E, _hip.ptr(pv("u_Wqkv")), 3 * E,
+                      _hip.ptr(g("u_Wqkv")), 3 * E, _hip.ptr(mb["dNE"]), E, E, A, _hip.ptr(ub.Y), E, _hip.ptr(ub.U), A, _hip.ptr(g("u_W")), A, ws, wsn, S())
+            return
         _hip.call("ebn_dense_bwd_pair_f32", R, E, A, _hip.ptr(ub.Y), E, _hip.ptr(ub.U), A, _hip.ptr(pv("u_W")), A, zero, _hip.ptr(g("u_W")), A,
                   _hip.ptr(ub.dY), E, ws, wsn, S())
         _hip.call("ebn_attn_bwd_pooled_f32", _hip.ptr(ub.QKV), 3 * E, _hip.ptr(ub.dY), E, _hip.ptr(ub.w), _hip.ptr(ub.duser), E, _hip.ptr(ub.dQKV), 3 * E,
diff --git a/ebnerd-benchmark_amd/ebrec/models/newsrec/_engine_segments.py b/ebnerd-benchmark_amd/ebrec/models/newsrec/_engine_segments.py
--- a/ebnerd-benchmark_amd/ebrec/models/newsrec/_engine_segments.py
+++ b/ebnerd-benchmark_amd/ebrec/models/newsrec/_engine_segments.py
@@ -105,7 +105,7 @@
         return self.graph_collectives
 
     def _graph_key(self, B, C, advanced=False):
-        return (B, C, advanced, bool(self.adam_in_finish), bool(self.defer_finish), bool(self.multi))
+        return (B, C, advanced, bool(self.adam_in_finish), bool(self.defer_finish), bool(self.multi), bool(self.fuse_user_stage))
 
     def _capture(self, B, C, advanced=False):
         torch.cuda.synchronize()
diff --git a/include/ebnerd_hip.h b/include/ebnerd_hip.h
--- a/include/ebnerd_hip.h
+++ b/include/ebnerd_hip.h
@@ -145,6 +145,11 @@
                             int32_t L, int32_t h, int32_t d, const ebn_step_state* st, int32_t site, float drop_p,
                             ebn_stream_t stream);
 int ebn_attn_bwd_pooled_supported(int32_t L, int32_t d);
+int ebn_attn_bwd_pooled_proj_f32(const float* qkv, int64_t ld_qkv, const float* dpre, int64_t ld_dpre, const float* W,
+                                 int64_t ldw, int32_t A, const float* pool_w, const float* pool_dout, int64_t ld_pool,
+                                 float* dqkv, int64_t ld_dqkv, int64_t n_seq, int32_t L, int32_t h, int32_t d,
+                                 ebn_stream_t stream);
+int ebn_user_stage_fused_supported(int32_t H, int32_t E, int32_t h, int32_t d, int32_t A);
 
 int ebn_gemm_f32_rank1(int64_t M, int64_t N, int64_t K, float alpha, const float* A, int64_t lda, const float* B,
                        int64_t ldb, float* C, int64_t ldc, const float* row_scale, const float* seq_rows,
@@ -153,6 +158,10 @@
 int ebn_dense_bwd_pair_f32(int64_t R, int64_t K_in, int64_t N_out, const float* X, int64_t ldx, const float* dY,
                            int64_t lddy, const float* W, int64_t ldw, float beta_w, float* dW, int64_t lddw, float* dX,
                            int64_t lddx, float* workspace, int64_t workspace_floats, ebn_stream_t stream);
+int ebn_dense_bwd_pair_tn_f32(int64_t R, int64_t K_in, int64_t N_out, const float* X, int64_t ldx, const float* dY,
+                              int64_t lddy, const float* W, int64_t ldw, float* dW, int64_t lddw, float* dX, int64_t lddx,
+                              int64_t K2, int64_t N2, const float* X2, int64_t ldx2, const float* dY2, int64_t lddy2,
+                              float* dW2, int64_t lddw2, float* workspace, int64_t workspace_floats, ebn_stream_t stream);
 
 int ebn_dense_relu_fwd_f32(int64_t M, int64_t N, int64_t K, const float* A, int64_t lda, const float* B, int64_t ldb,
                            const float* bias, float* C, int64_t ldc, float* workspace, int64_t workspace_floats,
@@ -230,6 +239,11 @@
                              float* loss_out, float* dcand, float* duser, const ebn_encoder_grads* g,
                              const ebn_encoder_scratch* s, float* head_partials, float* dX, int32_t C, int32_t loss_kind,
                              float inv_batch, const ebn_step_state* st, ebn_stream_t stream);
+int ebn_user_stage_train_unfused_f32(const ebn_encoder_dims* dims, const ebn_encoder_params* p, const ebn_encoder_acts* a,
+                                     const float* cand, const float* labels, float* scores, float* probs, float* loss_rows,
+                                     float* loss_out, float* dcand, float* duser, const ebn_encoder_grads* g,
+                                     const ebn_encoder_scratch* s, float* head_partials, float* dX, int32_t C,
+                                     int32_t loss_kind, float inv_batch, const ebn_step_state* st, ebn_stream_t stream);
 
 int ebn_score_fwd_f32(const float* cand, const float* user, float* scores, float* probs,
                       int64_t B, int32_t C, int32_t E, int32_t mode, ebn_stream_t stream);
```

After: 25570, median of 6. No clear change (+0.3%).
